# kessel/dune-pnp

Hardware: NVIDIA B200
Metric: newton_step_dofs_per_s (higher is better)
Workload: dtype f64

## Files before the change

### dune_pnp_b200/capi.py

```python
import ctypes as C
import os

import numpy as np

_HERE = os.path.dirname(os.path.abspath(__file__))
LIB_PATH = os.path.join(_HERE, "libpnp_b200.so")

OP_PB, OP_POISSON, OP_DIFFUSION, OP_MASS, OP_PNP = range(5)
JAC_FD_FAITHFUL, JAC_ANALYTIC = 0, 1
SOLVER_BCGS, SOLVER_CG = 0, 1
PREC_NONE, PREC_JACOBI, PREC_SSOR, PREC_ILU0, PREC_AMG = range(5)
TIME_ALEXANDER2, TIME_IMPLICIT_EULER = 0, 1
STATUS = {0: "PNP_OK", 1: "PNP_E_NOT_CONVERGED", 2: "PNP_E_LINEAR_SOLVER", 3: "PNP_E_LINE_SEARCH", 4: "PNP_E_NAN",
          5: "PNP_E_BREAKDOWN", 6: "PNP_E_CUDA", 7: "PNP_E_CONFIG", 8: "PNP_E_ARG", 9: "PNP_E_MESH"}

_dp = C.POINTER(C.c_double)
_ip = C.POINTER(C.c_int)


class LinResult(C.Structure):
    _fields_ = [("converged", C.c_int), ("iterations", C.c_int), ("reduction", C.c_double), ("conv_rate", C.c_double),
                ("seconds", C.c_double), ("status", C.c_int)]


class NewtonOpts(C.Structure):
    _fields_ = [("reduction", C.c_double), ("abs_limit", C.c_double), ("min_linear_reduction", C.c_double),
                ("reassemble_threshold", C.c_double), ("max_iterations", C.c_int),
                ("line_search_max_iterations", C.c_int), ("damping", C.c_double), ("jac_mode", C.c_int),
                ("fd_epsilon", C.c_double), ("verbosity", C.c_int), ("line_search_strategy", C.c_int)]


class NewtonResult(C.Structure):
    _fields_ = [("converged", C.c_int), ("iterations", C.c_int), ("first_defect", C.c_double), ("defect", C.c_double),
                ("reduction", C.c_double), ("linear_iterations", C.c_int), ("line_search_trials", C.c_int),
                ("jacobian_assemblies", C.c_int), ("residual_assemblies", C.c_int), ("seconds_assembly", C.c_double),
                ("seconds_solve", C.c_double), ("seconds_total", C.c_double), ("n_history", C.c_int),
                ("defect_history", C.c_double * 64), ("linear_iterations_history", C.c_int * 64)]


class PnpError(RuntimeError):
    def __init__(self, status, msg):
        super().__init__("%s: %s" % (STATUS.get(status, status), msg))
        self.status = status


_LIB = None


def lib():
    global _LIB
    if _LIB is None:
        if not os.path.exists(LIB_PATH):
            raise ImportError("libpnp_b200.so is missing: run `python -c 'import __graft_entry__ as g; g.build()'` "
                              "(make -C dune_pnp_b200/csrc)")
        try:
            import importlib.util
            for pkg, names in (("nvidia.nccl", ["libnccl.so.2"]), ("nvidia.nvjitlink", ["libnvJitLink.so.12"]),
                               ("nvidia.cublas", ["libcublasLt.so.12", "libcublas.so.12"]),
                               ("nvidia.cusparse", ["libcusparse.so.12"]), ("nvidia.cusolver", ["libcusolver.so.11"])):
                spec = importlib.util.find_spec(pkg)
                if spec is None or not spec.submodule_search_locations:
                    continue
                for nm in names:
                    cand = os.path.join(list(spec.submodule_search_locations)[0], "lib", nm)
                    if os.path.exists(cand):
                        C.CDLL(cand, mode=C.RTLD_GLOBAL)
        except Exception:
            pass
        L = C.CDLL(LIB_PATH)
        L.pnp_last_error.restype = C.c_char_p
        L.pnp_launch_count.restype = C.c_long
        _LIB = L
    return _LIB


def _d(a):
    return None if a is None else a.ctypes.data_as(_dp)


def _i(a):
    return None if a is None else a.ctypes.data_as(_ip)


def tune(name, value):
    st = lib().pnp_tune(name.encode(), C.c_double(value))
    if st != 0:
        raise PnpError(st, "unknown tuning knob " + name)


class Context:

    def __init__(self, device=0, parent=None):
        self._h = C.c_void_p()
        self._children = []
        if parent is not None:
            st = lib().pnp_ctx_create_child(parent._h, C.byref(self._h))
            parent._children.append(self)
        else:
            st = lib().pnp_ctx_create(device, C.byref(self._h))
        if st != 0:
            raise PnpError(st, "cannot create a context on CUDA device %d (no CPU fallback exists)" % device)

    def close(self):
        if self._h:
            lib().pnp_ctx_destroy(self._h)
            self._h = C.c_void_p()

    def __del__(self):
        try:
            self.close()
        except Exception:
            pass

    def _ck(self, st):
        if st != 0:
            raise PnpError(st, lib().pnp_last_error(self._h).decode())

    def profile_spmv(self, enable):
        self._ck(lib().pnp_profile_spmv(self._h, int(enable)))

    def profile_spmv_get(self):
        n = (C.c_long * 3)(); ms = (C.c_double * 3)()
        self._ck(lib().pnp_profile_spmv_get(self._h, n, ms))
        return list(n), list(ms)

    def profile_bytes(self, reset=False):
        out = (C.c_double * 6)()
        self._ck(lib().pnp_profile_bytes(self._h, int(reset), out))
        return dict(zip(("spmv_fine", "spmv_coarse", "assembly", "blas1", "transfer", "dense"), list(out)))

    def profiler_range(self, start):
        self._ck(lib().pnp_profiler_range(self._h, int(start)))

    def timer_start(self):
        self._ck(lib().pnp_timer_start(self._h))

    def timer_stop(self):
        ms = C.c_double()
        self._ck(lib().pnp_timer_stop(self._h, C.byref(ms)))
        return ms.value

    def launch_count(self):
        return lib().pnp_launch_count(self._h)

    def mesh_set(self, x, y, tri, ba, bb, bphys):
        x = np.ascontiguousarray(x, dtype=np.float64); y = np.ascontiguousarray(y, dtype=np.float64)
        tri = np.ascontiguousarray(tri, dtype=np.int32); ba = np.ascontiguousarray(ba, dtype=np.int32)
        bb = np.ascontiguousarray(bb, dtype=np.int32); bphys = np.ascontiguousarray(bphys, dtype=np.int32)
        self._ck(lib().pnp_mesh_set(self._h, C.c_long(len(x)), _d(x), _d(y), C.c_long(len(tri)), _i(tri), C.c_long(len(ba)),
                                    _i(ba), _i(bb), _i(bphys)))

    def mesh_read_gmsh(self, path):
        self._ck(lib().pnp_mesh_read_gmsh(self._h, path.encode()))

    def mesh_refine(self, levels):
        self._ck(lib().pnp_mesh_refine(self._h, levels))

    def carry_set(self, vecs):
        arr = (C.c_int * len(vecs))(*vecs)
        self._ck(lib().pnp_carry_set(self._h, arr, len(vecs)))

    def carry_get(self, index, vec):
        self._ck(lib().pnp_carry_get(self._h, index, vec))

    def carry_set_host(self, field):
        field = np.ascontiguousarray(field, dtype=np.float64)
        self._ck(lib().pnp_carry_set_host(self._h, field.shape[0] if field.ndim == 2 else 1, _d(field)))

    def carry_get_host(self, index, fields):
        out = np.zeros((fields, self.mesh_sizes()["nv"]))
        self._ck(lib().pnp_carry_get_host(self._h, index, _d(out)))
        return out

    def mesh_set_local(self, n_own, x, y, tri, ba, bb, bphys):
        x = np.ascontiguousarray(x, dtype=np.float64); y = np.ascontiguousarray(y, dtype=np.float64)
        tri = np.ascontiguousarray(tri, dtype=np.int32); ba = np.ascontiguousarray(ba, dtype=np.int32)
        bb = np.ascontiguousarray(bb, dtype=np.int32); bphys = np.ascontiguousarray(bphys, dtype=np.int32)
        self._ck(lib().pnp_mesh_set_local(self._h, C.c_long(len(x)), C.c_long(n_own), _d(x), _d(y), C.c_long(len(tri)), _i(tri),
                                          C.c_long(len(ba)), _i(ba), _i(bb), _i(bphys)))

    def mesh_owned(self):
        n = C.c_long()
        self._ck(lib().pnp_mesh_owned(self._h, C.byref(n)))
        return n.value

    @staticmethod
    def comm_unique_id():
        buf = C.create_string_buffer(128)
        if lib().pnp_comm_unique_id(buf) != 0:
            raise PnpError(6, "ncclGetUniqueId failed")
        return buf.raw

    def comm_init(self, rank, world, unique_id):
        self._ck(lib().pnp_comm_init(self._h, rank, world, C.c_char_p(unique_id) if world > 1 else None))

    def halo_set(self, nbr, send_ptr, send_idx, recv_ptr):
        nbr = np.ascontiguousarray(nbr, dtype=np.int32); send_ptr = np.ascontiguousarray(send_ptr, dtype=np.int32)
        send_idx = np.ascontiguousarray(send_idx, dtype=np.int32); recv_ptr = np.ascontiguousarray(recv_ptr, dtype=np.int32)
        self._ck(lib().pnp_halo_set(self._h, len(nbr), _i(nbr), _i(send_ptr), _i(send_idx), _i(recv_ptr)))

    def mg_push_level(self, child, par0, par1):
        par0 = np.ascontiguousarray(par0, dtype=np.int32); par1 = np.ascontiguousarray(par1, dtype=np.int32)
        self._ck(lib().pnp_mg_push_level(self._h, child._h, _i(par0), _i(par1)))

    def mg_set_coarse_global(self, gid, n_global):
        gid = np.ascontiguousarray(gid, dtype=np.int32)
        self._ck(lib().pnp_mg_set_coarse_global(self._h, _i(gid), C.c_long(n_global)))

    def mg_set_coarse_replica(self, replica, gid, n_global):
        gid = np.ascontiguousarray(gid, dtype=np.int32)
        self._ck(lib().pnp_mg_set_coarse_replica(self._h, replica._h, _i(gid), C.c_long(n_global)))

    def mg_set_coarse_aggregates(self, agg, n_agg):
        agg = np.ascontiguousarray(agg, dtype=np.int32)
        self._ck(lib().pnp_mg_set_coarse_aggregates(self._h, _i(agg), C.c_long(n_agg)))

    def halo_exchange(self, vec):
        self._ck(lib().pnp_halo_exchange(self._h, vec))

    def mesh_finalize(self, renumber=True):
        self._ck(lib().pnp_mesh_finalize(self._h, int(renumber)))

    def mesh_sizes(self):
        v = [C.c_long() for _ in range(4)]
        self._ck(lib().pnp_mesh_sizes(self._h, *[C.byref(a) for a in v]))
        return dict(nv=v[0].value, nT=v[1].value, nB=v[2].value, nslots=v[3].value)

    def mesh_get(self):
        s = self.mesh_sizes()
        x = np.zeros(s["nv"]); y = np.zeros(s["nv"]); tri = np.zeros((s["nT"], 3), dtype=np.int32)
        ba = np.zeros(s["nB"], dtype=np.int32); bb = np.zeros(s["nB"], dtype=np.int32); ph = np.zeros(s["nB"], dtype=np.int32)
        self._ck(lib().pnp_mesh_get(self._h, _d(x), _d(y), _i(tri), _i(ba), _i(bb), _i(ph)))
        return dict(x=x, y=y, tri=tri, ba=ba, bb=bb, bphys=ph)

    def params_set(self, sys, surf):
        sys = np.ascontiguousarray(sys, dtype=np.float64); surf = np.ascontiguousarray(surf, dtype=np.float64)
        self._ck(lib().pnp_params_set(self._h, _d(sys), _d(surf)))

    def params_read(self, path):
        self._ck(lib().pnp_params_read(self._h, path.encode()))

    def params_get(self):
        sys = np.zeros(16)
        self._ck(lib().pnp_params_get(self._h, _d(sys), None, None, 0))
        surf = np.zeros((int(sys[0]), 9)); buf = C.create_string_buffer(512)
        self._ck(lib().pnp_params_get(self._h, _d(sys), _d(surf), buf, 512))
        return sys, surf, buf.value.decode()

    def operator(self, op, comp0=0):
        h = C.c_int()
        self._ck(lib().pnp_operator_create(self._h, op, comp0, C.byref(h)))
        return h.value

    def operator_set_coefficient(self, op, which, vec):
        self._ck(lib().pnp_operator_set_coefficient(self._h, op, which, vec))

    def operator_set_valency(self, op, valency):
        self._ck(lib().pnp_operator_set_valency(self._h, op, C.c_double(valency)))

    def constraints(self, op, fields):
        out = np.zeros(fields * self.ndof(), dtype=np.int8)
        self._ck(lib().pnp_constraints_get(self._h, op, out.ctypes.data_as(C.c_char_p)))
        return out.astype(bool)

    def pattern(self, op, fields):
        nv = self.ndof()
        nnz = C.c_long(); rowptr = np.zeros(fields * nv + 1, dtype=np.int32)
        self._ck(lib().pnp_pattern_get(self._h, op, C.byref(nnz), _i(rowptr), None))
        col = np.zeros(nnz.value, dtype=np.int32)
        self._ck(lib().pnp_pattern_get(self._h, op, C.byref(nnz), _i(rowptr), _i(col)))
        return rowptr, col

    def vec(self, fields, host=None):
        h = C.c_int()
        self._ck(lib().pnp_vec_create(self._h, fields, C.byref(h)))
        if host is not None:
            self.upload(h.value, host)
        return h.value

    def vec_destroy(self, v):
        self._ck(lib().pnp_vec_destroy(self._h, v))

    def upload(self, v, host):
        host = np.ascontiguousarray(host, dtype=np.float64)
        self._ck(lib().pnp_vec_upload(self._h, v, _d(host)))

    def download(self, v, fields):
        out = np.zeros(fields * self.ndof())
        self._ck(lib().pnp_vec_download(self._h, v, _d(out)))
        return out

    def vec_set(self, v, value):
        self._ck(lib().pnp_vec_set(self._h, v, C.c_double(value)))

    def vec_copy(self, dst, src):
        self._ck(lib().pnp_vec_copy(self._h, dst, src))

    def axpy(self, y, a, x):
        self._ck(lib().pnp_vec_axpy(self._h, y, C.c_double(a), x))

    def norm(self, x):
        out = C.c_double()
        self._ck(lib().pnp_vec_norm(self._h, x, C.byref(out)))
        return out.value

    def dot(self, x, y):
        out = C.c_double()
        self._ck(lib().pnp_vec_dot(self._h, x, y, C.byref(out)))
        return out.value

    def pack3(self, dst3, phi, cp, cm):
        self._ck(lib().pnp_vec_pack3(self._h, dst3, phi, cp, cm))

    def extract(self, src3, field, dst1):
        self._ck(lib().pnp_vec_extract(self._h, src3, field, dst1))

    def matrix(self, op):
        h = C.c_int()
        self._ck(lib().pnp_matrix_create(self._h, op, C.byref(h)))
        return h.value

    def matrix_destroy(self, m):
        self._ck(lib().pnp_matrix_destroy(self._h, m))

    def residual(self, op, u, r):
        self._ck(lib().pnp_residual(self._h, op, u, r))

    def jacobian(self, op, u, A, mode=JAC_FD_FAITHFUL, eps=1e-11):
        self._ck(lib().pnp_jacobian(self._h, op, u, A, mode, C.c_double(eps)))

    def matrix_values(self, op, A, nnz):
        val = np.zeros(nnz)
        self._ck(lib().pnp_matrix_values_get(self._h, op, A, _d(val)))
        return val

    def spmv(self, A, x, y):
        self._ck(lib().pnp_spmv(self._h, A, x, y))

    def solver(self, kind=SOLVER_BCGS, prec=PREC_NONE, maxit=5000, prec_steps=1, verbosity=0):
        h = C.c_int()
        self._ck(lib().pnp_solver_create(self._h, kind, prec, maxit, prec_steps, verbosity, C.byref(h)))
        return h.value

    def solver_set_option(self, solver, name, value):
        self._ck(lib().pnp_solver_set_option(self._h, solver, name.encode(), C.c_double(value)))

    def solver_get(self, solver, name):
        out = C.c_double(0)
        self._ck(lib().pnp_solver_get(self._h, solver, name.encode(), C.byref(out)))
        return out.value

    def precond_apply(self, solver, A, d, v):
        self._ck(lib().pnp_precond_apply(self._h, solver, A, d, v))

    def solve(self, solver, A, z, r, reduction):
        res = LinResult()
        self._ck(lib().pnp_solver_apply(self._h, solver, A, z, r, C.c_double(reduction), C.byref(res)))
        return res

    def newton_opts(self, **kw):
        o = NewtonOpts()
        self._ck(lib().pnp_newton_opts_from_params(self._h, C.byref(o)))
        for k, v in kw.items():
            setattr(o, k, v)
        return o

    def newton(self, op, u, solver, opts, check=True):
        res = NewtonResult()
        st = lib().pnp_newton_apply(self._h, op, u, solver, C.byref(opts), C.byref(res))
        if check:
            self._ck(st)
        return st, res

    def slp(self, op, u, solver, reduction, jac_mode=JAC_FD_FAITHFUL, eps=1e-11):
        res = LinResult()
        self._ck(lib().pnp_slp_apply(self._h, op, u, solver, C.c_double(reduction), jac_mode, C.c_double(eps), C.byref(res)))
        return res

    def onestep(self, op_space, op_time, solver, dt, x_old, dirichlet_values, x_new, reduction=1e-5, method=TIME_ALEXANDER2,
                jac_mode=JAC_FD_FAITHFUL, eps=1e-11, time=0.0):
        res = (LinResult * 2)()
        self._ck(lib().pnp_onestep_apply(self._h, method, op_space, op_time, solver, C.c_double(time), C.c_double(dt), x_old,
                                         dirichlet_values, x_new, C.c_double(reduction), jac_mode, C.c_double(eps), res))
        return list(res)[: (1 if method == TIME_IMPLICIT_EULER else 2)]

    def ion_flux(self, phi, cp, cm):
        ns = int(self.params_get()[0][0])
        ip = np.zeros(ns); im = np.zeros(ns)
        self._ck(lib().pnp_ion_flux(self._h, phi, cp, cm, _d(ip), _d(im)))
        return ip, im

    def write_cell_data(self, vec, filename):
        self._ck(lib().pnp_write_cell_data(self._h, vec, filename.encode()))

    def write_vtk(self, name, vecs, names, ascii=False):
        arr = (C.c_int * len(vecs))(*vecs)
        nm = (C.c_char_p * len(names))(*[n.encode() for n in names])
        self._ck(lib().pnp_write_vtk(self._h, name.encode(), len(vecs), arr, nm, int(ascii)))

    def matrix_set_csr(self, op, A, rowptr, col, val):
        rowptr = np.ascontiguousarray(rowptr, dtype=np.int32); col = np.ascontiguousarray(col, dtype=np.int32)
        val = np.ascontiguousarray(val, dtype=np.float64)
        self._ck(lib().pnp_matrix_set_csr(self._h, op, A, _i(rowptr), _i(col), _d(val)))

    def mesh_renumber(self, new_index):
        new_index = np.ascontiguousarray(new_index, dtype=np.int32)
        self._ck(lib().pnp_mesh_renumber(self._h, _i(new_index)))

    def space_set_degree(self, degree):
        self._ck(lib().pnp_space_set_degree(self._h, int(degree)))

    def space_sizes(self):
        deg = C.c_int(); nE = C.c_long(); nd = C.c_long()
        self._ck(lib().pnp_space_sizes(self._h, C.byref(deg), C.byref(nE), C.byref(nd)))
        return dict(degree=deg.value, n_edges=nE.value, ndof=nd.value)

    def space_offsets(self):
        eo = C.c_long(); vo = C.c_long()
        self._ck(lib().pnp_space_offsets(self._h, C.byref(eo), C.byref(vo)))
        return eo.value, vo.value

    def operator_set_intorder(self, op, intorder):
        self._ck(lib().pnp_operator_set_intorder(self._h, op, int(intorder)))

    def ndof(self):
        return self.space_sizes()["ndof"]

    def space_edges(self):
        nE = self.space_sizes()["n_edges"]
        va = np.zeros(nE, dtype=np.int32); vb = np.zeros(nE, dtype=np.int32)
        self._ck(lib().pnp_space_edges(self._h, _i(va), _i(vb)))
        return va, vb

    def interpolate_bcext(self, component, pb_vec, out_vec):
        self._ck(lib().pnp_interpolate_bcext(self._h, component, -1 if pb_vec is None else pb_vec, out_vec))
```

### dune_pnp_b200/csrc/pnp_amg.cu

```cuda
#include <cub/cub.cuh>
#include <cusolverDn.h>

#include <chrono>
#include <cmath>
#include <cstdlib>
#include <cstring>

#include "pnp_common.cuh"
#include "pnp_spmv_tma.cuh"
#include "pnp_sweep.cuh"

namespace pnp {

std::shared_ptr<SweepPlan> sweep_plan_build(Ctx&, const SweepView&, int F);
void sweep_gs(Ctx&, const SweepPlan&, const SweepView&, const double* vals, long stride, const double* d, double* x, int dir);

namespace {

constexpr int BLK = 256;

struct Level {
  int nv = 0; long nslots = 0;
  const int* rp = nullptr; const unsigned* col = nullptr; const double* vals = nullptr;
  DBuf<int> rp_own; DBuf<unsigned> col_own; DBuf<double> vals_own;
  DBuf<double> dinv, x, x2, b, r;
  double lmax = 2.0;
  DBuf<int> agg, par1;
  DBuf<int> agg_ptr, agg_mem;
  DBuf<int> seg_ptr, seg_items;
  DBuf<unsigned char> seg_w;
  double alpha = 1.0;
  Ctx* lc = nullptr;
  Vec u; Matrix Amat;
  const unsigned char* dm = nullptr;
  bool redisc = false;
  DBuf<XY> xy_own; DBuf<unsigned char> dmask_own;
  std::shared_ptr<SweepPlan> gs_plan;
};

}

struct Amg {
  int NP = 1, F = 1;
  bool symbolic = false;
  long nv0 = -1, nslots0 = -1;
  long mg_epoch = -1;
  double sym_key = 0.0;
  double omega = 0.7, alpha = 1.6;
  int coarse_sweeps = 40;
  int gamma = 1;
  int wlevels = 99;
  int smoother = 0;
  double cheb_ratio = 8.0;
  int comp0 = 0;
  int pre_steps = -1, post_steps = -1;
  int dense_max = 4096, dense_n = 0;
  cusolverDnHandle_t cus = nullptr;
  DBuf<double> dense, dense_work;
  DBuf<int> dense_piv, dense_info;
  bool distributed = false;
  bool redisc = false;
  DBuf<double> grhs;
  std::unique_ptr<Solver> rep_solver; Matrix rep_A; Vec rep_u; DBuf<double> rep_x;
  int n_geo = 0;
  std::vector<std::unique_ptr<Level>> L;
  DBuf<unsigned char> tmp;
  void* temp(size_t bytes) { if (bytes > tmp.n) tmp.alloc(bytes); return tmp.p; }
  cudaGraphExec_t cg_exec = nullptr;
  bool cg_failed = false;
  int cg_calls = 0;
  double cg_key[8] = {0, 0, 0, 0, 0, 0, 0, 0};
  std::vector<std::pair<double*, double*>> cg_before, cg_after;
  long cg_launches = 0; double cg_bytes[Ctx::ACC_N] = {0, 0, 0, 0, 0, 0};
  void cg_reset() { if (cg_exec) cudaGraphExecDestroy(cg_exec); cg_exec = nullptr; cg_calls = 0; }
  ~Amg() { if (cg_exec) cudaGraphExecDestroy(cg_exec); if (cus) cusolverDnDestroy(cus); }
};

namespace {

__device__ __forceinline__ unsigned hash32(unsigned x) {
  x ^= x >> 16; x *= 0x7feb352du; x ^= x >> 15; x *= 0x846ca68bu; x ^= x >> 16;
  return x;
}
__global__ void k_mis_select(const int* __restrict__ rp, const unsigned* __restrict__ col, int nv,
                             const unsigned char* __restrict__ st, unsigned char* __restrict__ st_out) {
  for (int v = blockIdx.x * blockDim.x + threadIdx.x; v < nv; v += gridDim.x * blockDim.x) {
    unsigned char s = st[v];
    if (s == 0) {
      const unsigned pv = hash32((unsigned)v);
      bool win = true;
      for (int k = rp[v] + 1; k < rp[v + 1]; k++) {
        const int w = (int)(col[k] & STAR_VMASK);
        if (w >= nv || w == v || st[w] != 0) continue;
        const unsigned pw = hash32((unsigned)w);
        if (pw > pv || (pw == pv && w > v)) { win = false; break; }
      }
      if (win) s = 1;
    }
    st_out[v] = s;
  }
}
__global__ void k_mis_cover(const int* __restrict__ rp, const unsigned* __restrict__ col, int nv,
                            unsigned char* __restrict__ st, int* __restrict__ undecided) {
  int local = 0;
  for (int v = blockIdx.x * blockDim.x + threadIdx.x; v < nv; v += gridDim.x * blockDim.x) {
    if (st[v] != 0) continue;
    bool covered = false;
    for (int k = rp[v] + 1; k < rp[v + 1]; k++) {
      const int w = (int)(col[k] & STAR_VMASK);
      if (w < nv && st[w] == 1) { covered = true; break; }
    }
    if (covered) st[v] = 2; else local++;
  }
  if (local) atomicAdd(undecided, local);
}
__global__ void k_root_flag(const unsigned char* __restrict__ st, int nv, int* __restrict__ flag) {
  for (int v = blockIdx.x * blockDim.x + threadIdx.x; v < nv; v += gridDim.x * blockDim.x) flag[v] = st[v] == 1;
}
__global__ void k_attach(const int* __restrict__ rp, const unsigned* __restrict__ col, const double* __restrict__ vals,
                         int nv, const unsigned char* __restrict__ st, const int* __restrict__ root_id,
                         int* __restrict__ agg) {
  for (int v = blockIdx.x * blockDim.x + threadIdx.x; v < nv; v += gridDim.x * blockDim.x) {
    if (st[v] == 1) { agg[v] = root_id[v]; continue; }
    double best = -1.0; int bw = -1;
    for (int k = rp[v] + 1; k < rp[v + 1]; k++) {
      const int w = (int)(col[k] & STAR_VMASK);
      if (w >= nv || st[w] != 1) continue;
      const double s = fabs(vals[k]);
      if (s > best || (s == best && w < bw)) { best = s; bw = w; }
    }
    agg[v] = root_id[bw];
  }
}
__global__ void k_coarse_keys(const int* __restrict__ rp, const unsigned* __restrict__ col, int nv,
                              const int* __restrict__ agg, uint64_t* __restrict__ keys, int* __restrict__ slot_id) {
  for (int v = blockIdx.x * blockDim.x + threadIdx.x; v < nv; v += gridDim.x * blockDim.x) {
    const unsigned I = (unsigned)agg[v];
    for (int k = rp[v]; k < rp[v + 1]; k++) {
      const unsigned w = col[k] & STAR_VMASK;
      if (w >= (unsigned)nv) { keys[k] = ~0ull; slot_id[k] = k; continue; }
      const unsigned J = (unsigned)agg[w];
      keys[k] = ((uint64_t)I << 32) | (J == I ? 0u : J + 1u);
      slot_id[k] = k;
    }
  }
}
__global__ void k_coarse_cols(const uint64_t* __restrict__ ukeys, long n, unsigned* __restrict__ col) {
  for (long i = blockIdx.x * (long)blockDim.x + threadIdx.x; i < n; i += (long)gridDim.x * blockDim.x) {
    const unsigned lo = (unsigned)(ukeys[i] & 0xffffffffu);
    col[i] = lo == 0 ? (unsigned)(ukeys[i] >> 32) : lo - 1u;
  }
}
__global__ void k_row_starts(const uint64_t* __restrict__ ukeys, long n, int nc, int* __restrict__ rp) {
  for (int I = blockIdx.x * blockDim.x + threadIdx.x; I <= nc; I += gridDim.x * blockDim.x)
    rp[I] = (int)lower_bound_u64(ukeys, n, (uint64_t)(unsigned)I << 32);
}
__global__ void k_lower_bounds_i32(const int* __restrict__ sorted, int n, int m, int* __restrict__ out) {
  for (int I = blockIdx.x * blockDim.x + threadIdx.x; I <= m; I += gridDim.x * blockDim.x) {
    int lo = 0, hi = n;
    while (lo < hi) { int mid = (lo + hi) >> 1; if (sorted[mid] < I) lo = mid + 1; else hi = mid; }
    out[I] = lo;
  }
}
__global__ void k_iota(int* a, int n) {
  for (int i = blockIdx.x * blockDim.x + threadIdx.x; i < n; i += gridDim.x * blockDim.x) a[i] = i;
}

template <int NP>
__global__ void k_galerkin(const int* __restrict__ seg_ptr, const int* __restrict__ seg_items,
                           const unsigned char* __restrict__ seg_w, long nsc, const double* __restrict__ vf, long nsf, double* __restrict__ vc,
                           const unsigned char* __restrict__ dmask, const unsigned* __restrict__ colf, const int* __restrict__ rpf,
                           int comp0) {
  for (long cs = blockIdx.x * (long)blockDim.x + threadIdx.x; cs < nsc; cs += (long)gridDim.x * blockDim.x) {
    double acc[NP];
#pragma unroll
    for (int p = 0; p < NP; p++) acc[p] = 0.0;
    constexpr int U = 4;
    const int t1 = seg_ptr[cs + 1];
    for (int t0 = seg_ptr[cs]; t0 < t1; t0 += U) {
      int s[U]; double w[U]; double v[U][NP];
#pragma unroll
      for (int q = 0; q < U; q++) {
        const bool ok = t0 + q < t1;
        s[q] = ok ? seg_items[t0 + q] : -1;
        const unsigned char wc = (ok && seg_w) ? seg_w[t0 + q] : 0;
        w[q] = ok ? (wc == 0 ? 1.0 : (wc == 1 ? 0.5 : 0.25)) : 0.0;
      }
#pragma unroll
      for (int q = 0; q < U; q++)
#pragma unroll
        for (int p = 0; p < NP; p++) v[q][p] = s[q] >= 0 ? vf[p * nsf + s[q]] : 0.0;
      if (dmask) {
#pragma unroll
        for (int q = 0; q < U; q++) {
          if (s[q] < 0) continue;
          const unsigned wv = colf[s[q]] & STAR_VMASK;
          const unsigned m = dmask[wv];
          if (m && rpf[wv] == s[q]) {
            if (NP == 1) { if ((m >> comp0) & 1u) v[q][0] = 0.0; }
            else if (NP == PNP_COMPACT_PLANES) { if (m & 1u) v[q][0] = 0.0; }
            else {
              if (m & 1u) v[q][0] = 0.0;
              if (m & 2u) v[q][NP == 7 ? 4 : 0] = 0.0;
              if (m & 4u) v[q][NP == 7 ? 6 : 0] = 0.0;
            }
          }
        }
      }
#pragma unroll
      for (int q = 0; q < U; q++)
        if (s[q] >= 0) {
#pragma unroll
          for (int p = 0; p < NP; p++) acc[p] += w[q] * v[q][p];
        }
    }
#pragma unroll
    for (int p = 0; p < NP; p++) vc[p * nsc + cs] = acc[p];
  }
}
template <int NP>
__global__ void k_dinv(const int* __restrict__ rp, const double* __restrict__ vals, long stride, int nv,
                       double* __restrict__ dinv) {
  for (int v = blockIdx.x * blockDim.x + threadIdx.x; v < nv; v += gridDim.x * blockDim.x) {
    const int s = rp[v];
    if (NP == 1) { const double d = vals[s]; dinv[v] = d != 0.0 ? 1.0 / d : 0.0; }
    else {
      const PnpBlock B = pnp_block_at<NP>(vals, stride, s);
      const double a = B.a, b = B.b, c_ = B.c, d = B.d, e = B.e, f = B.f, g = B.g;
      const double det = a * e * g - b * d * g - c_ * e * f;
      double* o = dinv + 9l * v;
      const double scale = fabs(a * e * g) + fabs(b * d * g) + fabs(c_ * e * f);
      if (fabs(det) > 1e-12 * scale && scale > 0.0) {
        const double id = 1.0 / det;
        o[0] = e * g * id;   o[1] = -b * g * id;           o[2] = -c_ * e * id;
        o[3] = -d * g * id;  o[4] = (a * g - c_ * f) * id; o[5] = c_ * d * id;
        o[6] = -e * f * id;  o[7] = b * f * id;            o[8] = (a * e - b * d) * id;
      } else {
        for (int i = 0; i < 9; i++) o[i] = 0.0;
        o[0] = a != 0.0 ? 1.0 / a : 0.0; o[4] = e != 0.0 ? 1.0 / e : 0.0; o[8] = g != 0.0 ? 1.0 / g : 0.0;
      }
    }
  }
}
template <int F>
__global__ void k_jacobi0(const double* __restrict__ dinv, const double* __restrict__ b, double omega,
                          double* __restrict__ x, int nv, double* __restrict__ dvec) {
  for (int v = blockIdx.x * blockDim.x + threadIdx.x; v < nv; v += gridDim.x * blockDim.x) {
    if (F == 1) {
      const double z = omega * dinv[v] * b[v];
      x[v] = z; if (dvec) dvec[v] = z;
    } else {
      const double* B = dinv + 9l * v;
      const double r0 = b[3l * v], r1 = b[3l * v + 1], r2 = b[3l * v + 2];
#pragma unroll
      for (int k = 0; k < 3; k++) {
        const double z = omega * (B[3 * k] * r0 + B[3 * k + 1] * r1 + B[3 * k + 2] * r2);
        x[3l * v + k] = z; if (dvec) dvec[3l * v + k] = z;
      }
    }
  }
}
template <int NP>
__global__ void k_gershgorin(const int* __restrict__ rp, const double* __restrict__ vals, long stride, int nv,
                             unsigned long long* __restrict__ out) {
  double best = 0.0;
  for (int v = blockIdx.x * blockDim.x + threadIdx.x; v < nv; v += gridDim.x * blockDim.x) {
    const int s0 = rp[v], s1 = rp[v + 1];
    if (NP == 1) {
      double sum = 0.0;
      for (int s = s0; s < s1; s++) sum += fabs(vals[s]);
      const double d = fabs(vals[s0]);
      if (d > 0.0) best = fmax(best, sum / d);
    } else {
      double s0_ = 0.0, s1_ = 0.0, s2_ = 0.0;
      for (int s = s0; s < s1; s++) {
        const PnpBlock B = pnp_block_at<NP>(vals, stride, s);
        s0_ += fabs(B.a) + fabs(B.b) + fabs(B.c);
        s1_ += fabs(B.d) + fabs(B.e);
        s2_ += fabs(B.f) + fabs(B.g);
      }
      const PnpBlock D = pnp_block_at<NP>(vals, stride, s0);
      const double d0 = fabs(D.a), d1 = fabs(D.e), d2 = fabs(D.g);
      if (d0 > 0.0) best = fmax(best, s0_ / d0);
      if (d1 > 0.0) best = fmax(best, s1_ / d1);
      if (d2 > 0.0) best = fmax(best, s2_ / d2);
    }
  }
  for (int o = 16; o > 0; o >>= 1) best = fmax(best, __shfl_xor_sync(0xffffffffu, best, o));
  if ((threadIdx.x & 31) == 0) atomicMax(out, (unsigned long long)__double_as_longlong(best));
}
template <int F>
__global__ void k_restrict(const int* __restrict__ agg_ptr, const int* __restrict__ agg_mem, const int* __restrict__ par1,
                           int nc, const double* __restrict__ r, double* __restrict__ bc) {
  for (int I = blockIdx.x * blockDim.x + threadIdx.x; I < nc; I += gridDim.x * blockDim.x) {
    double acc[F];
#pragma unroll
    for (int k = 0; k < F; k++) acc[k] = 0.0;
    for (int t = agg_ptr[I]; t < agg_ptr[I + 1]; t++) {
      const long v = agg_mem[t];
      const double w = (par1 && par1[v] >= 0) ? 0.5 : 1.0;
#pragma unroll
      for (int k = 0; k < F; k++) acc[k] += w * r[F * v + k];
    }
#pragma unroll
    for (int k = 0; k < F; k++) bc[(long)F * I + k] = acc[k];
  }
}
template <int F>
__global__ void k_prolong(const int* __restrict__ agg, const int* __restrict__ par1, int nv, const double* __restrict__ xc,
                          double alpha, double* __restrict__ x, const unsigned char* __restrict__ dmask, int comp0) {
  for (int v = blockIdx.x * blockDim.x + threadIdx.x; v < nv; v += gridDim.x * blockDim.x) {
    const long I = agg[v];
    const long J = par1 ? par1[v] : -1;
    const unsigned m = dmask ? (F == 3 ? dmask[v] : (dmask[v] >> comp0) & 1u) : 0u;
#pragma unroll
    for (int k = 0; k < F; k++)
      if (!((m >> k) & 1u))
        x[(long)F * v + k] += alpha * (J >= 0 ? 0.5 * (xc[F * I + k] + xc[F * J + k]) : xc[F * I + k]);
  }
}
__global__ void k_level_geometry(const int* __restrict__ int2ext_c, const int* __restrict__ ext2int_f, const XY* __restrict__ xy_f,
                                 const unsigned char* __restrict__ dmask_f, int nvc, XY* __restrict__ xy_c,
                                 unsigned char* __restrict__ dmask_c) {
  for (int i = blockIdx.x * blockDim.x + threadIdx.x; i < nvc; i += gridDim.x * blockDim.x) {
    const int j = ext2int_f[int2ext_c[i]];
    xy_c[i] = xy_f[j]; dmask_c[i] = dmask_f[j];
  }
}
__global__ void k_geo_parents(const int* __restrict__ int2ext_f, int nvf, int nvc, const uint64_t* __restrict__ edges,
                              const int* __restrict__ ext2int_c, int* __restrict__ par0, int* __restrict__ par1) {
  for (int i = blockIdx.x * blockDim.x + threadIdx.x; i < nvf; i += gridDim.x * blockDim.x) {
    const int e = int2ext_f[i];
    if (e < nvc) { par0[i] = ext2int_c[e]; par1[i] = -1; }
    else {
      const uint64_t k = edges[e - nvc];
      par0[i] = ext2int_c[(int)(k >> 32)]; par1[i] = ext2int_c[(int)(k & 0xffffffffu)];
    }
  }
}
__global__ void k_geo_pairs(const int* __restrict__ par0, const int* __restrict__ par1, int nvf, int nrows_c,
                            int* __restrict__ key, int* __restrict__ val) {
  for (int i = blockIdx.x * blockDim.x + threadIdx.x; i < nvf; i += gridDim.x * blockDim.x) {
    key[2 * i] = (par0[i] >= 0 && par0[i] < nrows_c) ? par0[i] : 0x7fffffff; val[2 * i] = i;
    key[2 * i + 1] = (par1[i] >= 0 && par1[i] < nrows_c) ? par1[i] : 0x7fffffff; val[2 * i + 1] = i;
  }
}
template <int F>
__global__ void k_inject(const int* __restrict__ par0, const int* __restrict__ par1, int nvf, const double* __restrict__ uf,
                         double* __restrict__ uc) {
  for (int i = blockIdx.x * blockDim.x + threadIdx.x; i < nvf; i += gridDim.x * blockDim.x)
    if (par1[i] < 0 && par0[i] >= 0) {
#pragma unroll
      for (int k = 0; k < F; k++) uc[(long)F * par0[i] + k] = uf[(long)F * i + k];
    }
}
template <int F>
__global__ void k_mask_dirichlet(double* __restrict__ b, const unsigned char* __restrict__ dmask, int nv, int comp0) {
  for (int v = blockIdx.x * blockDim.x + threadIdx.x; v < nv; v += gridDim.x * blockDim.x) {
    const unsigned m = F == 3 ? dmask[v] : (dmask[v] >> comp0) & 1u;
#pragma unroll
    for (int k = 0; k < F; k++) if ((m >> k) & 1u) b[(long)F * v + k] = 0.0;
  }
}
template <int NP>
__global__ void k_dense_fill_global(const int* __restrict__ rp, const unsigned* __restrict__ col, const double* __restrict__ vals,
                                    long stride, int nrows, const int* __restrict__ gid, double* __restrict__ Ad, long n,
                                    const unsigned char* __restrict__ dmask, int comp0) {
  constexpr int F = NP == 1 ? 1 : 3;
  for (int r = blockIdx.x * blockDim.x + threadIdx.x; r < nrows; r += gridDim.x * blockDim.x) {
    const long rg = gid[r];
    for (int s = rp[r]; s < rp[r + 1]; s++) {
      const long cg = gid[col[s] & STAR_VMASK];
      const unsigned dm = (dmask && s == rp[r]) ? dmask[r] : 0u;
      if (NP == 1) { if (!((dm >> comp0) & 1u)) atomicAdd(&Ad[cg * n + rg], vals[s]); }
      else {
        const PnpBlock B = pnp_block_at<NP>(vals, stride, s);
#pragma unroll
        for (int ki = 0; ki < 3; ki++)
#pragma unroll
          for (int kj = 0; kj < 3; kj++)
            if (pnp_plane(ki, kj) >= 0 && !(ki == kj && ((dm >> ki) & 1u))) atomicAdd(&Ad[(F * cg + kj) * n + F * rg + ki], B.at(ki, kj));
      }
    }
  }
}
template <int F>
__global__ void k_to_global(const double* __restrict__ loc, const int* __restrict__ gid, int nrows, double* __restrict__ glob) {
  for (int v = blockIdx.x * blockDim.x + threadIdx.x; v < nrows; v += gridDim.x * blockDim.x)
#pragma unroll
    for (int k = 0; k < F; k++) atomicAdd(&glob[(long)F * gid[v] + k], loc[(long)F * v + k]);
}
template <int F>
__global__ void k_add_from_global(const double* __restrict__ glob, const int* __restrict__ gid, int nrows, double alpha,
                                  double* __restrict__ x, const unsigned char* __restrict__ dmask, int comp0) {
  for (int v = blockIdx.x * blockDim.x + threadIdx.x; v < nrows; v += gridDim.x * blockDim.x) {
    const unsigned m = F == 3 ? dmask[v] : (dmask[v] >> comp0) & 1u;
#pragma unroll
    for (int k = 0; k < F; k++) if (!((m >> k) & 1u)) x[(long)F * v + k] += alpha * glob[(long)F * gid[v] + k];
  }
}
template <int F>
__global__ void k_from_global(const double* __restrict__ glob, const int* __restrict__ gid, int nloc, double* __restrict__ loc) {
  for (int v = blockIdx.x * blockDim.x + threadIdx.x; v < nloc; v += gridDim.x * blockDim.x)
#pragma unroll
    for (int k = 0; k < F; k++) loc[(long)F * v + k] = glob[(long)F * gid[v] + k];
}
__device__ __forceinline__ int find_slot(const int* rp, const unsigned* col, int I, int J) {
  for (int s = rp[I]; s < rp[I + 1]; s++) if ((int)(col[s] & STAR_VMASK) == J) return s;
  return -1;
}
__global__ void k_geo_items(const int* __restrict__ rpf, const unsigned* __restrict__ colf, int nvf,
                            const int* __restrict__ par0, const int* __restrict__ par1, const int* __restrict__ rpc,
                            const unsigned* __restrict__ colc, int* __restrict__ key, unsigned* __restrict__ val,
                            int* __restrict__ err) {
  for (int i = blockIdx.x * blockDim.x + threadIdx.x; i < nvf; i += gridDim.x * blockDim.x) {
    const int I[2] = {par0[i], par1[i]};
    for (int s = rpf[i]; s < rpf[i + 1]; s++) {
      const int j = (int)(colf[s] & STAR_VMASK);
      const int J[2] = {par0[j], par1[j]};
#pragma unroll
      for (int a = 0; a < 2; a++)
#pragma unroll
        for (int b = 0; b < 2; b++) {
          const long o = 4l * s + 2 * a + b;
          if (I[a] < 0 || J[b] < 0) { key[o] = 0x7fffffff; val[o] = 0; continue; }
          const int cs = find_slot(rpc, colc, I[a], J[b]);
          if (cs < 0) { atomicExch(err, 1); key[o] = 0x7fffffff; val[o] = 0; continue; }
          const unsigned wc = (I[1] >= 0 ? 1u : 0u) + (J[1] >= 0 ? 1u : 0u);
          key[o] = cs; val[o] = (unsigned)s | (wc << 29);
        }
    }
  }
}
__global__ void k_geo_unpack(const unsigned* __restrict__ val, long n, int* __restrict__ items, unsigned char* __restrict__ w) {
  for (long t = blockIdx.x * (long)blockDim.x + threadIdx.x; t < n; t += (long)gridDim.x * blockDim.x) {
    items[t] = (int)(val[t] & 0x1fffffffu); w[t] = (unsigned char)(val[t] >> 29);
  }
}

#define KL(c, kern, n, ...)                                                                              \
  do { kern<<<grid_for((n), BLK), BLK, 0, (c).stream>>>(__VA_ARGS__); PNP_CHECK_LAUNCH(); (c).launches++; } while (0)

template <int EPI>
void level_op(Ctx& c, const Amg& A, const Level& l, const double* x, const double* b, double* y, double omega_or_c2 = -1.0,
              double c1 = 0.0, double* dvec = nullptr) {
  StarOpArgs a{l.rp, l.col, l.vals, l.nslots, l.nv, x, y};
  a.b = b; a.dinv = l.dinv.p; a.block = A.F == 3; a.omega = omega_or_c2 < 0 ? A.omega : omega_or_c2; a.c1 = c1; a.dvec = dvec;
  const bool fine = &l == A.L[0].get();
  if (A.distributed) halo_exchange(*l.lc, const_cast<double*>(x), A.F);
  if (fine) c.prof_mark(EPI == EPI_RESIDUAL ? 1 : 2);
  launch_star_op_auto<EPI, 0>(c, A.NP, a, fine);
  if (fine) c.prof_mark();
}

bool coarsen(Ctx& c, Amg& A, int li) {
  Level& f = *A.L[li];
  const int nv = f.nv;
  DBuf<unsigned char> st(nv), st2(nv);
  st.zero(c.stream);
  DBuf<int> d_und(1);
  for (int round = 0; round < 200; round++) {
    KL(c, k_mis_select, nv, f.rp, f.col, nv, st.p, st2.p);
    std::swap(st.p, st2.p);
    d_und.zero(c.stream);
    KL(c, k_mis_cover, nv, f.rp, f.col, nv, st.p, d_und.p);
    int und = 0;
    d_und.download(&und, 1, c.stream);
    if (und == 0) break;
    PNP_REQUIRE(round < 199, PNP_E_ARG, "AMG: independent-set selection did not terminate");
  }
  DBuf<int> flag(nv), root_id(nv);
  KL(c, k_root_flag, nv, st.p, nv, flag.p);
  size_t bytes = 0;
  cub::DeviceScan::ExclusiveSum(nullptr, bytes, flag.p, root_id.p, nv, c.stream);
  PNP_CUDA(cub::DeviceScan::ExclusiveSum(A.temp(bytes), bytes, flag.p, root_id.p, nv, c.stream));
  int last_id = 0, last_flag = 0;
  PNP_CUDA(cudaMemcpyAsync(&last_id, root_id.p + nv - 1, sizeof(int), cudaMemcpyDeviceToHost, c.stream));
  PNP_CUDA(cudaMemcpyAsync(&last_flag, flag.p + nv - 1, sizeof(int), cudaMemcpyDeviceToHost, c.stream));
  PNP_CUDA(cudaStreamSynchronize(c.stream));
  const int nc = last_id + last_flag;
  if (nc < 1 || nc > 0.8 * nv) return false;
  f.alpha = A.alpha;
  f.agg.alloc(nv);
  KL(c, k_attach, nv, f.rp, f.col, f.vals, nv, st.p, root_id.p, f.agg.p);
  {
    DBuf<int> ids(nv), agg_sorted(nv);
    f.agg_mem.alloc(nv); f.agg_ptr.alloc(nc + 1);
    KL(c, k_iota, nv, ids.p, nv);
    cub::DeviceRadixSort::SortPairs(nullptr, bytes, f.agg.p, agg_sorted.p, ids.p, f.agg_mem.p, nv, 0, 32, c.stream);
    PNP_CUDA(cub::DeviceRadixSort::SortPairs(A.temp(bytes), bytes, f.agg.p, agg_sorted.p, ids.p, f.agg_mem.p, nv, 0, 32,
                                            c.stream));
    KL(c, k_lower_bounds_i32, nc + 1, agg_sorted.p, nv, nc, f.agg_ptr.p);
  }
  auto nl = std::make_unique<Level>();
  {
    const long ns = f.nslots;
    PNP_REQUIRE(ns < (1l << 31), PNP_E_MESH, "AMG: too many matrix slots on one level");
    DBuf<uint64_t> keys(ns), skeys(ns), ukeys(ns);
    DBuf<int> slot(ns), counts(ns + 1), d_nu(1);
    f.seg_items.alloc(ns);
    KL(c, k_coarse_keys, nv, f.rp, f.col, nv, f.agg.p, keys.p, slot.p);
    cub::DeviceRadixSort::SortPairs(nullptr, bytes, keys.p, skeys.p, slot.p, f.seg_items.p, (int)ns, 0, 64, c.stream);
    PNP_CUDA(cub::DeviceRadixSort::SortPairs(A.temp(bytes), bytes, keys.p, skeys.p, slot.p, f.seg_items.p, (int)ns, 0, 64,
                                            c.stream));
    cub::DeviceRunLengthEncode::Encode(nullptr, bytes, skeys.p, ukeys.p, counts.p, d_nu.p, (int)ns, c.stream);
    PNP_CUDA(cub::DeviceRunLengthEncode::Encode(A.temp(bytes), bytes, skeys.p, ukeys.p, counts.p, d_nu.p, (int)ns, c.stream));
    int nu = 0;
    d_nu.download(&nu, 1, c.stream);
    {
      uint64_t lastkey = 0;
      PNP_CUDA(cudaMemcpyAsync(&lastkey, ukeys.p + (nu - 1), sizeof(uint64_t), cudaMemcpyDeviceToHost, c.stream));
      PNP_CUDA(cudaStreamSynchronize(c.stream));
      if (lastkey == ~0ull) nu--;
    }
    nl->nv = nc; nl->nslots = nu;
    PNP_CUDA(cudaMemsetAsync(counts.p + nu, 0, sizeof(int), c.stream));
    f.seg_ptr.alloc((size_t)nu + 1);
    cub::DeviceScan::ExclusiveSum(nullptr, bytes, counts.p, f.seg_ptr.p, nu + 1, c.stream);
    PNP_CUDA(cub::DeviceScan::ExclusiveSum(A.temp(bytes), bytes, counts.p, f.seg_ptr.p, nu + 1, c.stream));
    nl->rp_own.alloc((size_t)nc + 1); nl->col_own.alloc(nu);
    KL(c, k_row_starts, nc + 1, ukeys.p, (long)nu, nc, nl->rp_own.p);
    KL(c, k_coarse_cols, nu, ukeys.p, (long)nu, nl->col_own.p);
    c.launches += 8;
    PNP_CUDA(cudaStreamSynchronize(c.stream));
  }
  nl->vals_own.alloc((size_t)A.NP * nl->nslots);
  nl->rp = nl->rp_own.p; nl->col = nl->col_own.p; nl->vals = nl->vals_own.p;
  A.L.push_back(std::move(nl));
  return true;
}

void coarsen_geometric(Ctx& c, Amg& A, int li, const HierLevel& h, const int* int2ext_f, bool redisc) {
  Level& f = *A.L[li];
  const int nvf = f.nv, nvc = (int)h.nv;
  size_t bytes = 0;
  f.agg.alloc(nvf); f.par1.alloc(nvf);
  KL(c, k_geo_parents, nvf, int2ext_f, nvf, nvc, h.edges.p, h.ext2int.p, f.agg.p, f.par1.p);
  {
    DBuf<int> key(2 * (size_t)nvf), val(2 * (size_t)nvf), skey(2 * (size_t)nvf), sval(2 * (size_t)nvf);
    KL(c, k_geo_pairs, nvf, f.agg.p, f.par1.p, nvf, nvc, key.p, val.p);
    cub::DeviceRadixSort::SortPairs(nullptr, bytes, key.p, skey.p, val.p, sval.p, 2 * nvf, 0, 32, c.stream);
    PNP_CUDA(cub::DeviceRadixSort::SortPairs(A.temp(bytes), bytes, key.p, skey.p, val.p, sval.p, 2 * nvf, 0, 32, c.stream));
    f.agg_ptr.alloc((size_t)nvc + 1);
    KL(c, k_lower_bounds_i32, nvc + 1, skey.p, 2 * nvf, nvc, f.agg_ptr.p);
    int nvalid = 0;
    PNP_CUDA(cudaMemcpyAsync(&nvalid, f.agg_ptr.p + nvc, sizeof(int), cudaMemcpyDeviceToHost, c.stream));
    PNP_CUDA(cudaStreamSynchronize(c.stream));
    f.agg_mem.alloc(nvalid);
    PNP_CUDA(cudaMemcpyAsync(f.agg_mem.p, sval.p, (size_t)nvalid * sizeof(int), cudaMemcpyDeviceToDevice, c.stream));
    PNP_CUDA(cudaStreamSynchronize(c.stream));
  }
  auto nl = std::make_unique<Level>();
  nl->nv = nvc; nl->nslots = h.nslots; nl->rp = h.rp.p; nl->col = h.adj.p;
  nl->redisc = redisc;
  if (redisc) {
    nl->xy_own.alloc(nvc); nl->dmask_own.alloc(nvc);
    KL(c, k_level_geometry, nvc, h.int2ext.p, c.ext2int.p, c.xy.p, c.dmask.p, nvc, nl->xy_own.p, nl->dmask_own.p);
    nl->dm = nl->dmask_own.p;
    nl->u.fields = A.F; nl->u.d.alloc((size_t)A.F * nvc);
  } else {
    const long n4 = 4 * f.nslots;
    PNP_REQUIRE(n4 < (1l << 31) && f.nslots < (1l << 29), PNP_E_MESH, "multigrid: too many matrix slots on one level");
    DBuf<int> key(n4), skey(n4), err(1);
    DBuf<unsigned> val(n4), sval(n4);
    err.zero(c.stream);
    KL(c, k_geo_items, nvf, f.rp, f.col, nvf, f.agg.p, f.par1.p, nl->rp, nl->col, key.p, val.p, err.p);
    int herr = 0;
    err.download(&herr, 1, c.stream);
    PNP_REQUIRE(herr == 0, PNP_E_MESH, "multigrid: refinement levels are not nested");
    cub::DeviceRadixSort::SortPairs(nullptr, bytes, key.p, skey.p, val.p, sval.p, (int)n4, 0, 32, c.stream);
    PNP_CUDA(cub::DeviceRadixSort::SortPairs(A.temp(bytes), bytes, key.p, skey.p, val.p, sval.p, (int)n4, 0, 32, c.stream));
    key.release(); val.release();
    f.seg_ptr.alloc((size_t)nl->nslots + 1);
    KL(c, k_lower_bounds_i32, nl->nslots + 1, skey.p, (int)n4, (int)nl->nslots, f.seg_ptr.p);
    int nvalid = 0;
    PNP_CUDA(cudaMemcpyAsync(&nvalid, f.seg_ptr.p + nl->nslots, sizeof(int), cudaMemcpyDeviceToHost, c.stream));
    PNP_CUDA(cudaStreamSynchronize(c.stream));
    f.seg_items.alloc(nvalid); f.seg_w.alloc(nvalid);
    KL(c, k_geo_unpack, nvalid, sval.p, (long)nvalid, f.seg_items.p, f.seg_w.p);
    PNP_CUDA(cudaStreamSynchronize(c.stream));
    c.launches += 4;
  }
  f.alpha = 1.0;
  nl->vals_own.alloc((size_t)A.NP * nl->nslots);
  nl->vals = nl->vals_own.p;
  A.L.push_back(std::move(nl));
}

void alloc_work(Ctx& c, Amg& A, Level& l) {
  const size_t n = (size_t)A.F * l.nv, nall = (A.distributed && l.lc) ? (size_t)A.F * l.lc->nv : n;
  l.dinv.alloc(A.F == 3 ? 9 * (size_t)l.nv : n); l.x.alloc(nall); l.x2.alloc(nall); l.b.alloc(nall); l.r.alloc(nall);
  l.x.zero(c.stream); l.x2.zero(c.stream); l.b.zero(c.stream); l.r.zero(c.stream);
}

void coarsen_distributed(Ctx& c, Amg& A, int li, MgLevelRef& ref) {
  Level& f = *A.L[li];
  Ctx& fc = *f.lc; Ctx& kc = *ref.lc;
  const int nvf_all = (int)fc.nv, nvc = (int)kc.n_own;
  size_t bytes = 0;
  f.agg.alloc(nvf_all); f.par1.alloc(nvf_all);
  PNP_CUDA(cudaMemcpyAsync(f.agg.p, ref.par0.p, nvf_all * sizeof(int), cudaMemcpyDeviceToDevice, c.stream));
  PNP_CUDA(cudaMemcpyAsync(f.par1.p, ref.par1.p, nvf_all * sizeof(int), cudaMemcpyDeviceToDevice, c.stream));
  {
    DBuf<int> key(2 * (size_t)nvf_all), val(2 * (size_t)nvf_all), skey(2 * (size_t)nvf_all), sval(2 * (size_t)nvf_all);
    KL(c, k_geo_pairs, nvf_all, f.agg.p, f.par1.p, nvf_all, nvc, key.p, val.p);
    cub::DeviceRadixSort::SortPairs(nullptr, bytes, key.p, skey.p, val.p, sval.p, 2 * nvf_all, 0, 32, c.stream);
    PNP_CUDA(cub::DeviceRadixSort::SortPairs(A.temp(bytes), bytes, key.p, skey.p, val.p, sval.p, 2 * nvf_all, 0, 32, c.stream));
    f.agg_ptr.alloc((size_t)nvc + 1);
    KL(c, k_lower_bounds_i32, nvc + 1, skey.p, 2 * nvf_all, nvc, f.agg_ptr.p);
    int nvalid = 0;
    PNP_CUDA(cudaMemcpyAsync(&nvalid, f.agg_ptr.p + nvc, sizeof(int), cudaMemcpyDeviceToHost, c.stream));
    PNP_CUDA(cudaStreamSynchronize(c.stream));
    f.agg_mem.alloc(nvalid);
    PNP_CUDA(cudaMemcpyAsync(f.agg_mem.p, sval.p, (size_t)nvalid * sizeof(int), cudaMemcpyDeviceToDevice, c.stream));
    PNP_CUDA(cudaStreamSynchronize(c.stream));
  }
  f.alpha = 1.0;
  auto nl = std::make_unique<Level>();
  nl->lc = &kc; nl->nv = nvc; nl->nslots = kc.nslots; nl->rp = kc.rp.p; nl->col = kc.adj.p;
  nl->dm = kc.dmask.p;
  nl->u.fields = A.F; nl->u.d.alloc((size_t)A.F * kc.nv); nl->u.d.zero(c.stream);
  nl->Amat.op = A.F == 3 ? OP_PNP : OP_PB; nl->Amat.nplanes = A.NP;
  nl->Amat.vals.alloc((size_t)A.NP * kc.nslots);
  nl->vals = nl->Amat.vals.p;
  A.L.push_back(std::move(nl));
}

void dense_factor(Ctx& c, Amg& A);

void dense_factor_global(Ctx& c, Amg& A);
void replica_setup(Ctx& c, Amg& A);

const double* level_values(Ctx& c, Amg& A, int li, const double* uf, int comp0) {
  Level& l = *A.L[li]; Level& n = *A.L[li + 1];
  if (n.redisc) {
    if (A.F == 1) KL(c, k_inject<1>, l.nv, l.agg.p, l.par1.p, l.nv, uf, n.u.d.p);
    else KL(c, k_inject<3>, l.nv, l.agg.p, l.par1.p, l.nv, uf, n.u.d.p);
    c.acct(Ctx::ACC_TRANSFER, 8.0 * l.nv + 16.0 * A.F * n.nv);
    Operator op = c.last_op; op.aux0 = op.aux1 = -1;
    assemble_jacobian_on(c, StarView{n.rp, n.col, n.xy_own.p, n.dmask_own.p, n.nv}, n.nslots, op, n.u.d.p, n.vals_own.p,
                         A.NP, c.last_mode, c.last_eps);
    return n.u.d.p;
  }
  if (A.NP == 1)
    KL(c, k_galerkin<1>, n.nslots, l.seg_ptr.p, l.seg_items.p, l.seg_w.p, n.nslots, l.vals, l.nslots, n.vals_own.p, l.dm, l.col, l.rp, comp0);
  else if (A.NP == PNP_COMPACT_PLANES)
    KL(c, k_galerkin<PNP_COMPACT_PLANES>, n.nslots, l.seg_ptr.p, l.seg_items.p, l.seg_w.p, n.nslots, l.vals, l.nslots, n.vals_own.p, l.dm, l.col, l.rp, comp0);
  else
    KL(c, k_galerkin<7>, n.nslots, l.seg_ptr.p, l.seg_items.p, l.seg_w.p, n.nslots, l.vals, l.nslots, n.vals_own.p, l.dm, l.col, l.rp, comp0);
  c.acct(Ctx::ACC_ASSEMBLY, 8.0 * A.NP * ((double)l.nslots + (double)n.nslots) + 5.0 * (double)l.seg_items.n + 4.0 * (double)n.nslots);
  return nullptr;
}

void level_dinv(Ctx& c, Amg& A, Level& l) {
  if (A.NP == 1) KL(c, k_dinv<1>, l.nv, l.rp, l.vals, l.nslots, l.nv, l.dinv.p);
  else if (A.NP == PNP_COMPACT_PLANES) KL(c, k_dinv<PNP_COMPACT_PLANES>, l.nv, l.rp, l.vals, l.nslots, l.nv, l.dinv.p);
  else KL(c, k_dinv<7>, l.nv, l.rp, l.vals, l.nslots, l.nv, l.dinv.p);
}

void gershgorin_bounds(Ctx& c, Amg& A) {
  DBuf<unsigned long long> d_l(A.L.size());
  d_l.zero(c.stream);
  for (size_t li = 0; li < A.L.size(); li++) {
    Level& l = *A.L[li];
    if (A.NP == 1) KL(c, k_gershgorin<1>, l.nv, l.rp, l.vals, l.nslots, l.nv, d_l.p + li);
    else if (A.NP == PNP_COMPACT_PLANES) KL(c, k_gershgorin<PNP_COMPACT_PLANES>, l.nv, l.rp, l.vals, l.nslots, l.nv, d_l.p + li);
    else KL(c, k_gershgorin<7>, l.nv, l.rp, l.vals, l.nslots, l.nv, d_l.p + li);
  }
  if (A.distributed) allreduce_max_u64(c, d_l.p, A.L.size());
  std::vector<unsigned long long> h = d_l.to_host(c.stream);
  for (size_t li = 0; li < A.L.size(); li++) {
    double v; std::memcpy(&v, &h[li], sizeof v);
    A.L[li]->lmax = (v > 0.0 && std::isfinite(v)) ? v : 2.0;
  }
}

void numeric(Ctx& c, Amg& A, int comp0) {
  if (A.distributed) {
    PNP_REQUIRE(c.last_u, PNP_E_ARG, "distributed multigrid needs the state of the last Jacobian assembly (the vector must stay alive)");
    PNP_REQUIRE(c.last_vals == A.L[0]->vals, PNP_E_ARG,
                "distributed multigrid re-discretises its coarse levels: the matrix must be the Jacobian of the last assembly");
    const double* uf = c.last_u;
    for (size_t li = 0; li + 1 < A.L.size(); li++) {
      Level& l = *A.L[li]; Level& n = *A.L[li + 1];
      const int nvf_all = (int)l.lc->nv;
      if (A.F == 1) KL(c, k_inject<1>, nvf_all, l.agg.p, l.par1.p, nvf_all, uf, n.u.d.p);
      else KL(c, k_inject<3>, nvf_all, l.agg.p, l.par1.p, nvf_all, uf, n.u.d.p);
      c.acct(Ctx::ACC_TRANSFER, 8.0 * nvf_all + 16.0 * A.F * n.nv);
      Operator op = c.last_op; op.aux0 = op.aux1 = -1;
      n.Amat.op = op.op;
      n.lc->launches = 0;
      assemble_jacobian(*n.lc, op, n.u, n.Amat, c.last_mode, c.last_eps);
      c.absorb(*n.lc);
      uf = n.u.d.p;
    }
    for (size_t li = 0; li < A.L.size(); li++) {
      Level& l = *A.L[li];
      level_dinv(c, A, l);
      c.acct(Ctx::ACC_ASSEMBLY, (4.0 + 8.0 * A.NP + (A.F == 3 ? 72.0 : 8.0)) * l.nv);
    }
    if (c.mg_replica) replica_setup(c, A); else dense_factor_global(c, A);
    if (A.smoother == 1) gershgorin_bounds(c, A);
    return;
  }
  const double* uf = c.last_u;
  for (size_t li = 0; li < A.L.size(); li++) {
    Level& l = *A.L[li];
    if (li + 1 < A.L.size()) uf = level_values(c, A, (int)li, uf, comp0);
    level_dinv(c, A, l);
    c.acct(Ctx::ACC_ASSEMBLY, (4.0 + 8.0 * A.NP + (A.F == 3 ? 72.0 : 8.0)) * l.nv);
  }
  A.dense_n = 0;
  if ((long)A.F * A.L.back()->nv <= A.dense_max) dense_factor(c, A);
  if (A.smoother == 1) gershgorin_bounds(c, A);
}

template <int NP>
__global__ void k_dense_fill(const int* __restrict__ rp, const unsigned* __restrict__ col, const double* __restrict__ vals,
                             long stride, int nv, double* __restrict__ Ad, long n) {
  constexpr int F = NP == 1 ? 1 : 3;
  for (int r = blockIdx.x * blockDim.x + threadIdx.x; r < nv; r += gridDim.x * blockDim.x)
    for (int s = rp[r]; s < rp[r + 1]; s++) {
      const long cidx = col[s] & STAR_VMASK;
      if (cidx >= nv) continue;
      if (NP == 1) Ad[cidx * n + r] = vals[s];
      else {
        const PnpBlock B = pnp_block_at<NP>(vals, stride, s);
#pragma unroll
        for (int ki = 0; ki < 3; ki++)
#pragma unroll
          for (int kj = 0; kj < 3; kj++)
            if (pnp_plane(ki, kj) >= 0) Ad[(F * cidx + kj) * n + F * r + ki] = B.at(ki, kj);
      }
    }
}
__global__ void k_dense_fix_diag(double* __restrict__ Ad, long n) {
  for (long i = blockIdx.x * (long)blockDim.x + threadIdx.x; i < n; i += (long)gridDim.x * blockDim.x)
    if (Ad[i * n + i] == 0.0) Ad[i * n + i] = 1.0;
}
#define PNP_CUSOLVER(call)                                                                                          \
  do { cusolverStatus_t s_ = (call); if (s_ != CUSOLVER_STATUS_SUCCESS)                                             \
    throw ::pnp::Error(PNP_E_CUDA, std::string(#call) + " -> cusolver status " + std::to_string((int)s_)); } while (0)

void dense_factor(Ctx& c, Amg& A) {
  Level& l = *A.L.back();
  const long n = (long)A.F * l.nv;
  A.dense_n = (int)n;
  if (!A.cus) PNP_CUSOLVER(cusolverDnCreate(&A.cus));
  PNP_CUSOLVER(cusolverDnSetStream(A.cus, c.stream));
  if (A.dense.n != (size_t)(n * n)) { A.dense.alloc(n * n); A.dense_piv.alloc(n); A.dense_info.alloc(1); }
  A.dense.zero(c.stream);
  if (A.NP == 1) KL(c, k_dense_fill<1>, l.nv, l.rp, l.col, l.vals, l.nslots, l.nv, A.dense.p, n);
  else if (A.NP == PNP_COMPACT_PLANES) KL(c, k_dense_fill<PNP_COMPACT_PLANES>, l.nv, l.rp, l.col, l.vals, l.nslots, l.nv, A.dense.p, n);
  else KL(c, k_dense_fill<7>, l.nv, l.rp, l.col, l.vals, l.nslots, l.nv, A.dense.p, n);
  KL(c, k_dense_fix_diag, n, A.dense.p, n);
  int lwork = 0;
  PNP_CUSOLVER(cusolverDnDgetrf_bufferSize(A.cus, (int)n, (int)n, A.dense.p, (int)n, &lwork));
  if (A.dense_work.n < (size_t)lwork) A.dense_work.alloc(lwork);
  PNP_CUSOLVER(cusolverDnDgetrf(A.cus, (int)n, (int)n, A.dense.p, (int)n, A.dense_work.p, A.dense_piv.p, A.dense_info.p));
  c.acct(Ctx::ACC_DENSE, 24.0 * (double)n * (double)n);
  int info = 0;
  A.dense_info.download(&info, 1, c.stream);
  PNP_REQUIRE(info == 0, PNP_E_BREAKDOWN, "multigrid: coarsest-level matrix is singular (LU info " + std::to_string(info) + ")");
}
void dense_solve(Ctx& c, Amg& A, Level& l) {
  const long n = A.dense_n;
  PNP_CUDA(cudaMemcpyAsync(l.x.p, l.b.p, n * sizeof(double), cudaMemcpyDeviceToDevice, c.stream));
  PNP_CUSOLVER(cusolverDnDgetrs(A.cus, CUBLAS_OP_N, (int)n, 1, A.dense.p, (int)n, A.dense_piv.p, l.x.p, (int)n, A.dense_info.p));
  c.launches += 2; c.acct(Ctx::ACC_DENSE, 8.0 * (double)n * (double)n);
}

void dense_factor_global(Ctx& c, Amg& A) {
  Level& l = *A.L.back();
  const long n = (long)A.F * c.mg_nglobal;
  A.dense_n = (int)n;
  if (!A.cus) PNP_CUSOLVER(cusolverDnCreate(&A.cus));
  PNP_CUSOLVER(cusolverDnSetStream(A.cus, c.stream));
  if (A.dense.n != (size_t)(n * n)) { A.dense.alloc(n * n); A.dense_piv.alloc(n); A.dense_info.alloc(1); A.grhs.alloc(n); }
  A.dense.zero(c.stream);
  const unsigned char* dm = c.mg_aggregated ? l.lc->dmask.p : nullptr;
  if (A.NP == 1) KL(c, k_dense_fill_global<1>, l.nv, l.rp, l.col, l.vals, l.nslots, l.nv, c.mg_gid.p, A.dense.p, n, dm, A.comp0);
  else if (A.NP == PNP_COMPACT_PLANES)
    KL(c, k_dense_fill_global<PNP_COMPACT_PLANES>, l.nv, l.rp, l.col, l.vals, l.nslots, l.nv, c.mg_gid.p, A.dense.p, n, dm, A.comp0);
  else KL(c, k_dense_fill_global<7>, l.nv, l.rp, l.col, l.vals, l.nslots, l.nv, c.mg_gid.p, A.dense.p, n, dm, A.comp0);
  allreduce_sum(c, A.dense.p, (size_t)(n * n));
  KL(c, k_dense_fix_diag, n, A.dense.p, n);
  int lwork = 0;
  PNP_CUSOLVER(cusolverDnDgetrf_bufferSize(A.cus, (int)n, (int)n, A.dense.p, (int)n, &lwork));
  if (A.dense_work.n < (size_t)lwork) A.dense_work.alloc(lwork);
  static const bool timing = std::getenv("PNP_AMG_TIMING") != nullptr;
  if (timing) PNP_CUDA(cudaStreamSynchronize(c.stream));
  const auto t0 = std::chrono::steady_clock::now();
  PNP_CUSOLVER(cusolverDnDgetrf(A.cus, (int)n, (int)n, A.dense.p, (int)n, A.dense_work.p, A.dense_piv.p, A.dense_info.p));
  int info = 0;
  A.dense_info.download(&info, 1, c.stream);
  if (timing) std::printf("[amg] rank %d global dense LU n = %ld: %.1f ms\n", c.rank, n,
                          1e3 * std::chrono::duration<double>(std::chrono::steady_clock::now() - t0).count());
  PNP_REQUIRE(info == 0, PNP_E_BREAKDOWN, "multigrid: coarsest-level matrix is singular (LU info " + std::to_string(info) + ")");
}
void dense_correct_aggregated(Ctx& c, Amg& A, Level& l) {
  const long n = A.dense_n;
  A.grhs.zero(c.stream);
  if (A.F == 1) KL(c, k_to_global<1>, l.nv, l.r.p, c.mg_gid.p, l.nv, A.grhs.p);
  else KL(c, k_to_global<3>, l.nv, l.r.p, c.mg_gid.p, l.nv, A.grhs.p);
  allreduce_sum(c, A.grhs.p, (size_t)n);
  PNP_CUSOLVER(cusolverDnDgetrs(A.cus, CUBLAS_OP_N, (int)n, 1, A.dense.p, (int)n, A.dense_piv.p, A.grhs.p, (int)n, A.dense_info.p));
  if (A.F == 1) KL(c, k_add_from_global<1>, l.nv, A.grhs.p, c.mg_gid.p, l.nv, A.alpha, l.x.p, l.lc->dmask.p, A.comp0);
  else KL(c, k_add_from_global<3>, l.nv, A.grhs.p, c.mg_gid.p, l.nv, A.alpha, l.x.p, l.lc->dmask.p, A.comp0);
  c.launches += 2;
}
void dense_solve_global(Ctx& c, Amg& A, Level& l) {
  const long n = A.dense_n;
  A.grhs.zero(c.stream);
  if (A.F == 1) KL(c, k_to_global<1>, l.nv, l.b.p, c.mg_gid.p, l.nv, A.grhs.p);
  else KL(c, k_to_global<3>, l.nv, l.b.p, c.mg_gid.p, l.nv, A.grhs.p);
  allreduce_sum(c, A.grhs.p, (size_t)n);
  PNP_CUSOLVER(cusolverDnDgetrs(A.cus, CUBLAS_OP_N, (int)n, 1, A.dense.p, (int)n, A.dense_piv.p, A.grhs.p, (int)n, A.dense_info.p));
  const int nloc = (int)l.lc->nv;
  if (A.F == 1) KL(c, k_from_global<1>, nloc, A.grhs.p, c.mg_gid.p, nloc, l.x.p);
  else KL(c, k_from_global<3>, nloc, A.grhs.p, c.mg_gid.p, nloc, l.x.p);
  c.launches += 2;
}

}
void amg_setup(Ctx& c, Solver& S, const Matrix& M);
void amg_apply(Ctx& c, Solver& S, const Matrix&, const double* d, double* y);
namespace {
void replica_setup(Ctx& c, Amg& A) {
  Ctx& rc = *c.mg_replica;
  Level& l = *A.L.back();
  const long n = (long)A.F * c.mg_nglobal;
  A.dense_n = (int)n;
  if (A.grhs.n != (size_t)n) { A.grhs.alloc(n); A.rep_x.alloc(n); A.rep_u.d.alloc(n); }
  A.rep_u.fields = A.F;
  A.rep_u.d.zero(c.stream);
  if (A.F == 1) KL(c, k_to_global<1>, l.nv, l.u.d.p, c.mg_gid.p, l.nv, A.rep_u.d.p);
  else KL(c, k_to_global<3>, l.nv, l.u.d.p, c.mg_gid.p, l.nv, A.rep_u.d.p);
  allreduce_sum(c, A.rep_u.d.p, (size_t)n);
  Operator op = c.last_op; op.aux0 = op.aux1 = -1;
  A.rep_A.op = op.op; A.rep_A.nplanes = A.NP;
  if (A.rep_A.vals.n != (size_t)A.NP * rc.nslots) A.rep_A.vals.alloc((size_t)A.NP * rc.nslots);
  rc.launches = 0;
  assemble_jacobian(rc, op, A.rep_u, A.rep_A, c.last_mode, c.last_eps);
  if (!A.rep_solver) { A.rep_solver = std::make_unique<Solver>(); A.rep_solver->prec = PNP_PREC_AMG; }
  auto& ro = A.rep_solver->opts;
  ro["amg_geometric"] = 1;  ro["amg_omega"] = A.omega; ro["amg_alpha"] = A.alpha; ro["amg_gamma"] = A.gamma;
  ro["amg_dense_max"] = A.dense_max; ro["amg_coarse_sweeps"] = A.coarse_sweeps; ro["amg_smoother"] = A.smoother;
  ro["amg_cheb_ratio"] = A.cheb_ratio; ro["amg_pre_steps"] = A.pre_steps; ro["amg_post_steps"] = A.post_steps;
  amg_setup(rc, *A.rep_solver, A.rep_A);
  c.absorb(rc);
}
void replica_solve(Ctx& c, Amg& A, Level& l, int nu) {
  Ctx& rc = *c.mg_replica;
  const long n = (long)A.F * c.mg_nglobal;
  A.grhs.zero(c.stream);
  if (A.F == 1) KL(c, k_to_global<1>, l.nv, l.b.p, c.mg_gid.p, l.nv, A.grhs.p);
  else KL(c, k_to_global<3>, l.nv, l.b.p, c.mg_gid.p, l.nv, A.grhs.p);
  allreduce_sum(c, A.grhs.p, (size_t)n);
  A.rep_solver->prec_steps = nu;
  rc.launches = 0;
  amg_apply(rc, *A.rep_solver, A.rep_A, A.grhs.p, A.rep_x.p);
  const int nloc = (int)l.lc->nv;
  if (A.F == 1) KL(c, k_from_global<1>, nloc, A.rep_x.p, c.mg_gid.p, nloc, l.x.p);
  else KL(c, k_from_global<3>, nloc, A.rep_x.p, c.mg_gid.p, nloc, l.x.p);
  c.absorb(rc); c.launches += 2;
}

void jacobi0(Ctx& c, Amg& A, Level& l, double omega, double* dvec) {
  if (A.F == 1) KL(c, k_jacobi0<1>, l.nv, l.dinv.p, l.b.p, omega, l.x.p, l.nv, dvec);
  else KL(c, k_jacobi0<3>, l.nv, l.dinv.p, l.b.p, omega, l.x.p, l.nv, dvec);
  c.acct(Ctx::ACC_TRANSFER, ((A.F == 3 ? 72.0 : 8.0) + 16.0 * A.F + (dvec ? 8.0 * A.F : 0.0)) * l.nv);
}

void smooth(Ctx& c, Amg& A, Level& l, int steps, bool zero) {
  const long n = (long)A.F * l.nv;
  if (steps <= 0) { if (zero) PNP_CUDA(cudaMemsetAsync(l.x.p, 0, n * sizeof(double), c.stream)); return; }
  if (A.smoother == 0) {
    int s = 0;
    if (zero) { jacobi0(c, A, l, A.omega, nullptr); s = 1; }
    for (; s < steps; s++) { level_op<2>(c, A, l, l.x.p, l.b.p, l.x2.p); std::swap(l.x.p, l.x2.p); }
    return;
  }
  if (A.smoother == 2) {
    const bool finest = &l == A.L[0].get();
    const SweepView V{l.rp, l.col, finest ? c.int2ext.p : nullptr, l.nv};
    if (!l.gs_plan) l.gs_plan = sweep_plan_build(c, V, A.F);
    if (zero) PNP_CUDA(cudaMemsetAsync(l.x.p, 0, n * sizeof(double), c.stream));
    for (int s = 0; s < steps; s++) {
      sweep_gs(c, *l.gs_plan, V, l.vals, l.nslots, l.b.p, l.x.p, +1);
      sweep_gs(c, *l.gs_plan, V, l.vals, l.nslots, l.b.p, l.x.p, -1);
    }
    c.acct(finest ? Ctx::ACC_SPMV_FINE : Ctx::ACC_SPMV_COARSE, 2.0 * steps * ((8.0 * A.NP + 4.0) * (double)l.nslots + 24.0 * n));
    return;
  }
  const double lmx = 1.1 * l.lmax, lmn = l.lmax / A.cheb_ratio;
  const double theta = 0.5 * (lmx + lmn), delta = 0.5 * (lmx - lmn), sigma = theta / delta;
  double rho = 1.0 / sigma;
  int s = 0;
  if (zero) { jacobi0(c, A, l, 1.0 / theta, l.r.p); s = 1; }
  else { level_op<3>(c, A, l, l.x.p, l.b.p, l.x2.p, 1.0 / theta, 0.0, l.r.p); std::swap(l.x.p, l.x2.p); s = 1; }
  for (; s < steps; s++) {
    const double rho_new = 1.0 / (2.0 * sigma - rho);
    level_op<3>(c, A, l, l.x.p, l.b.p, l.x2.p, 2.0 * rho_new / delta, rho_new * rho, l.r.p);
    std::swap(l.x.p, l.x2.p);
    rho = rho_new;
  }
}

void cycle(Ctx& c, Amg& A, int li, int nu, int comp0, bool zero);

void coarse_correction(Ctx& c, Amg& A, int nu, int comp0) {
  auto direct = [&] {
    const int visits = 0 < A.wlevels ? A.gamma : 1;
    for (int g = 0; g < visits; g++) cycle(c, A, 1, nu, comp0, g == 0);
  };
  auto snapshot = [&](std::vector<std::pair<double*, double*>>& v) {
    v.clear();
    for (size_t li = 1; li < A.L.size(); li++) v.push_back({A.L[li]->x.p, A.L[li]->x2.p});
  };
  auto restore = [&](const std::vector<std::pair<double*, double*>>& v) {
    for (size_t li = 1; li < A.L.size(); li++) { A.L[li]->x.p = v[li - 1].first; A.L[li]->x2.p = v[li - 1].second; }
  };
  cudaStreamCaptureStatus cap = cudaStreamCaptureStatusNone;
  PNP_CUDA(cudaStreamIsCapturing(c.stream, &cap));
  if (!tune().graph || A.cg_failed || A.smoother != 0 || cap != cudaStreamCaptureStatusNone) { direct(); return; }
  const double key[8] = {(double)nu, A.omega, (double)A.gamma, (double)A.wlevels, (double)A.pre_steps, (double)A.post_steps,
                         (double)A.coarse_sweeps, (double)comp0 + 16.0 * A.dense_n};
  if (A.cg_exec && std::memcmp(key, A.cg_key, sizeof key) != 0) A.cg_reset();
  if (!A.cg_exec) {
    if (A.cg_calls++ < 1) { direct(); return; }
    std::memcpy(A.cg_key, key, sizeof key);
    snapshot(A.cg_before);
    const long l0 = c.launches;
    double b0[Ctx::ACC_N];
    for (int k = 0; k < Ctx::ACC_N; k++) b0[k] = c.alg_bytes[k];
    cudaGraph_t graph = nullptr;
    bool ok = cudaStreamBeginCapture(c.stream, cudaStreamCaptureModeThreadLocal) == cudaSuccess;
    if (ok) {
      try { direct(); } catch (const Error&) { ok = false; }
      if (cudaStreamEndCapture(c.stream, &graph) != cudaSuccess || !graph) ok = false;
    }
    if (ok && cudaGraphInstantiate(&A.cg_exec, graph, 0) != cudaSuccess) { ok = false; A.cg_exec = nullptr; }
    if (graph) cudaGraphDestroy(graph);
    A.cg_launches = c.launches - l0; c.launches = l0;
    for (int k = 0; k < Ctx::ACC_N; k++) { A.cg_bytes[k] = c.alg_bytes[k] - b0[k]; c.alg_bytes[k] = b0[k]; }
    snapshot(A.cg_after);
    if (!ok) {
      cudaGetLastError();
      A.cg_failed = true; A.cg_exec = nullptr;
      restore(A.cg_before);
      direct();
      return;
    }
  }
  restore(A.cg_before);
  PNP_CUDA(cudaGraphLaunch(A.cg_exec, c.stream));
  restore(A.cg_after);
  c.launches += A.cg_launches;
  for (int k = 0; k < Ctx::ACC_N; k++) c.alg_bytes[k] += A.cg_bytes[k];
}

void cycle(Ctx& c, Amg& A, int li, int nu, int comp0, bool zero) {
  Level& l = *A.L[li];
  const bool coarsest = li + 1 == (int)A.L.size();
  if (coarsest && A.dense_n > 0 && A.distributed && c.mg_aggregated) {
    smooth(c, A, l, nu, zero);
    level_op<1>(c, A, l, l.x.p, l.b.p, l.r.p);
    dense_correct_aggregated(c, A, l);
    smooth(c, A, l, nu, false);
    return;
  }
  if (coarsest && A.dense_n > 0) {
    if (A.distributed && c.mg_replica) replica_solve(c, A, l, nu);
    else if (A.distributed) dense_solve_global(c, A, l);
    else dense_solve(c, A, l);
    return;
  }
  const int nu_pre = A.pre_steps >= 0 ? A.pre_steps : nu, nu_post = A.post_steps >= 0 ? A.post_steps : nu;
  smooth(c, A, l, coarsest ? A.coarse_sweeps : nu_pre, zero);
  if (coarsest) return;
  Level& nx = *A.L[li + 1];
  level_op<1>(c, A, l, l.x.p, l.b.p, l.r.p);
  if (A.distributed) halo_exchange(*l.lc, l.r.p, A.F);
  if (A.F == 1) KL(c, k_restrict<1>, nx.nv, l.agg_ptr.p, l.agg_mem.p, l.par1.p, nx.nv, l.r.p, nx.b.p);
  else KL(c, k_restrict<3>, nx.nv, l.agg_ptr.p, l.agg_mem.p, l.par1.p, nx.nv, l.r.p, nx.b.p);
  c.acct(Ctx::ACC_TRANSFER, (8.0 * A.F + 4.0) * l.nv + 4.0 * (double)l.agg_mem.n + (8.0 * A.F + 4.0) * nx.nv);
  if (nx.dm) {
    if (A.F == 1) KL(c, k_mask_dirichlet<1>, nx.nv, nx.b.p, nx.dm, nx.nv, comp0);
    else KL(c, k_mask_dirichlet<3>, nx.nv, nx.b.p, nx.dm, nx.nv, comp0);
    c.acct(Ctx::ACC_TRANSFER, 1.0 * nx.nv);
  }
  if (li == 0) coarse_correction(c, A, nu, comp0);
  else {
    const int visits = li < A.wlevels ? A.gamma : 1;
    for (int g = 0; g < visits; g++) cycle(c, A, li + 1, nu, comp0, g == 0);
  }
  if (A.distributed && !(li + 2 == (int)A.L.size() && A.dense_n > 0 && !c.mg_aggregated)) halo_exchange(*nx.lc, nx.x.p, A.F);
  const unsigned char* dm = l.dm;
  if (A.F == 1) KL(c, k_prolong<1>, l.nv, l.agg.p, l.par1.p, l.nv, nx.x.p, l.alpha, l.x.p, dm, comp0);
  else KL(c, k_prolong<3>, l.nv, l.agg.p, l.par1.p, l.nv, nx.x.p, l.alpha, l.x.p, dm, comp0);
  c.acct(Ctx::ACC_TRANSFER, (16.0 * A.F + 9.0) * l.nv + 8.0 * A.F * nx.nv);
  smooth(c, A, l, nu_post, false);
}

}

int amg_graph_state(const Solver& S) { return !S.amg ? 0 : (S.amg->cg_exec ? 1 : (S.amg->cg_failed ? -1 : 0)); }

void amg_setup(Ctx& c, Solver& S, const Matrix& M) {
  if (!S.amg) S.amg = std::make_shared<Amg>();
  Amg& A = *S.amg;
  const int comp0 = M.comp0;
  A.comp0 = comp0;
  const bool want_redisc = S.opt("amg_geometric", 1) != 0 && S.opt("amg_rediscretise", 1) != 0 && c.n_own == c.nv &&
                           !c.hier.empty() && c.mg.empty() && c.last_u && c.last_vals == M.vals.p &&
                           (M.op == OP_PB || M.op == OP_PNP || M.op == OP_MASS);
  const double sym_key = S.opt("amg_geometric", 1) + 3.0 * S.opt("amg_dense_max", 4096) + 1e7 * S.opt("amg_alpha", 1.6);
  if (!A.symbolic || A.NP != M.nplanes || A.nv0 != c.n_own || A.nslots0 != c.nslots || A.redisc != want_redisc ||
      A.mg_epoch != c.mg_epoch || A.sym_key != sym_key) {
    A.L.clear(); A.cg_reset(); A.cg_failed = false;
    A.NP = M.nplanes; A.F = M.nplanes == 1 ? 1 : 3;
    A.nv0 = c.n_own; A.nslots0 = c.nslots; A.mg_epoch = c.mg_epoch; A.sym_key = sym_key;
    auto l0 = std::make_unique<Level>();
    l0->nv = (int)c.n_own; l0->nslots = c.nslots; l0->rp = c.rp.p; l0->col = c.adj.p; l0->vals = M.vals.p;
    A.L.push_back(std::move(l0));
    A.alpha = S.opt("amg_alpha", 1.6);
    A.L[0]->lc = &c;
    A.L[0]->dm = c.dmask.p;
    A.redisc = want_redisc;
    A.distributed = S.opt("amg_geometric", 1) != 0 && !c.mg.empty() && c.mg_nglobal > 0 &&
                    (M.op == OP_PB || M.op == OP_PNP || M.op == OP_MASS);
    if (A.distributed) {
      for (auto& ref : c.mg) coarsen_distributed(c, A, (int)A.L.size() - 1, ref);
      A.n_geo = (int)c.mg.size();
    }
    const bool geometric = !A.distributed && S.opt("amg_geometric", 1) != 0 && c.n_own == c.nv && !c.hier.empty();
    if (!A.distributed) A.n_geo = 0;
    if (geometric) {
      const int* i2e = c.int2ext.p;
      const double* uf = c.last_u;
      for (int hi = (int)c.hier.size() - 1; hi >= 0; hi--) {
        const int li = (int)A.L.size() - 1;
        coarsen_geometric(c, A, li, c.hier[hi], i2e, A.redisc);
        i2e = c.hier[hi].int2ext.p;
        uf = level_values(c, A, li, uf, comp0);
        A.n_geo++;
      }
    }
    A.dense_max = (int)S.opt("amg_dense_max", 4096);
    for (int li = (int)A.L.size() - 1; li < 24 && !A.distributed; li++) {
      if (A.L[li]->nv <= 64 || (long)A.F * A.L[li]->nv <= A.dense_max) break;
      if (!coarsen(c, A, li)) break;
      level_values(c, A, li, nullptr, comp0);
    }
    for (auto& l : A.L) alloc_work(c, A, *l);
    if (!A.distributed) {
      Level& l0r = *A.L[0];
      const size_t nall = (size_t)A.F * c.nv;
      l0r.x.alloc(nall); l0r.x2.alloc(nall);
      l0r.x.zero(c.stream); l0r.x2.zero(c.stream);
    }
    A.symbolic = true;
    if (S.verbosity > 0) {
      std::printf("multigrid hierarchy (%d geometric transfers):", A.n_geo);
      for (auto& l : A.L) std::printf(" %d", l->nv);
      std::printf("\n");
    }
  }
  A.L[0]->vals = M.vals.p;
  static const bool timing = std::getenv("PNP_AMG_TIMING") != nullptr;
  if (timing) PNP_CUDA(cudaStreamSynchronize(c.stream));
  const auto t_num0 = std::chrono::steady_clock::now();
  A.omega = S.opt("amg_omega", 0.7); A.gamma = (int)S.opt("amg_gamma", 1); A.wlevels = (int)S.opt("amg_wlevels", 99);
  A.coarse_sweeps = (int)S.opt("amg_coarse_sweeps", 40); A.smoother = (int)S.opt("amg_smoother", 0);
  PNP_REQUIRE(A.smoother >= 0 && A.smoother <= 2, PNP_E_ARG, "amg_smoother: 0 damped Jacobi, 1 Chebyshev, 2 symmetric Gauss-Seidel");
  PNP_REQUIRE(A.smoother != 2 || !A.distributed, PNP_E_ARG, "the Gauss-Seidel smoother sweeps the rows of one GPU: use Jacobi / Chebyshev on a partitioned mesh");
  PNP_REQUIRE(A.smoother != 2 || A.NP != PNP_COMPACT_PLANES, PNP_E_ARG, "the Gauss-Seidel smoother sweeps 7-plane PNP matrices only");
  A.cheb_ratio = S.opt("amg_cheb_ratio", 8.0);
  A.pre_steps = (int)S.opt("amg_pre_steps", -1); A.post_steps = (int)S.opt("amg_post_steps", -1);
  numeric(c, A, comp0);
  if (timing) {
    PNP_CUDA(cudaStreamSynchronize(c.stream));
    std::printf("[amg] rank %d numeric setup %.1f ms (levels %zu, dense n = %d, distributed %d)\n", c.rank,
                1e3 * std::chrono::duration<double>(std::chrono::steady_clock::now() - t_num0).count(), A.L.size(), A.dense_n,
                (int)A.distributed);
  }
}

void amg_apply(Ctx& c, Solver& S, const Matrix&, const double* d, double* y) {
  Amg& A = *S.amg;
  Level& l0 = *A.L[0];
  const long n = (long)A.F * l0.nv;
  const int nu = S.prec_steps > 0 ? S.prec_steps : 1;
  if (c.n_own == c.nv) {
    double *keep_b = l0.b.p, *keep_x = l0.x.p, *keep_x2 = l0.x2.p;
    const int pre = A.pre_steps >= 0 ? A.pre_steps : nu, post = A.post_steps >= 0 ? A.post_steps : nu;
    const int swaps = A.smoother == 2 ? 0 : (pre > 0 ? pre - 1 : 0) + post;
    struct Restore {
      Level& l; double *b, *x, *x2;
      ~Restore() { l.b.p = b; l.x.p = x; l.x2.p = x2; }
    } restore{l0, keep_b, keep_x, keep_x2};
    l0.b.p = const_cast<double*>(d);
    if (swaps & 1) l0.x2.p = y; else l0.x.p = y;
    cycle(c, A, 0, nu, A.comp0, true);
    double* result = l0.x.p;
    if (result != y) { PNP_CUDA(cudaMemcpyAsync(y, result, n * sizeof(double), cudaMemcpyDeviceToDevice, c.stream)); c.acct(Ctx::ACC_BLAS1, 16.0 * n); }
    return;
  }
  PNP_CUDA(cudaMemcpyAsync(l0.b.p, d, n * sizeof(double), cudaMemcpyDeviceToDevice, c.stream));
  cycle(c, A, 0, nu, A.comp0, true);
  PNP_CUDA(cudaMemcpyAsync(y, l0.x.p, n * sizeof(double), cudaMemcpyDeviceToDevice, c.stream));
}

}
```

### dune_pnp_b200/csrc/pnp_capi.cu

```cuda
#include <cuda_profiler_api.h>

#include <cstring>

#include "pnp_common.cuh"

namespace pnp {
int newton_apply(Ctx&, const Operator&, Vec&, Solver&, const pnp_newton_opts&, pnp_newton_result&);
int amg_graph_state(const Solver&);
LinResult slp_apply(Ctx&, const Operator&, Vec&, Solver&, double, int, double);
int onestep_apply(Ctx&, int, const Operator&, const Operator&, Solver&, double, Vec&, Vec&, Vec&, double, int, double, LinResult*);
namespace {
__global__ void k_fill(double* x, long n, double v) {
  for (long i = blockIdx.x * (long)blockDim.x + threadIdx.x; i < n; i += (long)gridDim.x * blockDim.x) x[i] = v;
}
__global__ void k_pack3(const double* a, const double* b, const double* c, long nv, double* out) {
  for (long i = blockIdx.x * (long)blockDim.x + threadIdx.x; i < nv; i += (long)gridDim.x * blockDim.x) {
    out[3 * i] = a[i]; out[3 * i + 1] = b[i]; out[3 * i + 2] = c[i];
  }
}
__global__ void k_extract(const double* in, long nv, int field, double* out) {
  for (long i = blockIdx.x * (long)blockDim.x + threadIdx.x; i < nv; i += (long)gridDim.x * blockDim.x) out[i] = in[3 * i + field];
}
void to_lin(const LinResult& lr, pnp_lin_result* out) {
  if (!out) return;
  out->converged = lr.converged; out->iterations = lr.iterations; out->reduction = lr.reduction;
  out->conv_rate = lr.conv_rate; out->seconds = lr.seconds; out->status = lr.status;
}
}
}

using namespace pnp;


#define API_BEGIN(ctx)                                  \
  if (!(ctx)) return PNP_E_ARG;                         \
  Ctx& c = (ctx)->c;                                    \
  try {                                                 \
    PNP_CUDA(cudaSetDevice(c.device));
#define API_END                                                      \
    return PNP_OK;                                                   \
  } catch (const pnp::Error& e) { c.err = e.what(); return e.code; } \
  catch (const std::exception& e) { c.err = e.what(); return PNP_E_ARG; }

namespace pnp {
Ctx* ctx_make_owned_child(Ctx& p) {
  pnp_ctx* h = new pnp_ctx;
  h->c.device = p.device; h->c.stream = p.stream; h->c.owns_stream = false; h->c.sm_count = p.sm_count;
  h->c.params = p.params;
  h->c.parent = &p; p.children.push_back(&h->c);
  p.owned_children.push_back(h);
  return &h->c;
}
void ctx_destroy_owned_child(Ctx& p, Ctx* child) {
  for (size_t i = 0; i < p.owned_children.size(); i++) {
    pnp_ctx* h = (pnp_ctx*)p.owned_children[i];
    if (&h->c != child) continue;
    p.owned_children.erase(p.owned_children.begin() + i);
    pnp_ctx_destroy(h);
    return;
  }
}
}

extern "C" {

pnp_status pnp_ctx_create(int device, pnp_ctx** out) {
  if (!out) return PNP_E_ARG;
  *out = nullptr;
  int ndev = 0;
  if (cudaGetDeviceCount(&ndev) != cudaSuccess || device < 0 || device >= ndev) return PNP_E_CUDA;
  pnp_ctx* h = new pnp_ctx;
  h->c.device = device;
  if (cudaSetDevice(device) != cudaSuccess || cudaStreamCreate(&h->c.stream) != cudaSuccess) { delete h; return PNP_E_CUDA; }
  cudaDeviceGetAttribute(&h->c.sm_count, cudaDevAttrMultiProcessorCount, device);
  *out = h;
  return PNP_OK;
}
pnp_status pnp_ctx_create_child(pnp_ctx* parent, pnp_ctx** out) {
  if (!parent || !out) return PNP_E_ARG;
  pnp_ctx* h = new pnp_ctx;
  Ctx& p = parent->c;
  h->c.device = p.device; h->c.stream = p.stream; h->c.owns_stream = false; h->c.sm_count = p.sm_count;
  h->c.rank = p.rank; h->c.world = p.world; h->c.nccl = p.nccl;
  h->c.params = p.params;
  h->c.parent = &p; p.children.push_back(&h->c);
  *out = h;
  return PNP_OK;
}
void pnp_ctx_destroy(pnp_ctx* ctx) {
  if (!ctx) return;
  Ctx& c = ctx->c;
  cudaSetDevice(c.device);
  if (c.parent) {
    Ctx& p = *c.parent;
    for (size_t i = 0; i < p.children.size(); i++) if (p.children[i] == &c) { p.children.erase(p.children.begin() + i); break; }
    for (size_t i = 0; i < p.mg.size(); i++) if (p.mg[i].lc == &c) { p.mg.resize(i); p.mg_gid.release(); p.mg_nglobal = 0; p.mg_replica = nullptr; break; }
    if (p.mg_replica == &c) { p.mg_replica = nullptr; p.mg_gid.release(); p.mg_nglobal = 0; }
    p.mg_epoch++;
  }
  if (c.stream) cudaStreamSynchronize(c.stream);
  c.solvers.clear();
  {
    std::vector<void*> owned;
    owned.swap(c.owned_children);
    for (void* h : owned) pnp_ctx_destroy((pnp_ctx*)h);
  }
  for (Ctx* k : c.children) { k->solvers.clear(); k->parent = nullptr; k->stream = nullptr; k->nccl = nullptr; }
  if (c.h_red) cudaFreeHost(c.h_red);
  for (cudaEvent_t e : c.prof_ev) cudaEventDestroy(e);
  if (c.tm0) cudaEventDestroy(c.tm0);
  if (c.tm1) cudaEventDestroy(c.tm1);
  if (c.owns_comm) comm_destroy(c);
  cudaStream_t s = c.owns_stream ? c.stream : nullptr;
  delete ctx;
  if (s) cudaStreamDestroy(s);
}
pnp_status pnp_mg_push_level(pnp_ctx* ctx, pnp_ctx* child, const int* par0, const int* par1) {
  API_BEGIN(ctx)
  PNP_REQUIRE(c.degree == 1, PNP_E_ARG, "built for linear elements only");
  PNP_REQUIRE(child && par0 && par1, PNP_E_ARG, "null arguments");
  Ctx& f = c.mg.empty() ? c : *c.mg.back().lc;
  Ctx& k = child->c;
  PNP_REQUIRE(f.finalized && k.finalized, PNP_E_ARG, "both levels must be finalized");
  std::vector<int> fi2e = f.int2ext.to_host(c.stream), ke2i = k.ext2int.to_host(c.stream);
  std::vector<int> p0(f.nv), p1(f.nv);
  for (long i = 0; i < f.nv; i++) {
    const int e = fi2e[i];
    PNP_REQUIRE(par0[e] < k.nv && par1[e] < k.nv, PNP_E_ARG, "parent index out of range");
    p0[i] = par0[e] >= 0 ? ke2i[par0[e]] : -1;
    p1[i] = par1[e] >= 0 ? ke2i[par1[e]] : -1;
  }
  MgLevelRef r; r.lc = &k;
  r.par0.alloc(f.nv); r.par1.alloc(f.nv);
  r.par0.upload(p0.data(), f.nv, c.stream); r.par1.upload(p1.data(), f.nv, c.stream);
  PNP_CUDA(cudaStreamSynchronize(c.stream));
  c.mg.push_back(std::move(r));
  c.mg_epoch++;
  API_END
}
pnp_status pnp_mg_set_coarse_aggregates(pnp_ctx* ctx, const int* agg, long n_aggregates) {
  const pnp_status st = pnp_mg_set_coarse_global(ctx, agg, n_aggregates);
  if (st == PNP_OK) ctx->c.mg_aggregated = true;
  return st;
}
pnp_status pnp_mg_set_coarse_global(pnp_ctx* ctx, const int* gid, long n_global) {
  API_BEGIN(ctx)
  c.mg_aggregated = false; c.mg_replica = nullptr;
  PNP_REQUIRE(!c.mg.empty() && gid && n_global > 0, PNP_E_ARG, "no multigrid level pushed");
  Ctx& k = *c.mg.back().lc;
  std::vector<int> i2e = k.int2ext.to_host(c.stream), g(k.nv);
  for (long i = 0; i < k.nv; i++) { g[i] = gid[i2e[i]]; PNP_REQUIRE(g[i] >= 0 && g[i] < n_global, PNP_E_ARG, "global index out of range"); }
  c.mg_gid.alloc(k.nv); c.mg_gid.upload(g.data(), k.nv, c.stream);
  PNP_CUDA(cudaStreamSynchronize(c.stream));
  c.mg_nglobal = n_global; c.mg_epoch++;
  API_END
}
pnp_status pnp_mg_set_coarse_replica(pnp_ctx* ctx, pnp_ctx* replica, const int* gid, long n_global) {
  API_BEGIN(ctx)
  c.mg_aggregated = false; c.mg_replica = nullptr;
  PNP_REQUIRE(!c.mg.empty() && gid && n_global > 0 && replica, PNP_E_ARG, "no multigrid level pushed / null arguments");
  Ctx& k = *c.mg.back().lc;
  Ctx& r = replica->c;
  PNP_REQUIRE(r.finalized && r.n_own == r.nv && r.nv == n_global, PNP_E_ARG, "the replica must hold the whole coarsest mesh, finalized");
  std::vector<int> i2e = k.int2ext.to_host(c.stream), re2i = r.ext2int.to_host(c.stream), g(k.nv);
  for (long i = 0; i < k.nv; i++) {
    const int gi = gid[i2e[i]];
    PNP_REQUIRE(gi >= 0 && gi < n_global, PNP_E_ARG, "global index out of range");
    g[i] = re2i[gi];
  }
  c.mg_gid.alloc(k.nv); c.mg_gid.upload(g.data(), k.nv, c.stream);
  PNP_CUDA(cudaStreamSynchronize(c.stream));
  c.mg_nglobal = n_global; c.mg_replica = &r; c.mg_epoch++;
  API_END
}
pnp_status pnp_profile_spmv(pnp_ctx* ctx, int enable) {
  API_BEGIN(ctx) c.prof = enable != 0; c.prof_used = 0; API_END
}
pnp_status pnp_profile_spmv_get(pnp_ctx* ctx, long* launches, double* total_ms) {
  API_BEGIN(ctx)
  PNP_CUDA(cudaStreamSynchronize(c.stream));
  for (int k = 0; k < 3; k++) { if (launches) launches[k] = 0; if (total_ms) total_ms[k] = 0; }
  for (size_t i = 0; i + 1 < c.prof_used; i += 2) {
    float t = 0; PNP_CUDA(cudaEventElapsedTime(&t, c.prof_ev[i], c.prof_ev[i + 1]));
    const int k = c.prof_kind[i / 2];
    if (launches) launches[k]++;
    if (total_ms) total_ms[k] += t;
  }
  API_END
}
pnp_status pnp_profile_bytes(pnp_ctx* ctx, int reset, double* out6) {
  API_BEGIN(ctx)
  for (int k = 0; k < Ctx::ACC_N; k++) { if (out6) out6[k] = c.alg_bytes[k]; if (reset) c.alg_bytes[k] = 0; }
  API_END
}
pnp_status pnp_profiler_range(pnp_ctx* ctx, int start) {
  API_BEGIN(ctx)
  PNP_CUDA(cudaStreamSynchronize(c.stream));
  if (start) cudaProfilerStart(); else cudaProfilerStop();
  API_END
}
pnp_status pnp_timer_start(pnp_ctx* ctx) {
  API_BEGIN(ctx)
  if (!c.tm0) { PNP_CUDA(cudaEventCreate(&c.tm0)); PNP_CUDA(cudaEventCreate(&c.tm1)); }
  PNP_CUDA(cudaEventRecord(c.tm0, c.stream));
  API_END
}
pnp_status pnp_timer_stop(pnp_ctx* ctx, double* ms) {
  API_BEGIN(ctx)
  PNP_REQUIRE(c.tm0 && ms, PNP_E_ARG, "timer not started");
  PNP_CUDA(cudaEventRecord(c.tm1, c.stream));
  PNP_CUDA(cudaEventSynchronize(c.tm1));
  float t = 0; PNP_CUDA(cudaEventElapsedTime(&t, c.tm0, c.tm1));
  *ms = t;
  API_END
}
pnp_status pnp_tune(const char* name, double value) {
  if (!name) return PNP_E_ARG;
  const std::string n(name);
  Tune& t = tune();
  if (n == "tma") t.tma = value != 0;
  else if (n == "tma_stages") t.tma_stages = (int)value;
  else if (n == "tma_lpr") t.tma_lpr = (int)value;
  else if (n == "graph") t.graph = value != 0;
  else if (n == "fd_warp") t.fd_warp = value != 0;
  else if (n == "jac_compact") t.jac_compact = value != 0;
  else if (n == "p2_chunk") t.p2_chunk = (long)value;
  else if (n == "tma_min_rows") t.tma_min_rows = (long)value;
  else return PNP_E_ARG;
  return PNP_OK;
}
const char* pnp_last_error(pnp_ctx* ctx) { return ctx ? ctx->c.err.c_str() : "null context"; }
long pnp_launch_count(pnp_ctx* ctx) { return ctx ? ctx->c.launches : 0; }

pnp_status pnp_mesh_set(pnp_ctx* ctx, long nv, const double* x, const double* y, long nT, const int* tri, long nB,
                        const int* ba, const int* bb, const int* bphys) {
  API_BEGIN(ctx) mesh_set(c, nv, x, y, nT, tri, nB, ba, bb, bphys, nv); API_END
}
pnp_status pnp_mesh_set_local(pnp_ctx* ctx, long nv, long n_own, const double* x, const double* y, long nT, const int* tri,
                              long nB, const int* ba, const int* bb, const int* bphys) {
  API_BEGIN(ctx) mesh_set(c, nv, x, y, nT, tri, nB, ba, bb, bphys, n_own); API_END
}
pnp_status pnp_comm_unique_id(char* out128) {
  try { comm_unique_id(out128); return PNP_OK; } catch (...) { return PNP_E_CUDA; }
}
pnp_status pnp_comm_init(pnp_ctx* ctx, int rank, int world, const char* unique_id128) {
  API_BEGIN(ctx) comm_init(c, rank, world, unique_id128); API_END
}
pnp_status pnp_comm_init_file(pnp_ctx* ctx, int rank, int world, const char* path) {
  API_BEGIN(ctx)
  PNP_REQUIRE(world == 1 || path, PNP_E_ARG, "null rendezvous path");
  comm_bootstrap_file(c, rank, world, path ? path : "");
  API_END
}
pnp_status pnp_comm_allgatherv(pnp_ctx* ctx, const void* send, long nbytes, void* recv, long cap, long* counts) {
  API_BEGIN(ctx)
  PNP_REQUIRE(nbytes >= 0 && counts && (nbytes == 0 || send), PNP_E_ARG, "bad all-gather arguments");
  std::vector<long> cnt;
  std::vector<unsigned char> all = comm_allgatherv(c, send, nbytes, cnt);
  for (int r = 0; r < c.world; r++) counts[r] = cnt[r];
  if (recv) {
    PNP_REQUIRE((long)all.size() <= cap, PNP_E_ARG, "receive buffer too small");
    std::memcpy(recv, all.data(), all.size());
  }
  API_END
}
pnp_status pnp_halo_set(pnp_ctx* ctx, int n_nbr, const int* nbr, const int* send_ptr, const int* send_idx, const int* recv_ptr) {
  API_BEGIN(ctx) halo_set(c, n_nbr, nbr, send_ptr, send_idx, recv_ptr); API_END
}
pnp_status pnp_halo_exchange(pnp_ctx* ctx, int vec_handle) {
  API_BEGIN(ctx)
  PNP_REQUIRE(c.degree == 1, PNP_E_ARG, "built for linear elements only");
  halo_exchange(c, c.vec(vec_handle).d.p, c.vec(vec_handle).fields);
  PNP_CUDA(cudaStreamSynchronize(c.stream));
  API_END
}
pnp_status pnp_mesh_read_gmsh(pnp_ctx* ctx, const char* path) {
  API_BEGIN(ctx)
  std::vector<double> x, y; std::vector<int> tri, ba, bb, ph;
  read_gmsh_file(path, x, y, tri, ba, bb, ph);
  mesh_set(c, (long)x.size(), x.data(), y.data(), (long)tri.size() / 3, tri.data(), (long)ba.size(), ba.data(), bb.data(),
           ph.data(), (long)x.size());
  API_END
}
pnp_status pnp_mesh_refine(pnp_ctx* ctx, int levels) { API_BEGIN(ctx) mesh_refine(c, levels); API_END }
pnp_status pnp_carry_set(pnp_ctx* ctx, const int* vec_handles, int n) { API_BEGIN(ctx) PNP_REQUIRE(c.degree == 1, PNP_E_ARG, "built for linear elements only"); carry_set(c, vec_handles, n); API_END }
pnp_status pnp_carry_get(pnp_ctx* ctx, int index, int vec_handle) { API_BEGIN(ctx) PNP_REQUIRE(c.degree == 1, PNP_E_ARG, "built for linear elements only"); carry_get(c, index, c.vec(vec_handle)); API_END }
pnp_status pnp_carry_set_host(pnp_ctx* ctx, int fields, const double* host) {
  API_BEGIN(ctx)
  PNP_REQUIRE(c.degree == 1, PNP_E_ARG, "built for linear elements only");
  PNP_REQUIRE(c.nv > 0 && fields >= 1 && host, PNP_E_ARG, "no mesh / bad field count");
  Vec cf; cf.fields = fields; cf.d.alloc((size_t)fields * c.nv);
  cf.d.upload(host, (size_t)fields * c.nv, c.stream);
  PNP_CUDA(cudaStreamSynchronize(c.stream));
  c.carry.clear();
  c.carry.push_back(std::move(cf));
  API_END
}
pnp_status pnp_carry_get_host(pnp_ctx* ctx, int index, double* host) {
  API_BEGIN(ctx)
  PNP_REQUIRE(c.degree == 1, PNP_E_ARG, "built for linear elements only");
  PNP_REQUIRE(index >= 0 && index < (int)c.carry.size() && host, PNP_E_ARG, "no such carried field");
  c.carry[index].d.download(host, c.carry[index].d.n, c.stream);
  API_END
}
pnp_status pnp_mesh_finalize(pnp_ctx* ctx, int renumber) { API_BEGIN(ctx) mesh_finalize(c, renumber != 0); API_END }
pnp_status pnp_mesh_sizes(pnp_ctx* ctx, long* nv, long* nT, long* nB, long* nslots) {
  API_BEGIN(ctx)
  if (nv) *nv = c.nv;
  if (nT) *nT = c.nT; if (nB) *nB = c.nB; if (nslots) *nslots = c.finalized ? c.nslots : 0;
  API_END
}
pnp_status pnp_mesh_get(pnp_ctx* ctx, double* x, double* y, int* tri, int* ba, int* bb, int* bphys) {
  API_BEGIN(ctx)
  if (x) c.cx.download(x, c.nv, c.stream);
  if (y) c.cy.download(y, c.nv, c.stream);
  if (tri) c.ctri.download(tri, 3 * c.nT, c.stream);
  if (ba) c.cba.download(ba, c.nB, c.stream);
  if (bb) c.cbb.download(bb, c.nB, c.stream);
  if (bphys) c.cbphys.download(bphys, c.nB, c.stream);
  API_END
}

pnp_status pnp_params_set(pnp_ctx* ctx, const double* sys, const double* surf) {
  API_BEGIN(ctx)
  PNP_REQUIRE(sys && (sys[0] == 0 || surf), PNP_E_ARG, "null parameter arrays");
  HostParams p;
  p.n_surfaces = (int)sys[0]; p.cylindrical = sys[1] != 0; p.l_b = sys[2]; p.c0 = sys[3]; p.PI = sys[4];
  p.linearSolverIterations = (int)sys[5]; p.newtonReassembleThreshold = sys[6]; p.newtonReduction = sys[7];
  p.newtonMinLinearReduction = sys[8]; p.newtonMaxIterations = sys[9]; p.newtonLineSearchMaxIteration = sys[10];
  p.tau = sys[11]; p.nSteps = (int)sys[12]; p.outputFreq = (int)sys[13]; p.potentialUpdateFreq = (int)sys[14];
  p.verbosity = (int)sys[15];
  PNP_REQUIRE(p.n_surfaces >= 0, PNP_E_CONFIG, "n_surfaces must be non-negative");
  p.surfaces.assign(p.n_surfaces, HostSurface());
  for (int i = 0; i < p.n_surfaces; i++)
    for (int k = 0; k < 3; k++) {
      p.surfaces[i].btype[k] = (int)surf[9 * i + 3 * k];
      p.surfaces[i].flux[k] = surf[9 * i + 3 * k + 1];
      p.surfaces[i].dval[k] = surf[9 * i + 3 * k + 2];
    }
  p.set = true;
  c.params = p;
  c.constraints_built = false;
  if (c.finalized) constraints_build(c);
  API_END
}
pnp_status pnp_params_read(pnp_ctx* ctx, const char* cfg_path) {
  API_BEGIN(ctx)
  read_config_file(cfg_path, c.params);
  c.constraints_built = false;
  if (c.finalized) constraints_build(c);
  API_END
}
pnp_status pnp_params_get(pnp_ctx* ctx, double* sys, double* surf, char* meshfile, int meshfile_cap) {
  API_BEGIN(ctx)
  PNP_REQUIRE(c.params.set, PNP_E_ARG, "parameters not set");
  const HostParams& p = c.params;
  const double v[16] = {(double)p.n_surfaces, (double)p.cylindrical, p.l_b, p.c0, p.PI, (double)p.linearSolverIterations,
                        p.newtonReassembleThreshold, p.newtonReduction, p.newtonMinLinearReduction, p.newtonMaxIterations,
                        p.newtonLineSearchMaxIteration, p.tau, (double)p.nSteps, (double)p.outputFreq,
                        (double)p.potentialUpdateFreq, (double)p.verbosity};
  if (sys) std::memcpy(sys, v, sizeof v);
  if (surf)
    for (int i = 0; i < p.n_surfaces; i++)
      for (int k = 0; k < 3; k++) {
        surf[9 * i + 3 * k] = p.surfaces[i].btype[k];
        surf[9 * i + 3 * k + 1] = p.surfaces[i].flux[k];
        surf[9 * i + 3 * k + 2] = p.surfaces[i].dval[k];
      }
  if (meshfile && meshfile_cap > 0) { std::strncpy(meshfile, p.meshfile.c_str(), meshfile_cap - 1); meshfile[meshfile_cap - 1] = 0; }
  API_END
}
pnp_status pnp_constraints_build(pnp_ctx* ctx) { API_BEGIN(ctx) constraints_build(c); API_END }

pnp_status pnp_operator_create(pnp_ctx* ctx, int op, int comp0, int* handle) {
  API_BEGIN(ctx)
  PNP_REQUIRE(op >= PNP_OP_PB && op <= PNP_OP_PNP && comp0 >= 0 && comp0 < 3 && handle, PNP_E_ARG, "bad operator arguments");
  auto o = std::make_unique<Operator>();
  o->op = op; o->comp0 = comp0;
  c.ops.push_back(std::move(o));
  *handle = (int)c.ops.size() - 1;
  API_END
}
pnp_status pnp_operator_set_coefficient(pnp_ctx* ctx, int h, int which, int vec_handle) {
  API_BEGIN(ctx)
  PNP_REQUIRE(which == 0 || which == 1, PNP_E_ARG, "coefficient index must be 0 or 1");
  c.vec(vec_handle);
  (which == 0 ? c.oper(h).aux0 : c.oper(h).aux1) = vec_handle;
  API_END
}
pnp_status pnp_operator_set_valency(pnp_ctx* ctx, int h, double valency) { API_BEGIN(ctx) c.oper(h).valency = valency; API_END }
pnp_status pnp_constraints_get(pnp_ctx* ctx, int h, char* out) {
  API_BEGIN(ctx)
  PNP_REQUIRE(c.constraints_built, PNP_E_ARG, "constraints not built");
  const Operator& op = c.oper(h);
  if (c.degree >= 2) { p2_constraints_get(c, op, out); return PNP_OK; }
  const int F = op_fields(op.op);
  std::vector<unsigned char> m = c.dmask.to_host(c.stream);
  std::vector<int> i2e = c.int2ext.to_host(c.stream);
  for (long v = 0; v < c.nv; v++)
    for (int k = 0; k < F; k++) out[(long)k * c.nv + i2e[v]] = (char)((m[v] >> (F == 3 ? k : op.comp0)) & 1);
  API_END
}
pnp_status pnp_pattern_get(pnp_ctx* ctx, int h, long* nnz, int* rowptr, int* col) {
  API_BEGIN(ctx)
  long n = pattern_export(c, h, rowptr, col);
  if (nnz) *nnz = n;
  API_END
}

pnp_status pnp_vec_create(pnp_ctx* ctx, int fields, int* handle) {
  API_BEGIN(ctx)
  PNP_REQUIRE(c.finalized, PNP_E_ARG, "mesh not finalized");
  PNP_REQUIRE((fields == 1 || fields == 3) && handle, PNP_E_ARG, "fields must be 1 or 3");
  auto v = std::make_unique<Vec>();
  v->fields = fields; v->d.alloc((size_t)fields * c.cols()); v->d.zero(c.stream);
  c.vecs.push_back(std::move(v));
  *handle = (int)c.vecs.size() - 1;
  API_END
}
pnp_status pnp_vec_destroy(pnp_ctx* ctx, int h) {
  API_BEGIN(ctx)
  if (c.vec(h).d.p == c.last_u) { c.last_u = nullptr; c.last_vals = nullptr; }
  c.vecs[h].reset();
  API_END
}
pnp_status pnp_vec_upload(pnp_ctx* ctx, int h, const double* host) { API_BEGIN(ctx) vec_upload(c, c.vec(h), host); API_END }
pnp_status pnp_vec_download(pnp_ctx* ctx, int h, double* host) { API_BEGIN(ctx) vec_download(c, c.vec(h), host); API_END }
pnp_status pnp_vec_set(pnp_ctx* ctx, int h, double value) {
  API_BEGIN(ctx)
  Vec& v = c.vec(h);
  k_fill<<<grid_for((long)v.d.n, 256), 256, 0, c.stream>>>(v.d.p, (long)v.d.n, value);
  PNP_CHECK_LAUNCH(); c.launches++;
  API_END
}
pnp_status pnp_vec_copy(pnp_ctx* ctx, int dst, int src) {
  API_BEGIN(ctx)
  PNP_REQUIRE(c.vec(dst).d.n == c.vec(src).d.n, PNP_E_ARG, "vector sizes differ");
  vec_copy(c, c.vec(src).d.p, c.vec(dst).d.p, (long)c.vec(src).d.n);
  API_END
}
pnp_status pnp_vec_axpy(pnp_ctx* ctx, int y, double a, int x) {
  API_BEGIN(ctx)
  PNP_REQUIRE(c.vec(y).d.n == c.vec(x).d.n, PNP_E_ARG, "vector sizes differ");
  vec_axpy(c, a, c.vec(x).d.p, c.vec(y).d.p, (long)c.vec(x).d.n);
  API_END
}
pnp_status pnp_vec_norm(pnp_ctx* ctx, int x, double* out) {
  API_BEGIN(ctx) *out = vec_norm(c, c.vec(x).d.p, c.rows() * c.vec(x).fields); API_END
}
pnp_status pnp_vec_dot(pnp_ctx* ctx, int x, int y, double* out) {
  API_BEGIN(ctx)
  PNP_REQUIRE(c.vec(y).d.n == c.vec(x).d.n, PNP_E_ARG, "vector sizes differ");
  *out = vec_dot(c, c.vec(x).d.p, c.vec(y).d.p, c.rows() * c.vec(x).fields);
  API_END
}
pnp_status pnp_vec_pack3(pnp_ctx* ctx, int dst3, int phi, int cp, int cm) {
  API_BEGIN(ctx)
  PNP_REQUIRE(c.vec(dst3).fields == 3 && c.vec(phi).fields == 1 && c.vec(cp).fields == 1 && c.vec(cm).fields == 1,
              PNP_E_ARG, "pack3 needs one 3-field and three 1-field vectors");
  if (c.degree >= 2) {
    const int src[3] = {phi, cp, cm};
    for (int k = 0; k < 3; k++) vec_copy(c, c.vec(src[k]).d.p, c.vec(dst3).d.p + k * c.p2_nd, c.p2_nd);
    return PNP_OK;
  }
  k_pack3<<<grid_for(c.nv, 256), 256, 0, c.stream>>>(c.vec(phi).d.p, c.vec(cp).d.p, c.vec(cm).d.p, c.nv, c.vec(dst3).d.p);
  PNP_CHECK_LAUNCH(); c.launches++;
  API_END
}
pnp_status pnp_vec_extract(pnp_ctx* ctx, int src3, int field, int dst1) {
  API_BEGIN(ctx)
  PNP_REQUIRE(c.vec(src3).fields == 3 && c.vec(dst1).fields == 1 && field >= 0 && field < 3, PNP_E_ARG, "bad extract arguments");
  if (c.degree >= 2) { vec_copy(c, c.vec(src3).d.p + field * c.p2_nd, c.vec(dst1).d.p, c.p2_nd); return PNP_OK; }
  k_extract<<<grid_for(c.nv, 256), 256, 0, c.stream>>>(c.vec(src3).d.p, c.nv, field, c.vec(dst1).d.p);
  PNP_CHECK_LAUNCH(); c.launches++;
  API_END
}

pnp_status pnp_matrix_create(pnp_ctx* ctx, int op_handle, int* handle) {
  API_BEGIN(ctx)
  PNP_REQUIRE(c.finalized && handle, PNP_E_ARG, "mesh not finalized");
  auto m = std::make_unique<Matrix>();
  m->op = c.oper(op_handle).op; m->nplanes = op_planes(m->op);
  if (c.degree >= 2) { PNP_REQUIRE(c.constraints_built, PNP_E_ARG, "constraints not built"); p2_matrix_init(c, *m, c.oper(op_handle)); }
  else { m->vals.alloc((size_t)m->nplanes * c.nslots); m->vals.zero(c.stream); }
  c.mats.push_back(std::move(m));
  *handle = (int)c.mats.size() - 1;
  API_END
}
pnp_status pnp_matrix_destroy(pnp_ctx* ctx, int h) {
  API_BEGIN(ctx)
  if (c.mat(h).vals.p == c.last_vals) c.last_vals = nullptr;
  c.mats[h].reset();
  API_END
}
pnp_status pnp_residual(pnp_ctx* ctx, int op, int u, int r) {
  API_BEGIN(ctx)
  assemble_residual(c, c.oper(op), c.vec(u), c.vec(r));
  PNP_CUDA(cudaStreamSynchronize(c.stream));
  API_END
}
pnp_status pnp_jacobian(pnp_ctx* ctx, int op, int u, int A, int mode, double eps) {
  API_BEGIN(ctx)
  assemble_jacobian(c, c.oper(op), c.vec(u), c.mat(A), mode, eps);
  PNP_CUDA(cudaStreamSynchronize(c.stream));
  API_END
}
pnp_status pnp_matrix_values_get(pnp_ctx* ctx, int op, int A, double* val) {
  API_BEGIN(ctx) matrix_export(c, op, c.mat(A), val); API_END
}
pnp_status pnp_spmv(pnp_ctx* ctx, int A, int x, int y) {
  API_BEGIN(ctx)
  const Matrix& M = c.mat(A);
  PNP_REQUIRE(c.vec(x).fields == (M.nplanes == 1 ? 1 : 3) && c.vec(y).fields == c.vec(x).fields && x != y, PNP_E_ARG,
              "spmv operands do not match the matrix");
  spmv(c, M, c.vec(x).d.p, c.vec(y).d.p);
  PNP_CUDA(cudaStreamSynchronize(c.stream));
  API_END
}

pnp_status pnp_solver_create(pnp_ctx* ctx, int kind, int prec, int maxit, int prec_steps, int verbosity, int* handle) {
  API_BEGIN(ctx)
  PNP_REQUIRE((kind == PNP_SOLVER_BCGS || kind == PNP_SOLVER_CG) && prec >= PNP_PREC_NONE && prec <= PNP_PREC_AMG && handle,
              PNP_E_ARG, "bad solver arguments");
  auto s = std::make_unique<Solver>();
  s->kind = kind; s->prec = prec; s->maxit = maxit; s->prec_steps = prec_steps; s->verbosity = verbosity;
  c.solvers.push_back(std::move(s));
  *handle = (int)c.solvers.size() - 1;
  API_END
}
pnp_status pnp_solver_set_option(pnp_ctx* ctx, int s, const char* name, double value) {
  API_BEGIN(ctx)
  PNP_REQUIRE(name, PNP_E_ARG, "null option name");
// ... 148 lines not shown
```

### dune_pnp_b200/csrc/pnp_common.cuh

```cuda
#pragma once
#include <cuda_runtime.h>

#include <cstdint>
#include <cstdio>
#include <map>
#include <memory>
#include <stdexcept>
#include <string>
#include <vector>

#include "../../include/pnp_b200.h"
#include "pnp_setup_algos.cuh"
#include "pnp_star.cuh"

namespace pnp {

struct Error : std::runtime_error {
  int code;
  Error(int c, const std::string& m) : std::runtime_error(m), code(c) {}
};

#define PNP_CUDA(call)                                                                               \
  do {                                                                                               \
    cudaError_t e_ = (call);                                                                         \
    if (e_ != cudaSuccess)                                                                           \
      throw ::pnp::Error(PNP_E_CUDA, std::string(__FILE__) + ":" + std::to_string(__LINE__) + " " +  \
                                         #call + " -> " + cudaGetErrorString(e_));                   \
  } while (0)
#define PNP_CHECK_LAUNCH() PNP_CUDA(cudaGetLastError())
#define PNP_REQUIRE(cond, code, msg)                                                                 \
  do { if (!(cond)) throw ::pnp::Error(code, std::string(msg)); } while (0)

template <class T> struct DBuf {
  T* p = nullptr;
  size_t n = 0;
  DBuf() = default;
  explicit DBuf(size_t n_) { alloc(n_); }
  DBuf(const DBuf&) = delete;
  DBuf& operator=(const DBuf&) = delete;
  DBuf(DBuf&& o) noexcept : p(o.p), n(o.n) { o.p = nullptr; o.n = 0; }
  DBuf& operator=(DBuf&& o) noexcept { if (this != &o) { release(); p = o.p; n = o.n; o.p = nullptr; o.n = 0; } return *this; }
  ~DBuf() { release(); }
  void release() { if (p) cudaFree(p); p = nullptr; n = 0; }
  void alloc(size_t n_) {
    release();
    n = n_;
    if (n) PNP_CUDA(cudaMalloc(&p, n * sizeof(T) + 64));
  }
  void zero(cudaStream_t s) { if (n) PNP_CUDA(cudaMemsetAsync(p, 0, n * sizeof(T), s)); }
  void upload(const T* h, size_t cnt, cudaStream_t s) {
    if (cnt) PNP_CUDA(cudaMemcpyAsync(p, h, cnt * sizeof(T), cudaMemcpyHostToDevice, s));
  }
  void download(T* h, size_t cnt, cudaStream_t s) const {
    if (cnt) PNP_CUDA(cudaMemcpyAsync(h, p, cnt * sizeof(T), cudaMemcpyDeviceToHost, s));
    PNP_CUDA(cudaStreamSynchronize(s));
  }
  std::vector<T> to_host(cudaStream_t s) const { std::vector<T> h(n); download(h.data(), n, s); return h; }
};

struct Tune {
  int tma = 1;
  int tma_stages = 2;
  int tma_lpr = 2;
  long tma_min_rows = -1;
  int graph = 1;
  int fd_warp = 1;
  int jac_compact = 1;
  long p2_chunk = 0;
};
inline Tune& tune() { static Tune t; return t; }

inline int grid_for(long n, int block, int max_blocks = 148 * 32) {
  long g = (n + block - 1) / block;
  if (g < 1) g = 1;
  return (int)(g > max_blocks ? max_blocks : g);
}

struct HostSurface { int btype[3] = {1, 1, 1}; double flux[3] = {0, 0, 0}; double dval[3] = {0, 0, 0}; };
struct HostParams {
  bool set = false;
  int n_surfaces = 0, verbosity = 0, cylindrical = 0;
  double l_b = 1, c0 = 0.06, PI = 3.1415;
  int linearSolverIterations = 50;
  double newtonReassembleThreshold = 0, newtonReduction = 1e-5, newtonMinLinearReduction = 1e-5;
  double newtonMaxIterations = 50, newtonLineSearchMaxIteration = 500, tau = 0.1;
  int nSteps = 100, outputFreq = 1, potentialUpdateFreq = 1;
  std::string meshfile;
  std::vector<HostSurface> surfaces;
};

struct Vec {
  int fields = 1;
  DBuf<double> d;
};
struct Matrix {
  int op = 0;
  int nplanes = 1;
  int comp0 = 0;
  DBuf<double> vals;
  const int* csr_rp = nullptr; const int* csr_col = nullptr; long csr_nnz = 0, csr_n = 0;
  void* csr_pattern = nullptr;
};

struct Operator {
  int op = OP_PB;
  int comp0 = 0;
  double valency = 1.0;
  int aux0 = -1, aux1 = -1;
  int intorder = 0;
};

struct HierLevel {
  long nv = 0, nslots = 0, nE = 0;
  DBuf<int> rp, int2ext, ext2int;
  DBuf<unsigned> adj;
  DBuf<uint64_t> edges;
};

struct Ctx;
struct MgLevelRef {
  Ctx* lc = nullptr;
  DBuf<int> par0, par1;
};

struct Amg;
struct P2Space;
struct SweepPrec;
struct SweepPlan;

struct Solver {
  int kind = PNP_SOLVER_BCGS, prec = PNP_PREC_NONE, maxit = 5000, prec_steps = 1, verbosity = 0;
  std::shared_ptr<Amg> amg;
  std::shared_ptr<SweepPrec> sweep;
  std::map<std::string, double> opts;
  double opt(const char* name, double dflt) const { auto it = opts.find(name); return it == opts.end() ? dflt : it->second; }
  DBuf<double> w[6];
  DBuf<double> dinv;
  DBuf<double> csr_lu; int csr_levels = 0;
  std::shared_ptr<void> pmg;
  void ensure(size_t n) { for (auto& b : w) if (b.n != n) b.alloc(n); if (dinv.n != n) dinv.alloc(n); }
};

struct Ctx {
  int device = 0;
  cudaStream_t stream = nullptr;
  std::string err;
  int sm_count = 148;
  long nv = 0, nT = 0, nB = 0;
  long n_own = 0;
  int degree = 1; long p2_nd = 0;
  std::shared_ptr<P2Space> p2;
  long rows() const { return degree >= 2 ? p2_nd : n_own; }
  long cols() const { return degree >= 2 ? p2_nd : nv; }
  int rank = 0, world = 1;
  void* nccl = nullptr;
  std::vector<int> halo_nbr, halo_send_ptr, halo_recv_ptr;
  std::vector<int> halo_send_ext;
  DBuf<int> halo_send_idx;
  DBuf<double> halo_send_buf;
  DBuf<double> cx, cy;
  DBuf<int> ctri, cba, cbb, cbphys;
  bool finalized = false;
  long nslots = 0;
  DBuf<int> rp;
  DBuf<unsigned> adj;
  DBuf<XY> xy;
  DBuf<unsigned char> dmask;
  DBuf<int> int2ext, ext2int;
  std::vector<BFace> bfaces;
  DBuf<BFace> d_bfaces;
  DBuf<int> d_bv, d_bv_ptr, d_bv_items;
  int n_bv = 0;
  DBuf<double> d_surf;
  DBuf<unsigned char> d_surf_dir;
  HostParams params;
  bool constraints_built = false;
  long launches = 0;
  enum { ACC_SPMV_FINE = 0, ACC_SPMV_COARSE = 1, ACC_ASSEMBLY = 2, ACC_BLAS1 = 3, ACC_TRANSFER = 4, ACC_DENSE = 5, ACC_N = 6 };
  double alg_bytes[ACC_N] = {0, 0, 0, 0, 0, 0};
  void acct(int cls, double bytes) { alg_bytes[cls] += bytes; }
  void absorb(Ctx& child) {
    launches += child.launches; child.launches = 0;
    for (int k = 0; k < ACC_N; k++) { alg_bytes[k] += child.alg_bytes[k]; child.alg_bytes[k] = 0; }
  }
  bool prof = false;
  std::vector<cudaEvent_t> prof_ev;
  std::vector<int> prof_kind;
  size_t prof_used = 0;
  cudaEvent_t tm0 = nullptr, tm1 = nullptr;
  void prof_mark(int kind = 0) {
    if (!prof) return;
    if (prof_used == prof_ev.size()) { cudaEvent_t e; cudaEventCreate(&e); prof_ev.push_back(e); }
    if (prof_used % 2 == 0) { if (prof_kind.size() <= prof_used / 2) prof_kind.resize(prof_used / 2 + 1); prof_kind[prof_used / 2] = kind; }
    cudaEventRecord(prof_ev[prof_used++], stream);
  }
  std::vector<std::unique_ptr<Vec>> vecs;
  std::vector<std::unique_ptr<Matrix>> mats;
  std::vector<std::unique_ptr<Operator>> ops;
  std::vector<std::unique_ptr<Solver>> solvers;
  Vec ws_r, ws_z, ws_prev;
  Matrix ws_A;
  Vec ws_stage[6];
  Matrix ws_B;
  DBuf<double> io_stage;
  bool owns_stream = true;
  std::vector<MgLevelRef> mg;
  DBuf<int> mg_gid; long mg_nglobal = 0; bool mg_aggregated = false;
  Ctx* mg_replica = nullptr;
  long mg_epoch = 0;
  Ctx* parent = nullptr;
  std::vector<Ctx*> children;
  std::vector<void*> owned_children;
  bool owns_comm = false;
  const double* last_u = nullptr; Operator last_op; int last_mode = 0; double last_eps = 1e-11;
  const double* last_vals = nullptr;
  std::vector<HierLevel> hier;
  std::vector<Vec> carry;
  void invalidate_mesh_objects() {
    finalized = false; constraints_built = false; p2.reset(); p2_nd = 0;
    vecs.clear(); mats.clear(); ops.clear(); solvers.clear();
    last_u = nullptr; last_vals = nullptr;
    ws_r.d.release(); ws_z.d.release(); ws_prev.d.release(); ws_A.vals.release(); ws_B.vals.release();
    for (auto& v : ws_stage) v.d.release();
    io_stage.release();
  }
  DBuf<double> red_partial, red_out;
  double* h_red = nullptr;

  StarView star() const { return StarView{rp.p, adj.p, xy.p, dmask.p, (int)n_own}; }
  PhysParams phys(double valency) const {
    PhysParams P; P.PI = params.PI; P.l_b = params.l_b; P.c0 = params.c0; P.valency = valency;
    P.cylindrical = params.cylindrical; return P;
  }
  Vec& vec(int h) { PNP_REQUIRE(h >= 0 && h < (int)vecs.size() && vecs[h], PNP_E_ARG, "bad vector handle"); return *vecs[h]; }
  Matrix& mat(int h) { PNP_REQUIRE(h >= 0 && h < (int)mats.size() && mats[h], PNP_E_ARG, "bad matrix handle"); return *mats[h]; }
  Operator& oper(int h) { PNP_REQUIRE(h >= 0 && h < (int)ops.size() && ops[h], PNP_E_ARG, "bad operator handle"); return *ops[h]; }
  Solver& solver(int h) { PNP_REQUIRE(h >= 0 && h < (int)solvers.size() && solvers[h], PNP_E_ARG, "bad solver handle"); return *solvers[h]; }
};

inline int op_fields(int op) { return op == OP_PNP ? 3 : 1; }
inline int op_planes(int op) { return op == OP_PNP ? 7 : 1; }

void mesh_set(Ctx&, long nv, const double* x, const double* y, long nT, const int* tri, long nB, const int* ba,
              const int* bb, const int* bphys, long n_own);
void mesh_refine(Ctx&, int levels);
void mesh_finalize(Ctx&, bool renumber);
void constraints_build(Ctx&);
void comm_init(Ctx&, int rank, int world, const char* unique_id128);
void comm_unique_id(char* out128);
void comm_destroy(Ctx&);
void comm_bootstrap_file(Ctx&, int rank, int world, const std::string& path);
std::vector<unsigned char> comm_allgatherv(Ctx&, const void* send, long nbytes, std::vector<long>& counts);
void halo_set(Ctx&, int n_nbr, const int* nbr, const int* send_ptr, const int* send_idx, const int* recv_ptr);
void halo_finalize(Ctx&);
void halo_exchange(Ctx&, double* x, int fields);
void allreduce_sum(Ctx&, double* dev, size_t n);
void allreduce_max_u64(Ctx&, unsigned long long* dev, size_t n);
void carry_set(Ctx&, const int* handles, int n);
void carry_get(Ctx&, int i, Vec& out);
void vec_upload(Ctx&, Vec&, const double* host_lex);
void vec_download(Ctx&, const Vec&, double* host_lex);
void vec_from_lex_device(Ctx&, Vec&, const double* d_lex);
void vec_to_lex_device(Ctx&, const Vec&, double* d_lex);
Ctx* ctx_make_owned_child(Ctx& parent);
void ctx_destroy_owned_child(Ctx& parent, Ctx* child);
long pattern_export(Ctx&, int op_handle, int* rowptr, int* col);
void matrix_export(Ctx&, int op_handle, const Matrix&, double* val);
void matrix_import(Ctx&, int op_handle, Matrix&, const int* rowptr, const int* col, const double* val);
void mesh_renumber(Ctx&, const int* new_index);
void read_gmsh_file(const std::string& path, std::vector<double>& x, std::vector<double>& y, std::vector<int>& tri,
                    std::vector<int>& ba, std::vector<int>& bb, std::vector<int>& bphys);
void read_config_file(const std::string& path, HostParams& p);
void interpolate_bcext(Ctx&, int comp, const Vec* pb, Vec& out);
void assemble_residual(Ctx&, const Operator&, Vec& u, Vec& r);
void assemble_jacobian(Ctx&, const Operator&, Vec& u, Matrix& A, int mode, double eps);
void assemble_jacobian_on(Ctx&, const StarView& M, long stride, const Operator&, const double* u, double* vals, int nplanes,
                          int mode, double eps);
void spmv(Ctx&, const Matrix& A, double* x, double* y);
double vec_norm(Ctx&, const double* x, long n);
double vec_dot(Ctx&, const double* x, const double* y, long n);
void vec_axpy(Ctx&, double a, const double* x, double* y, long n);
void vec_copy(Ctx&, const double* x, double* y, long n);
void vec_zero(Ctx&, double* x, long n);
struct LinResult { bool converged = false; int iterations = 0; double reduction = 1, conv_rate = 1; int status = 0; double seconds = 0; };
LinResult solver_apply(Ctx&, Solver&, const Matrix& A, Vec& z, Vec& r, double reduction);
void precond_apply(Ctx&, Solver&, const Matrix& A, Vec& d, Vec& v);
int sweep_levels(const Solver&, bool ilu);
void p2_build(Ctx&);
void p2_constraints(Ctx&);
void p2_matrix_init(Ctx&, Matrix&, const Operator&);
void p2_assemble_residual(Ctx&, const Operator&, Vec& u, Vec& r);
void p2_assemble_jacobian(Ctx&, const Operator&, Vec& u, Matrix& A, int mode, double eps);
void csr_spmv(Ctx&, const Matrix& A, const double* x, double* y);
void csr_diag_inverse(Ctx&, const Matrix& A, double* dinv);
void csr_sweep_setup(Ctx&, Solver&, const Matrix& A, bool ilu);
void csr_ssor_apply(Ctx&, Solver&, const Matrix& A, const double* d, double* y);
void csr_ilu0_apply(Ctx&, Solver&, const Matrix& A, const double* d, double* y);
void pmg_setup(Ctx&, Solver&, const Matrix& A);
void pmg_apply(Ctx&, Solver&, const Matrix& A, const double* d, double* y);
const unsigned char* p2_dirichlet_flags(Ctx&);
void p2_sizes(Ctx&, long* nE, long* nd);
void p2_offsets(Ctx&, long* eoff, long* voff);
void p2_edges(Ctx&, int* eva, int* evb);
void p2_constraints_get(Ctx&, const Operator&, char* out);
long p2_pattern_export(Ctx&, const Operator&, int* rowptr, int* col);
void p2_matrix_import(Ctx&, const Operator&, Matrix&, const int* rowptr, const int* col, const double* val);
void p2_interpolate_bcext(Ctx&, int comp, const Vec* pb, Vec& out);
void p2_ion_flux(Ctx&, const Vec& phi, const Vec& cp, const Vec& cm, double* ip, double* im);
void p2_write_cell_data(Ctx&, const Vec& u, const std::string& filename);
void p2_vertex_values(Ctx&, const Vec& u, double* out);
void ion_flux(Ctx&, const Vec& phi, const Vec& cp, const Vec& cm, double* ip, double* im);
void write_cell_data(Ctx&, const Vec& u, const std::string& filename);
void write_vtk(Ctx&, const std::string& name, int nfields, const Vec* const* fields, const char* const* names, int ascii);

}

struct pnp_ctx { pnp::Ctx c; };
```

### dune_pnp_b200/csrc/pnp_spmv_tma.cuh

```cuda
#pragma once
#include "pnp_spmv.cuh"

namespace pnp {

constexpr int TMA_TR = 128;
constexpr int tma_nw(int lpr) { return TMA_TR * lpr / 32; }
constexpr int tma_producers(int np, int epi, int ndot) { return np + 3 + ((epi != EPI_PLAIN || ndot >= 1) ? 1 : 0); }
constexpr int tma_threads(int np, int epi, int ndot, int lpr) { return (tma_nw(lpr) + tma_producers(np, epi, ndot)) * 32; }
constexpr int TMA_CAP = 960;
constexpr int TMA_MAX_STAGES = 3;
constexpr int TMA_W = 128;

template <int NP> struct TmaLayout {
  static constexpr int F = NP == 1 ? 1 : 3;
  static constexpr int PLANE = (TMA_CAP + 2) * 8;
  static constexpr int COLS = NP * PLANE;
  static constexpr int RP = COLS + (TMA_CAP + 4) * 4;
  static constexpr int B = RP + (TMA_TR + 4) * 4;
  static constexpr int XW = B + (F * TMA_TR + 2) * 8;
  static constexpr int STAGE = XW + (F * (TMA_TR + 2 * TMA_W) + 2) * 8;
  static constexpr int YBUF = TMA_TR * F * 8;
  static constexpr int HEAD = 128;
  static_assert(PLANE % 16 == 0 && COLS % 16 == 0 && RP % 16 == 0 && B % 16 == 0 && XW % 16 == 0 && STAGE % 16 == 0, "bulk copy alignment");
  static constexpr int smem_bytes(int stages) { return HEAD + stages * STAGE + YBUF; }
};

__device__ __forceinline__ unsigned smem_u32(const void* p) { return (unsigned)__cvta_generic_to_shared(p); }
__device__ __forceinline__ void mbar_init(uint64_t* bar, unsigned count) {
  asm volatile("mbarrier.init.shared::cta.b64 [%0], %1;" ::"r"(smem_u32(bar)), "r"(count) : "memory");
}
__device__ __forceinline__ void mbar_expect_tx(uint64_t* bar, unsigned bytes) {
  asm volatile("mbarrier.arrive.expect_tx.shared::cta.b64 _, [%0], %1;" ::"r"(smem_u32(bar)), "r"(bytes) : "memory");
}
__device__ __forceinline__ void mbar_arrive(uint64_t* bar) {
  asm volatile("mbarrier.arrive.shared::cta.b64 _, [%0];" ::"r"(smem_u32(bar)) : "memory");
}
__device__ __forceinline__ void mbar_wait(uint64_t* bar, unsigned parity) {
  unsigned done;
  do {
    asm volatile("{\n .reg .pred p;\n mbarrier.try_wait.parity.shared::cta.b64 p, [%1], %2;\n selp.u32 %0, 1, 0, p;\n}"
                 : "=r"(done) : "r"(smem_u32(bar)), "r"(parity) : "memory");
  } while (!done);
}
__device__ __forceinline__ void bulk_g2s(void* dst, const void* src, unsigned bytes, uint64_t* bar) {
  asm volatile("cp.async.bulk.shared::cluster.global.mbarrier::complete_tx::bytes [%0], [%1], %2, [%3];"
               ::"r"(smem_u32(dst)), "l"(src), "r"(bytes), "r"(smem_u32(bar)) : "memory");
}

template <int NP>
__device__ __forceinline__ void block_inverse_row(const double* dv, int k, double* o) {
  const PnpBlock B = pnp_block<NP>(dv);
  const double a = B.a, b = B.b, c_ = B.c, d = B.d, e = B.e, f = B.f, g = B.g;
  const double det = a * e * g - b * d * g - c_ * e * f;
  const double scale = fabs(a * e * g) + fabs(b * d * g) + fabs(c_ * e * f);
  if (fabs(det) > 1e-12 * scale && scale > 0.0) {
    const double id = 1.0 / det;
    if (k == 0) { o[0] = e * g * id; o[1] = -b * g * id; o[2] = -c_ * e * id; }
    else if (k == 1) { o[0] = -d * g * id; o[1] = (a * g - c_ * f) * id; o[2] = c_ * d * id; }
    else { o[0] = -e * f * id; o[1] = b * f * id; o[2] = (a * e - b * d) * id; }
  } else {
    const double dd = k == 0 ? a : (k == 1 ? e : g);
    const double inv = dd != 0.0 ? 1.0 / dd : 0.0;
    o[0] = k == 0 ? inv : 0.0; o[1] = k == 1 ? inv : 0.0; o[2] = k == 2 ? inv : 0.0;
  }
}

template <int NP, bool STAGED>
__device__ __forceinline__ void slot_product(const StarOpArgs& a, bool ok, int s, const double* sv, const int* vb, const unsigned* sc,
                                             int cbase, const double* sx, int wlo, unsigned wn, double* acc, double* dg) {
  constexpr int F = NP == 1 ? 1 : 3;
  const unsigned c = !ok ? 0u : ((STAGED ? sc[s - cbase] : a.col[s]) & STAR_VMASK);
  const unsigned cw = c - (unsigned)wlo;
  const bool in = cw < wn;
  double x[F], v[NP];
#pragma unroll
  for (int k = 0; k < F; k++) x[k] = !ok ? 0.0 : (in ? sx[F * cw + k] : a.x[(size_t)F * c + k]);
#pragma unroll
  for (int p = 0; p < NP; p++) v[p] = !ok ? 0.0 : (STAGED ? sv[vb[p] + s] : a.vals[(size_t)p * a.stride + s]);
  if (dg) {
#pragma unroll
    for (int p = 0; p < NP; p++) dg[p] = v[p];
  }
  if constexpr (NP == 1) acc[0] += v[0] * x[0];
  else block_mac<NP>(v, x, acc);
}

template <int NP, int EPI, int NDOT, int LPR>
__global__ void __launch_bounds__(tma_threads(NP, EPI, NDOT, LPR), 1) k_star_op_tma(const StarOpArgs a, const int nstages) {
  using L = TmaLayout<NP>;
  constexpr int F = L::F;
  constexpr int TMA_NW = tma_nw(LPR);
  constexpr int RW = 32 / LPR;
  extern __shared__ __align__(128) unsigned char smem[];
  uint64_t* full = reinterpret_cast<uint64_t*>(smem);
  uint64_t* empty = full + TMA_MAX_STAGES;
  unsigned char* stages = smem + L::HEAD;
  double* ybuf = reinterpret_cast<double*>(stages + (size_t)nstages * L::STAGE);
  const int warp = threadIdx.x >> 5, lane = threadIdx.x & 31;
  const int ntiles = (a.nv + TMA_TR - 1) / TMA_TR;
  const int sp = (int)(a.stride & 1);
  if (threadIdx.x == 0) {
    for (int s = 0; s < nstages; s++) { mbar_init(&full[s], tma_producers(NP, EPI, NDOT)); mbar_init(&empty[s], TMA_NW); }
    asm volatile("fence.mbarrier_init.release.cluster;" ::: "memory");
  }
  __syncthreads();
  double dsum[NDOT > 0 ? NDOT : 1];
#pragma unroll
  for (int j = 0; j < (NDOT > 0 ? NDOT : 1); j++) dsum[j] = 0.0;

  if (warp >= TMA_NW) {
    const int role = warp - TMA_NW;
    auto load_batch = [&](int batch, int& lo, int& hi) {
      const long tt = blockIdx.x + (long)(batch * 32 + lane) * gridDim.x;
      lo = 0; hi = 0;
      if (tt < ntiles) { lo = a.rp[tt * TMA_TR]; hi = a.rp[min((int)tt * TMA_TR + TMA_TR, a.nv)]; }
    };
    int cur_lo, cur_hi, nxt_lo, nxt_hi;
    load_batch(0, cur_lo, cur_hi);
    load_batch(1, nxt_lo, nxt_hi);
    int t = blockIdx.x;
    for (int it = 0; t < ntiles; t += gridDim.x, it++) {
      if (it > 0 && (it & 31) == 0) { cur_lo = nxt_lo; cur_hi = nxt_hi; load_batch(it / 32 + 1, nxt_lo, nxt_hi); }
      const int lo = __shfl_sync(0xffffffffu, cur_lo, it & 31), hi = __shfl_sync(0xffffffffu, cur_hi, it & 31);
      if (lane == 0) {
        const int stage = it % nstages;
        const unsigned parity = (unsigned)((it / nstages) & 1);
        mbar_wait(&empty[stage], parity ^ 1u);
        unsigned char* st = stages + (size_t)stage * L::STAGE;
        const int r0 = t * TMA_TR, rows = min(TMA_TR, a.nv - r0);
        const bool staged = hi - lo <= TMA_CAP;
        const void* src = nullptr; void* dst = nullptr; unsigned nb = 0;
        if (role < NP) {
          if (staged) {
            const int o = (lo + role * sp) & 1;
            nb = (unsigned)(((hi - lo + o) + 1) & ~1) * 8u;
            src = a.vals + (size_t)role * a.stride + (lo - o); dst = st + role * L::PLANE;
          }
        } else if (role == NP) {
          if (staged) {
            const int lo_c = lo & ~3;
            nb = (unsigned)(((hi - lo_c) + 3) & ~3) * 4u;
            src = a.col + lo_c; dst = st + L::COLS;
          }
        } else if (role == NP + 1) {
          nb = (unsigned)((rows + 1 + 3) & ~3) * 4u;
          src = a.rp + r0; dst = st + L::RP;
        } else if (role == NP + 2) {
          const int wlo = max(r0 - TMA_W, 0), whi = min(r0 + TMA_TR + TMA_W, a.nv);
          nb = (unsigned)((F * (whi - wlo) + 1) & ~1) * 8u;
          src = a.x + (size_t)F * wlo; dst = st + L::XW;
        } else {
          nb = (unsigned)((F * rows + 1) & ~1) * 8u;
          src = (EPI == EPI_PLAIN ? a.w1 : a.b) + (size_t)F * r0; dst = st + L::B;
        }
        if (nb) { mbar_expect_tx(&full[stage], nb); bulk_g2s(dst, src, nb, &full[stage]); }
        else mbar_arrive(&full[stage]);
      }
      __syncwarp();
    }
  } else {
    const int sub = lane % LPR;
    double* yw = ybuf + warp * RW * F;
    int t = blockIdx.x;
    for (int it = 0; t < ntiles; t += gridDim.x, it++) {
      const int stage = it % nstages;
      const unsigned parity = (unsigned)((it / nstages) & 1);
      mbar_wait(&full[stage], parity);
      const unsigned char* st = stages + (size_t)stage * L::STAGE;
      const double* sv = reinterpret_cast<const double*>(st);
      const unsigned* sc = reinterpret_cast<const unsigned*>(st + L::COLS);
      const int* srp = reinterpret_cast<const int*>(st + L::RP);
      const double* sb = reinterpret_cast<const double*>(st + L::B);
      const double* sx = reinterpret_cast<const double*>(st + L::XW);
      const int r0 = t * TMA_TR, rows = min(TMA_TR, a.nv - r0);
      const int wlo = max(r0 - TMA_W, 0);
      const unsigned wn = (unsigned)(min(r0 + TMA_TR + TMA_W, a.nv) - wlo);
      const double* sxo = sx + (size_t)F * (r0 - wlo);
      const int lo = srp[0], hi = srp[rows];
      const bool staged = hi - lo <= TMA_CAP;
      const int cbase = lo & ~3;
      int vb[NP];
#pragma unroll
      for (int p = 0; p < NP; p++) vb[p] = p * (TMA_CAP + 2) - lo + ((lo + p * sp) & 1);
      const int rl = RW * warp + lane / LPR;
      const bool valid = rl < rows;
      const int b0 = valid ? srp[rl] : hi, e0 = valid ? srp[rl + 1] : hi;
      double acc[F], dg[NP];
#pragma unroll
      for (int k = 0; k < F; k++) acc[k] = 0.0;
#pragma unroll
      for (int p = 0; p < NP; p++) dg[p] = 0.0;
      const int len = e0 - b0;
      const int maxlen = __reduce_max_sync(0xffffffffu, len);
      if (staged) {
        constexpr int MAXS = (8 + LPR - 1) / LPR;
        unsigned cj[MAXS];
        bool okj[MAXS];
        double xj[MAXS][F];
#pragma unroll
        for (int u = 0; u < MAXS; u++) {
          const int j = sub + u * LPR;
          okj[u] = j < len;
          cj[u] = okj[u] ? (sc[b0 + j - cbase] & STAR_VMASK) : 0u;
        }
#pragma unroll
        for (int u = 0; u < MAXS; u++) {
          const unsigned cw = cj[u] - (unsigned)wlo;
          const bool in = cw < wn;
          const bool ldg = okj[u] && !in, lds = okj[u] && in;
#pragma unroll
          for (int k = 0; k < F; k++) {
            double xg = 0.0, xs = 0.0;
            if (ldg) xg = a.x[(size_t)F * cj[u] + k];
            if (lds) xs = sx[F * cw + k];
            xj[u][k] = in ? xs : xg;
          }
        }
#pragma unroll
        for (int u = 0; u < MAXS; u++) {
          const int s = b0 + sub + u * LPR;
          double v[NP];
#pragma unroll
          for (int p = 0; p < NP; p++) v[p] = okj[u] ? sv[vb[p] + s] : 0.0;
          if (EPI == EPI_JACOBI && u == 0) {
#pragma unroll
            for (int p = 0; p < NP; p++) dg[p] = v[p];
          }
          if constexpr (NP == 1) acc[0] += v[0] * xj[u][0];
          else block_mac<NP>(v, xj[u], acc);
        }
        for (int j = sub + MAXS * LPR; j < maxlen; j += LPR)
          slot_product<NP, true>(a, j < len, b0 + j, sv, vb, sc, cbase, sx, wlo, wn, acc, nullptr);
      } else {
        slot_product<NP, false>(a, sub < len, b0 + sub, sv, vb, sc, cbase, sx, wlo, wn, acc, EPI == EPI_JACOBI ? dg : nullptr);
        for (int j = sub + LPR; j < maxlen; j += LPR)
          slot_product<NP, false>(a, j < len, b0 + j, sv, vb, sc, cbase, sx, wlo, wn, acc, nullptr);
      }
      if (LPR > 1) {
#pragma unroll
        for (int k = 0; k < F; k++)
#pragma unroll
          for (int o = LPR / 2; o > 0; o >>= 1) acc[k] += __shfl_xor_sync(0xffffffffu, acc[k], o);
      }
      const bool mine = valid && sub == 0;
      double yv[F];
#pragma unroll
      for (int k = 0; k < F; k++) yv[k] = 0.0;
      if (mine) {
        if (EPI == EPI_PLAIN) {
#pragma unroll
          for (int k = 0; k < F; k++) {
            yv[k] = acc[k];
            if (NDOT >= 1) dsum[0] += acc[k] * sb[F * rl + k];
            if (NDOT >= 2) dsum[NDOT >= 2 ? 1 : 0] += acc[k] * acc[k];
          }
        } else if (EPI == EPI_RESIDUAL) {
#pragma unroll
          for (int k = 0; k < F; k++) yv[k] = sb[F * rl + k] - acc[k];
        } else {
          double r[F], z[F];
#pragma unroll
          for (int k = 0; k < F; k++) r[k] = sb[F * rl + k] - acc[k];
          if constexpr (F == 3) {
#pragma unroll
            for (int k = 0; k < F; k++) {
              double o[3];
              block_inverse_row<NP>(dg, k, o);
              z[k] = o[0] * r[0] + o[1] * r[1] + o[2] * r[2];
            }
          } else z[0] = (dg[0] != 0.0 ? 1.0 / dg[0] : 0.0) * r[0];
#pragma unroll
          for (int k = 0; k < F; k++) yv[k] = sxo[F * rl + k] + a.omega * z[k];
        }
      }
      if (sub == 0) {
#pragma unroll
        for (int k = 0; k < F; k++) yw[F * (lane / LPR) + k] = yv[k];
      }
      __syncwarp();
      {
        const size_t g0 = (size_t)F * (r0 + RW * warp);
        const size_t gend = (size_t)F * a.nv;
#pragma unroll
        for (int i = lane; i < RW * F; i += 32)
          if (g0 + i < gend) a.y[g0 + i] = yw[i];
      }
      __syncwarp();
      if (lane == 0) mbar_arrive(&empty[stage]);
    }
  }
  if (NDOT > 0) {
    __shared__ double sm[NDOT > 0 ? NDOT : 1][TMA_NW];
#pragma unroll
    for (int j = 0; j < (NDOT > 0 ? NDOT : 1); j++) {
      double s = dsum[j];
#pragma unroll
      for (int o = 16; o > 0; o >>= 1) s += __shfl_xor_sync(0xffffffffu, s, o);
      if (lane == 0 && warp < TMA_NW) sm[j][warp] = s;
    }
    __syncthreads();
    if (warp == 0) {
#pragma unroll
      for (int j = 0; j < (NDOT > 0 ? NDOT : 1); j++) {
        double s = lane < TMA_NW ? sm[j][lane] : 0.0;
#pragma unroll
        for (int o = 16; o > 0; o >>= 1) s += __shfl_xor_sync(0xffffffffu, s, o);
        if (lane == 0) a.partial[(long)blockIdx.x * NDOT + j] = s;
      }
    }
  }
}

inline bool star_op_tma_ok(const Ctx& c, const StarOpArgs& a, int epi) {
  const Tune& t = tune();
  if (!t.tma || epi == EPI_CHEBYSHEV) return false;
  if ((long)a.nv < (t.tma_min_rows >= 0 ? t.tma_min_rows : 2l * TMA_TR * c.sm_count)) return false;
  auto al = [](const void* p) { return (reinterpret_cast<uintptr_t>(p) & 15u) == 0; };
  return al(a.rp) && al(a.col) && al(a.vals) && al(a.x) && (!a.b || al(a.b)) && (!a.w1 || al(a.w1));
}

inline int star_op_tma_stages() {
  const int v = tune().tma_stages;
  return v < 2 ? 2 : (v > TMA_MAX_STAGES ? TMA_MAX_STAGES : v);
}

template <int NP, int EPI, int NDOT, int LPR>
inline int launch_star_op_tma_lpr(Ctx& c, const StarOpArgs& a) {
  using L = TmaLayout<NP>;
  const int nstages = star_op_tma_stages();
  const int smem = L::smem_bytes(nstages);
  static unsigned long long configured = 0;
  if (!(configured >> (c.device & 63) & 1ull)) {
    PNP_CUDA(cudaFuncSetAttribute(k_star_op_tma<NP, EPI, NDOT, LPR>, cudaFuncAttributeMaxDynamicSharedMemorySize, L::smem_bytes(TMA_MAX_STAGES)));
    configured |= 1ull << (c.device & 63);
  }
  const int ntiles = (a.nv + TMA_TR - 1) / TMA_TR;
  const int grid = ntiles < c.sm_count ? ntiles : c.sm_count;
  k_star_op_tma<NP, EPI, NDOT, LPR><<<grid, tma_threads(NP, EPI, NDOT, LPR), smem, c.stream>>>(a, nstages);
  PNP_CHECK_LAUNCH(); c.launches++;
  return grid;
}
template <int NP, int EPI, int NDOT>
inline int launch_star_op_tma_inst(Ctx& c, const StarOpArgs& a) {
  return tune().tma_lpr == 2 ? launch_star_op_tma_lpr<NP, EPI, NDOT, 2>(c, a) : launch_star_op_tma_lpr<NP, EPI, NDOT, 1>(c, a);
}

template <int EPI, int NDOT>
inline double star_op_bytes(int nplanes, const StarOpArgs& a) {
  const double F = nplanes == 1 ? 1 : 3, nv = a.nv, ns = a.rp ? (double)a.stride : 0.0;
  double b = (8.0 * nplanes + 4.0) * ns + (4.0 + 16.0 * F) * nv;
  if (EPI != EPI_PLAIN) b += 8.0 * F * nv;
  if (EPI == EPI_PLAIN && NDOT >= 1) b += 8.0 * F * nv;
  if (EPI == EPI_CHEBYSHEV) b += 16.0 * F * nv;
  return b;
}
template <int EPI, int NDOT>
inline int launch_star_op_auto(Ctx& c, int nplanes, const StarOpArgs& a, bool fine = true) {
  c.acct(fine ? Ctx::ACC_SPMV_FINE : Ctx::ACC_SPMV_COARSE, star_op_bytes<EPI, NDOT>(nplanes, a));
  if (EPI != EPI_CHEBYSHEV && star_op_tma_ok(c, a, EPI)) {
    constexpr int E = EPI == EPI_CHEBYSHEV ? EPI_PLAIN : EPI;
    return nplanes == 1 ? launch_star_op_tma_inst<1, E, NDOT>(c, a)
         : nplanes == PNP_COMPACT_PLANES ? launch_star_op_tma_inst<PNP_COMPACT_PLANES, E, NDOT>(c, a)
                                         : launch_star_op_tma_inst<7, E, NDOT>(c, a);
  }
  return launch_star_op<EPI, NDOT>(c, nplanes, a);
}

}
```

### include/pnp_b200.h

```cpp
#ifndef PNP_B200_H
#define PNP_B200_H

#ifdef __cplusplus
extern "C" {
#endif

typedef struct pnp_ctx pnp_ctx;
typedef int pnp_status;

enum {
  PNP_OK = 0,
  PNP_E_NOT_CONVERGED = 1,
  PNP_E_LINEAR_SOLVER = 2,
  PNP_E_LINE_SEARCH = 3,
  PNP_E_NAN = 4,
  PNP_E_BREAKDOWN = 5,
  PNP_E_CUDA = 6,
  PNP_E_CONFIG = 7,
  PNP_E_ARG = 8,
  PNP_E_MESH = 9
};

enum { PNP_OP_PB = 0, PNP_OP_POISSON = 1, PNP_OP_DIFFUSION = 2, PNP_OP_MASS = 3, PNP_OP_PNP = 4 };
enum { PNP_JAC_FD_FAITHFUL = 0, PNP_JAC_ANALYTIC = 1 };
enum { PNP_SOLVER_BCGS = 0, PNP_SOLVER_CG = 1 };
enum { PNP_PREC_NONE = 0, PNP_PREC_JACOBI = 1, PNP_PREC_SSOR = 2, PNP_PREC_ILU0 = 3, PNP_PREC_AMG = 4 };

pnp_status pnp_ctx_create(int device, pnp_ctx** out);
void pnp_ctx_destroy(pnp_ctx* ctx);
const char* pnp_last_error(pnp_ctx* ctx);
pnp_status pnp_tune(const char* name, double value);
long pnp_launch_count(pnp_ctx* ctx);

pnp_status pnp_profile_spmv(pnp_ctx*, int enable);
pnp_status pnp_profile_spmv_get(pnp_ctx*, long* launches, double* total_ms);
pnp_status pnp_profile_bytes(pnp_ctx*, int reset, double* out6);
pnp_status pnp_profiler_range(pnp_ctx*, int start);
pnp_status pnp_timer_start(pnp_ctx*);
pnp_status pnp_timer_stop(pnp_ctx*, double* elapsed_ms);

pnp_status pnp_mesh_set(pnp_ctx*, long nv, const double* x, const double* y, long nT, const int* tri ,
                        long nB, const int* ba, const int* bb, const int* bphys);
pnp_status pnp_mesh_read_gmsh(pnp_ctx*, const char* path);
pnp_status pnp_mesh_set_local(pnp_ctx*, long nv, long n_own, const double* x, const double* y, long nT, const int* tri,
                              long nB, const int* ba, const int* bb, const int* bphys);
pnp_status pnp_mesh_owned(pnp_ctx*, long* n_own);
pnp_status pnp_comm_unique_id(char* out128);
pnp_status pnp_comm_init(pnp_ctx*, int rank, int world, const char* unique_id128);
pnp_status pnp_comm_init_file(pnp_ctx*, int rank, int world, const char* path);
pnp_status pnp_comm_allgatherv(pnp_ctx*, const void* send, long nbytes, void* recv, long cap, long* counts);
pnp_status pnp_halo_set(pnp_ctx*, int n_nbr, const int* nbr, const int* send_ptr, const int* send_idx, const int* recv_ptr);
pnp_status pnp_halo_exchange(pnp_ctx*, int vec_handle);
pnp_status pnp_ctx_create_child(pnp_ctx* parent, pnp_ctx** child);
pnp_status pnp_mg_push_level(pnp_ctx*, pnp_ctx* child, const int* par0, const int* par1);
pnp_status pnp_mg_set_coarse_global(pnp_ctx*, const int* global_vertex_index, long n_global);
pnp_status pnp_mg_set_coarse_aggregates(pnp_ctx*, const int* aggregate, long n_aggregates);
pnp_status pnp_mg_set_coarse_replica(pnp_ctx*, pnp_ctx* replica, const int* global_vertex_index, long n_global);
typedef struct pnp_part pnp_part;
pnp_status pnp_part_create(long nv, const double* x, const double* y, long nT, const int* tri, long nB, const int* ba,
                           const int* bb, const int* bphys, int world, int rank, int levels, pnp_part** out);
void pnp_part_destroy(pnp_part*);
const char* pnp_part_last_error(pnp_part*);
pnp_status pnp_part_ghost_keys(pnp_part*, int level, long* n, unsigned long long* keys );
pnp_status pnp_part_claim(pnp_part*, int level, const long* ghost_ptr , const unsigned long long* ghost_keys_all,
                          long* claim_ptr , long* claim_pos );
pnp_status pnp_part_finalize(pnp_part*, int level, const long* mine_ptr , const long* mine_pos);
pnp_status pnp_part_sizes(pnp_part*, int level, long* sizes);
pnp_status pnp_part_get(pnp_part*, int level, double* x, double* y, int* tri, int* ba, int* bb, int* bphys, int* nbr,
                        int* send_ptr, int* send_idx, int* recv_ptr, int* par0, int* par1, int* gid);
pnp_status pnp_partition_build(pnp_ctx* root, int levels, int replica_level, int field_level, int nfields, long nf,
                               const double* fx, const double* fy, const double* fields, int* start_vec);
pnp_status pnp_mesh_refine(pnp_ctx*, int levels);
pnp_status pnp_carry_set(pnp_ctx*, const int* vec_handles, int n);
pnp_status pnp_carry_get(pnp_ctx*, int index, int vec_handle);
pnp_status pnp_carry_set_host(pnp_ctx*, int fields, const double* host);
pnp_status pnp_carry_get_host(pnp_ctx*, int index, double* host);
pnp_status pnp_mesh_renumber(pnp_ctx*, const int* new_index);
pnp_status pnp_mesh_finalize(pnp_ctx*, int renumber);
pnp_status pnp_mesh_sizes(pnp_ctx*, long* nv, long* nT, long* nB, long* nslots);
pnp_status pnp_mesh_get(pnp_ctx*, double* x, double* y, int* tri, int* ba, int* bb, int* bphys);

pnp_status pnp_params_set(pnp_ctx*, const double* sys, const double* surf);
pnp_status pnp_params_read(pnp_ctx*, const char* cfg_path);
pnp_status pnp_params_get(pnp_ctx*, double* sys, double* surf , char* meshfile, int meshfile_cap);
pnp_status pnp_constraints_build(pnp_ctx*);

pnp_status pnp_operator_create(pnp_ctx*, int op, int comp0, int* op_handle);
pnp_status pnp_operator_set_coefficient(pnp_ctx*, int op_handle, int which, int vec_handle);
pnp_status pnp_operator_set_valency(pnp_ctx*, int op_handle, double valency);
pnp_status pnp_constraints_get(pnp_ctx*, int op_handle, char* is_dirichlet);
pnp_status pnp_pattern_get(pnp_ctx*, int op_handle, long* nnz, int* rowptr, int* col);

pnp_status pnp_vec_create(pnp_ctx*, int fields, int* vec_handle);
pnp_status pnp_vec_destroy(pnp_ctx*, int vec_handle);
pnp_status pnp_vec_upload(pnp_ctx*, int vec_handle, const double* host);
pnp_status pnp_vec_download(pnp_ctx*, int vec_handle, double* host);
pnp_status pnp_vec_set(pnp_ctx*, int vec_handle, double value);
pnp_status pnp_vec_copy(pnp_ctx*, int dst, int src);
pnp_status pnp_vec_axpy(pnp_ctx*, int y, double a, int x);
pnp_status pnp_vec_norm(pnp_ctx*, int x, double* two_norm);
pnp_status pnp_vec_dot(pnp_ctx*, int x, int y, double* result);

pnp_status pnp_matrix_create(pnp_ctx*, int op_handle, int* mat_handle);
pnp_status pnp_matrix_destroy(pnp_ctx*, int mat_handle);
pnp_status pnp_residual(pnp_ctx*, int op_handle, int u, int r);
pnp_status pnp_jacobian(pnp_ctx*, int op_handle, int u, int mat_handle, int mode, double fd_epsilon);
pnp_status pnp_matrix_values_get(pnp_ctx*, int op_handle, int mat_handle, double* val);
pnp_status pnp_spmv(pnp_ctx*, int mat_handle, int x, int y);
pnp_status pnp_matrix_set_csr(pnp_ctx*, int op_handle, int mat_handle, const int* rowptr, const int* col, const double* val);

typedef struct {
  int converged;
  int iterations;
  double reduction;
  double conv_rate;
  double seconds;
  int status;
} pnp_lin_result;
pnp_status pnp_solver_create(pnp_ctx*, int kind, int prec, int maxit, int prec_steps, int verbosity, int* solver);
pnp_status pnp_solver_set_option(pnp_ctx*, int solver, const char* name, double value);
pnp_status pnp_solver_get(pnp_ctx*, int solver, const char* name, double* value);
pnp_status pnp_precond_apply(pnp_ctx*, int solver, int mat_handle, int d, int v);
pnp_status pnp_solver_apply(pnp_ctx*, int solver, int mat_handle, int z, int r, double reduction, pnp_lin_result*);

enum { PNP_LS_HACKBUSCH_REUSKEN_ACCEPT_BEST = 0, PNP_LS_NONE = 1, PNP_LS_HACKBUSCH_REUSKEN = 2 };
typedef struct {
  double reduction;
  double abs_limit;
  double min_linear_reduction;
  double reassemble_threshold;
  int max_iterations;
  int line_search_max_iterations;
  double damping;
  int jac_mode;
  double fd_epsilon;
  int verbosity;
  int line_search_strategy;
} pnp_newton_opts;
typedef struct {
  int converged;
  int iterations;
  double first_defect, defect, reduction;
  int linear_iterations, line_search_trials, jacobian_assemblies, residual_assemblies;
  double seconds_assembly, seconds_solve, seconds_total;
  int n_history;
  double defect_history[64];
  int linear_iterations_history[64];
} pnp_newton_result;
void pnp_newton_opts_default(pnp_newton_opts*);
pnp_status pnp_newton_opts_from_params(pnp_ctx*, pnp_newton_opts*);
pnp_status pnp_newton_apply(pnp_ctx*, int op_handle, int u, int solver, const pnp_newton_opts*, pnp_newton_result*);
pnp_status pnp_slp_apply(pnp_ctx*, int op_handle, int u, int solver, double reduction, int jac_mode, double fd_epsilon,
                         pnp_lin_result*);

enum { PNP_TIME_ALEXANDER2 = 0, PNP_TIME_IMPLICIT_EULER = 1 };
pnp_status pnp_onestep_apply(pnp_ctx*, int method, int op_space, int op_time, int solver, double time, double dt, int x_old,
                             int dirichlet_values, int x_new, double reduction, int jac_mode, double fd_epsilon,
                             pnp_lin_result* stage_results);

pnp_status pnp_ion_flux(pnp_ctx*, int phi, int cp, int cm, double* ip, double* im);
pnp_status pnp_write_cell_data(pnp_ctx*, int vec_handle, const char* filename);

pnp_status pnp_write_vtk(pnp_ctx*, const char* name, int n, const int* vec_handles, const char* const* names, int ascii);

pnp_status pnp_interpolate_bcext(pnp_ctx*, int component, int pb_vec, int out_vec);

pnp_status pnp_space_set_degree(pnp_ctx*, int degree);
pnp_status pnp_space_sizes(pnp_ctx*, int* degree, long* n_edges, long* ndof);
pnp_status pnp_space_edges(pnp_ctx*, int* va , int* vb);
pnp_status pnp_space_offsets(pnp_ctx*, long* edge_offset, long* vertex_offset);
pnp_status pnp_operator_set_intorder(pnp_ctx*, int op_handle, int intorder);
pnp_status pnp_vec_pack3(pnp_ctx*, int dst3, int phi, int cp, int cm);
pnp_status pnp_vec_extract(pnp_ctx*, int src3, int field, int dst1);

#ifdef __cplusplus
}
#endif
#endif
```

Measured before the change: 448.8 million.

## Fuse pairs of Jacobi smoothing sweeps into one block-local TMA kernel with halo

Adds a fused 'star pair' kernel that does two damped-Jacobi sweeps (or one sweep plus the residual) per launch. Each block keeps its first-sweep result for its own rows and a recomputed halo in shared memory, so the second pass reads x locally through 16-bit local column indices. A per-level fuse plan (halo rows, local columns, copied halo matrix values) is built at setup and its values refreshed at each numeric setup. The aim is to halve the launches and global x/matrix traffic of the multigrid smoother, at the cost of redundant halo computation, extra setup sorts and higher shared-memory use. It is on by default through the new mg_fuse tune flag.

```diff
diff --git a/dune_pnp_b200/capi.py b/dune_pnp_b200/capi.py
--- a/dune_pnp_b200/capi.py
+++ b/dune_pnp_b200/capi.py
@@ -140,6 +140,21 @@
         self._ck(lib().pnp_timer_stop(self._h, C.byref(ms)))
         return ms.value
 
+    def fuse_plan(self, rows_per_block, arrays=True):
+        sz = (C.c_long * 4)()
+        self._ck(lib().pnp_fuse_plan_get(self._h, int(rows_per_block), sz, None, None, None, None, None))
+        nv, ns, nh, hmax = list(sz)
+        out = dict(nv=nv, nslots=ns, nhalo=nh, hmax=hmax)
+        if arrays:
+            nb = (nv + rows_per_block - 1) // rows_per_block
+            rp = np.zeros(nv + 1, dtype=np.int32); col = np.zeros(ns, dtype=np.int32)
+            hptr = np.zeros(nb + 1, dtype=np.int32); hrows = np.zeros(max(nh, 1), dtype=np.int32)
+            lcol = np.zeros(ns, dtype=np.uint16)
+            self._ck(lib().pnp_fuse_plan_get(self._h, int(rows_per_block), sz, _i(rp), _i(col), _i(hptr), _i(hrows),
+                                             lcol.ctypes.data_as(C.c_void_p)))
+            out.update(rowptr=rp, col=col, hptr=hptr, hrows=hrows[:nh], lcol=lcol)
+        return out
+
     def launch_count(self):
         return lib().pnp_launch_count(self._h)
 
diff --git a/dune_pnp_b200/csrc/pnp_amg.cu b/dune_pnp_b200/csrc/pnp_amg.cu
--- a/dune_pnp_b200/csrc/pnp_amg.cu
+++ b/dune_pnp_b200/csrc/pnp_amg.cu
@@ -36,6 +36,7 @@
   bool redisc = false;
   DBuf<XY> xy_own; DBuf<unsigned char> dmask_own;
   std::shared_ptr<SweepPlan> gs_plan;
+  FusePlan fuse;
 };
 
 }
@@ -162,6 +163,52 @@
     out[I] = lo;
   }
 }
+__global__ void k_halo_keys(const int* __restrict__ rp, const unsigned* __restrict__ col, int nv, int T, uint64_t* __restrict__ keys) {
+  for (int v = blockIdx.x * blockDim.x + threadIdx.x; v < nv; v += gridDim.x * blockDim.x) {
+    const unsigned blk = (unsigned)(v / T);
+    for (int s = rp[v]; s < rp[v + 1]; s++) {
+      const unsigned w = col[s] & STAR_VMASK;
+      keys[s] = (w < (unsigned)nv && w / (unsigned)T != blk) ? ((uint64_t)blk << 32 | w) : ~0ull;
+    }
+  }
+}
+__global__ void k_halo_rows(const uint64_t* __restrict__ ukeys, long n, int* __restrict__ hrows) {
+  for (long i = blockIdx.x * (long)blockDim.x + threadIdx.x; i < n; i += (long)gridDim.x * blockDim.x) hrows[i] = (int)(ukeys[i] & 0xffffffffu);
+}
+__global__ void k_local_cols(const int* __restrict__ rp, const unsigned* __restrict__ col, int nv, int T, const int* __restrict__ hptr,
+                             const int* __restrict__ hrows, unsigned short* __restrict__ lcol) {
+  for (int v = blockIdx.x * blockDim.x + threadIdx.x; v < nv; v += gridDim.x * blockDim.x) {
+    const int blk = v / T, h0 = hptr[blk], h1 = hptr[blk + 1];
+    for (int s = rp[v]; s < rp[v + 1]; s++) {
+      const int w = (int)(col[s] & STAR_VMASK);
+      if (w / T == blk) { lcol[s] = (unsigned short)(w - blk * T); continue; }
+      int lo = h0, hi = h1;
+      while (lo < hi) { const int mid = (lo + hi) >> 1; if (hrows[mid] < w) lo = mid + 1; else hi = mid; }
+      lcol[s] = (unsigned short)(T + lo - h0);
+    }
+  }
+}
+__global__ void k_halo_lens(const int* __restrict__ rp, const int* __restrict__ hrows, int nh, int* __restrict__ len) {
+  for (int i = blockIdx.x * blockDim.x + threadIdx.x; i <= nh; i += gridDim.x * blockDim.x)
+    len[i] = i < nh ? rp[hrows[i] + 1] - rp[hrows[i]] : 0;
+}
+__global__ void k_halo_cols(const int* __restrict__ rp, const unsigned* __restrict__ col, const int* __restrict__ hrows, int nh,
+                            const int* __restrict__ hrp, unsigned* __restrict__ hcol) {
+  for (int i = blockIdx.x * blockDim.x + threadIdx.x; i < nh; i += gridDim.x * blockDim.x) {
+    const int s0 = rp[hrows[i]], n = hrp[i + 1] - hrp[i];
+    for (int k = 0; k < n; k++) hcol[hrp[i] + k] = col[s0 + k];
+  }
+}
+template <int NP>
+__global__ void k_halo_vals(const int* __restrict__ rp, const double* __restrict__ vals, long stride, const int* __restrict__ hrows,
+                            int nh, const int* __restrict__ hrp, long hns, double* __restrict__ hvals) {
+  for (int i = blockIdx.x * blockDim.x + threadIdx.x; i < nh; i += gridDim.x * blockDim.x) {
+    const int s0 = rp[hrows[i]], n = hrp[i + 1] - hrp[i];
+    for (int k = 0; k < n; k++)
+#pragma unroll
+      for (int p = 0; p < NP; p++) hvals[p * hns + hrp[i] + k] = vals[p * stride + s0 + k];
+  }
+}
 __global__ void k_iota(int* a, int n) {
   for (int i = blockIdx.x * blockDim.x + threadIdx.x; i < n; i += gridDim.x * blockDim.x) a[i] = i;
 }
@@ -450,6 +497,22 @@
   if (A.distributed) halo_exchange(*l.lc, const_cast<double*>(x), A.F);
   if (fine) c.prof_mark(EPI == EPI_RESIDUAL ? 1 : 2);
   launch_star_op_auto<EPI, 0>(c, A.NP, a, fine);
+  if (fine) c.prof_mark();
+}
+
+bool fuse_on(const Ctx& c, const Amg& A, const Level& l) {
+  if (A.distributed || A.smoother != 0) return false;
+  StarOpArgs a{l.rp, l.col, l.vals, l.nslots, l.nv, l.x.p, l.x2.p};
+  a.b = l.b.p;
+  return star_pair_ok(c, a, l.fuse, A.NP);
+}
+template <int SS>
+void level_pair(Ctx& c, const Amg& A, Level& l) {
+  StarOpArgs a{l.rp, l.col, l.vals, l.nslots, l.nv, l.x.p, l.x2.p};
+  a.b = l.b.p; a.omega = A.omega;
+  const bool fine = &l == A.L[0].get();
+  if (fine) c.prof_mark(SS ? 2 : 1);
+  launch_star_pair<SS>(c, A.NP, a, l.fuse, l.r.p, fine);
   if (fine) c.prof_mark();
 }
 
@@ -708,6 +771,7 @@
     Level& l = *A.L[li];
     if (li + 1 < A.L.size()) uf = level_values(c, A, (int)li, uf, comp0);
     level_dinv(c, A, l);
+    if (l.fuse.T) fuse_plan_values(c, l.fuse, l.rp, l.vals, l.nslots, A.NP);
     c.acct(Ctx::ACC_ASSEMBLY, (4.0 + 8.0 * A.NP + (A.F == 3 ? 72.0 : 8.0)) * l.nv);
   }
   A.dense_n = 0;
@@ -876,9 +940,14 @@
   const long n = (long)A.F * l.nv;
   if (steps <= 0) { if (zero) PNP_CUDA(cudaMemsetAsync(l.x.p, 0, n * sizeof(double), c.stream)); return; }
   if (A.smoother == 0) {
+    const bool fuse = fuse_on(c, A, l);
     int s = 0;
     if (zero) { jacobi0(c, A, l, A.omega, nullptr); s = 1; }
-    for (; s < steps; s++) { level_op<2>(c, A, l, l.x.p, l.b.p, l.x2.p); std::swap(l.x.p, l.x2.p); }
+    while (s < steps) {
+      if (fuse && steps - s >= 2) { level_pair<1>(c, A, l); s += 2; }
+      else { level_op<2>(c, A, l, l.x.p, l.b.p, l.x2.p); s++; }
+      std::swap(l.x.p, l.x2.p);
+    }
     return;
   }
   if (A.smoother == 2) {
@@ -977,10 +1046,12 @@
     return;
   }
   const int nu_pre = A.pre_steps >= 0 ? A.pre_steps : nu, nu_post = A.post_steps >= 0 ? A.post_steps : nu;
-  smooth(c, A, l, coarsest ? A.coarse_sweeps : nu_pre, zero);
+  const bool pair_r = !coarsest && nu_pre >= 2 && fuse_on(c, A, l);
+  smooth(c, A, l, coarsest ? A.coarse_sweeps : nu_pre - (pair_r ? 1 : 0), zero);
   if (coarsest) return;
   Level& nx = *A.L[li + 1];
-  level_op<1>(c, A, l, l.x.p, l.b.p, l.r.p);
+  if (pair_r) { level_pair<0>(c, A, l); std::swap(l.x.p, l.x2.p); }
+  else level_op<1>(c, A, l, l.x.p, l.b.p, l.r.p);
   if (A.distributed) halo_exchange(*l.lc, l.r.p, A.F);
   if (A.F == 1) KL(c, k_restrict<1>, nx.nv, l.agg_ptr.p, l.agg_mem.p, l.par1.p, nx.nv, l.r.p, nx.b.p);
   else KL(c, k_restrict<3>, nx.nv, l.agg_ptr.p, l.agg_mem.p, l.par1.p, nx.nv, l.r.p, nx.b.p);
@@ -1003,6 +1074,67 @@
   smooth(c, A, l, nu_post, false);
 }
 
+}
+
+void fuse_plan_build(Ctx& c, const int* rp, const unsigned* col, int nv, long nslots, int T, FusePlan& P) {
+  PNP_REQUIRE(T > 0 && T % TMA_TR == 0 && nv > 0, PNP_E_ARG, "fused smoothing: rows per block must be a positive multiple of 128");
+  PNP_REQUIRE(nslots < (1l << 31), PNP_E_MESH, "fused smoothing: too many matrix slots on one level");
+  const int nb = (nv + T - 1) / T;
+  const int ns = (int)nslots;
+  DBuf<uint64_t> keys(ns), skeys(ns);
+  DBuf<int> d_nu(1);
+  DBuf<unsigned char> tmp;
+  size_t bytes = 0;
+  KL(c, k_halo_keys, nv, rp, col, nv, T, keys.p);
+  cub::DeviceRadixSort::SortKeys(nullptr, bytes, keys.p, skeys.p, ns, 0, 64, c.stream);
+  tmp.alloc(bytes);
+  PNP_CUDA(cub::DeviceRadixSort::SortKeys(tmp.p, bytes, keys.p, skeys.p, ns, 0, 64, c.stream));
+  cub::DeviceSelect::Unique(nullptr, bytes, skeys.p, keys.p, d_nu.p, ns, c.stream);
+  if (bytes > tmp.n) tmp.alloc(bytes);
+  PNP_CUDA(cub::DeviceSelect::Unique(tmp.p, bytes, skeys.p, keys.p, d_nu.p, ns, c.stream));
+  int nu = 0;
+  d_nu.download(&nu, 1, c.stream);
+  if (nu > 0) {
+    uint64_t last = 0;
+    PNP_CUDA(cudaMemcpyAsync(&last, keys.p + (nu - 1), sizeof last, cudaMemcpyDeviceToHost, c.stream));
+    PNP_CUDA(cudaStreamSynchronize(c.stream));
+    if (last == ~0ull) nu--;
+  }
+  P.T = T; P.nblocks = nb;
+  P.hptr.alloc((size_t)nb + 1); P.hrows.alloc(nu); P.lcol.alloc(ns);
+  KL(c, k_row_starts, nb + 1, keys.p, (long)nu, nb, P.hptr.p);
+  if (nu) KL(c, k_halo_rows, nu, keys.p, (long)nu, P.hrows.p);
+  KL(c, k_local_cols, nv, rp, col, nv, T, P.hptr.p, P.hrows.p, P.lcol.p);
+  {
+    DBuf<int> len((size_t)nu + 1);
+    KL(c, k_halo_lens, nu + 1, rp, P.hrows.p, nu, len.p);
+    P.hrp.alloc((size_t)nu + 1);
+    cub::DeviceScan::ExclusiveSum(nullptr, bytes, len.p, P.hrp.p, nu + 1, c.stream);
+    if (bytes > tmp.n) tmp.alloc(bytes);
+    PNP_CUDA(cub::DeviceScan::ExclusiveSum(tmp.p, bytes, len.p, P.hrp.p, nu + 1, c.stream));
+    int hns = 0;
+    PNP_CUDA(cudaMemcpyAsync(&hns, P.hrp.p + nu, sizeof hns, cudaMemcpyDeviceToHost, c.stream));
+    PNP_CUDA(cudaStreamSynchronize(c.stream));
+    P.hns = hns;
+    P.hcol.alloc((size_t)hns);
+    if (nu) KL(c, k_halo_cols, nu, rp, col, P.hrows.p, nu, P.hrp.p, P.hcol.p);
+    P.hvals.release();
+  }
+  c.launches += 3;
+  const std::vector<int> hp = P.hptr.to_host(c.stream);
+  P.hmax = 0;
+  for (int b = 0; b < nb; b++) P.hmax = std::max(P.hmax, hp[b + 1] - hp[b]);
+  PNP_REQUIRE(T + P.hmax < 65536, PNP_E_MESH, "fused smoothing: block and halo rows exceed the 16-bit local column index");
+}
+
+void fuse_plan_values(Ctx& c, FusePlan& P, const int* rp, const double* vals, long stride, int nplanes) {
+  const int nh = (int)P.hrows.n;
+  if (P.hvals.n != (size_t)nplanes * P.hns) P.hvals.alloc((size_t)nplanes * P.hns);
+  if (!nh) return;
+  if (nplanes == 1) KL(c, k_halo_vals<1>, nh, rp, vals, stride, P.hrows.p, nh, P.hrp.p, P.hns, P.hvals.p);
+  else if (nplanes == PNP_COMPACT_PLANES) KL(c, k_halo_vals<PNP_COMPACT_PLANES>, nh, rp, vals, stride, P.hrows.p, nh, P.hrp.p, P.hns, P.hvals.p);
+  else KL(c, k_halo_vals<7>, nh, rp, vals, stride, P.hrows.p, nh, P.hrp.p, P.hns, P.hvals.p);
+  c.acct(Ctx::ACC_ASSEMBLY, (16.0 * nplanes + 4.0) * (double)P.hns + 12.0 * nh);
 }
 
 int amg_graph_state(const Solver& S) { return !S.amg ? 0 : (S.amg->cg_exec ? 1 : (S.amg->cg_failed ? -1 : 0)); }
@@ -1054,6 +1186,10 @@
       level_values(c, A, li, nullptr, comp0);
     }
     for (auto& l : A.L) alloc_work(c, A, *l);
+    if (!A.distributed && tune().mg_fuse && tune().tma)
+      for (auto& l : A.L)
+        if (l->nv >= (tune().tma_min_rows >= 0 ? tune().tma_min_rows : 2l * FUSE_T * c.sm_count))
+          fuse_plan_build(c, l->rp, l->col, l->nv, l->nslots, FUSE_T, l->fuse);
     if (!A.distributed) {
       Level& l0r = *A.L[0];
       const size_t nall = (size_t)A.F * c.nv;
@@ -1094,13 +1230,18 @@
   const int nu = S.prec_steps > 0 ? S.prec_steps : 1;
   if (c.n_own == c.nv) {
     double *keep_b = l0.b.p, *keep_x = l0.x.p, *keep_x2 = l0.x2.p;
-    const int pre = A.pre_steps >= 0 ? A.pre_steps : nu, post = A.post_steps >= 0 ? A.post_steps : nu;
-    const int swaps = A.smoother == 2 ? 0 : (pre > 0 ? pre - 1 : 0) + post;
     struct Restore {
       Level& l; double *b, *x, *x2;
       ~Restore() { l.b.p = b; l.x.p = x; l.x2.p = x2; }
     } restore{l0, keep_b, keep_x, keep_x2};
     l0.b.p = const_cast<double*>(d);
+    const int pre = A.pre_steps >= 0 ? A.pre_steps : nu, post = A.post_steps >= 0 ? A.post_steps : nu;
+    const bool fuse = fuse_on(c, A, l0), pair_r = fuse && pre >= 2 && A.L.size() > 1;
+    auto launches = [&](int steps, bool zero) {
+      const int m = steps <= 0 ? 0 : steps - (zero ? 1 : 0);
+      return fuse ? m / 2 + m % 2 : m;
+    };
+    const int swaps = A.smoother == 2 ? 0 : launches(pre - (pair_r ? 1 : 0), true) + (pair_r ? 1 : 0) + launches(post, false);
     if (swaps & 1) l0.x2.p = y; else l0.x.p = y;
     cycle(c, A, 0, nu, A.comp0, true);
     double* result = l0.x.p;
diff --git a/dune_pnp_b200/csrc/pnp_capi.cu b/dune_pnp_b200/csrc/pnp_capi.cu
--- a/dune_pnp_b200/csrc/pnp_capi.cu
+++ b/dune_pnp_b200/csrc/pnp_capi.cu
@@ -3,6 +3,7 @@
 #include <cstring>
 
 #include "pnp_common.cuh"
+#include "pnp_spmv_tma.cuh"
 
 namespace pnp {
 int newton_apply(Ctx&, const Operator&, Vec&, Solver&, const pnp_newton_opts&, pnp_newton_result&);
@@ -226,8 +227,27 @@
   else if (n == "jac_compact") t.jac_compact = value != 0;
   else if (n == "p2_chunk") t.p2_chunk = (long)value;
   else if (n == "tma_min_rows") t.tma_min_rows = (long)value;
+  else if (n == "mg_fuse") t.mg_fuse = value != 0;
   else return PNP_E_ARG;
   return PNP_OK;
+}
+pnp_status pnp_fuse_plan_get(pnp_ctx* ctx, int rows_per_block, long* sizes, int* rowptr, int* col, int* hptr, int* hrows,
+                             unsigned short* lcol) {
+  API_BEGIN(ctx)
+  PNP_REQUIRE(c.finalized && c.n_own == c.nv && sizes, PNP_E_ARG, "fuse plan: needs a finalized one-GPU mesh");
+  FusePlan P;
+  fuse_plan_build(c, c.rp.p, c.adj.p, (int)c.nv, c.nslots, rows_per_block, P);
+  sizes[0] = c.nv; sizes[1] = c.nslots; sizes[2] = (long)P.hrows.n; sizes[3] = P.hmax;
+  if (rowptr) c.rp.download(rowptr, c.nv + 1, c.stream);
+  if (col) {
+    std::vector<unsigned> a(c.nslots);
+    c.adj.download(a.data(), c.nslots, c.stream);
+    for (long s = 0; s < c.nslots; s++) col[s] = (int)(a[s] & STAR_VMASK);
+  }
+  if (hptr) P.hptr.download(hptr, P.nblocks + 1, c.stream);
+  if (hrows) P.hrows.download(hrows, P.hrows.n, c.stream);
+  if (lcol) P.lcol.download(lcol, c.nslots, c.stream);
+  API_END
 }
 const char* pnp_last_error(pnp_ctx* ctx) { return ctx ? ctx->c.err.c_str() : "null context"; }
 long pnp_launch_count(pnp_ctx* ctx) { return ctx ? ctx->c.launches : 0; }
diff --git a/dune_pnp_b200/csrc/pnp_common.cuh b/dune_pnp_b200/csrc/pnp_common.cuh
--- a/dune_pnp_b200/csrc/pnp_common.cuh
+++ b/dune_pnp_b200/csrc/pnp_common.cuh
@@ -67,6 +67,7 @@
   int fd_warp = 1;
   int jac_compact = 1;
   long p2_chunk = 0;
+  int mg_fuse = 1;
 };
 inline Tune& tune() { static Tune t; return t; }
 
diff --git a/dune_pnp_b200/csrc/pnp_spmv_tma.cuh b/dune_pnp_b200/csrc/pnp_spmv_tma.cuh
--- a/dune_pnp_b200/csrc/pnp_spmv_tma.cuh
+++ b/dune_pnp_b200/csrc/pnp_spmv_tma.cuh
@@ -83,6 +83,87 @@
   }
   if constexpr (NP == 1) acc[0] += v[0] * x[0];
   else block_mac<NP>(v, x, acc);
+}
+
+template <int NP, int LPR, bool DG>
+__device__ __forceinline__ void staged_row_acc(const StarOpArgs& a, bool staged, int b0, int len, int sub, const double* sv,
+                                               const int* vb, const unsigned* sc, int cbase, const double* sx, int wlo,
+                                               unsigned wn, double* acc, double* dg) {
+  constexpr int F = NP == 1 ? 1 : 3;
+#pragma unroll
+  for (int k = 0; k < F; k++) acc[k] = 0.0;
+#pragma unroll
+  for (int p = 0; p < NP; p++) dg[p] = 0.0;
+  const int maxlen = __reduce_max_sync(0xffffffffu, len);
+  if (staged) {
+    constexpr int MAXS = (8 + LPR - 1) / LPR;
+    unsigned cj[MAXS];
+    bool okj[MAXS];
+    double xj[MAXS][F];
+#pragma unroll
+    for (int u = 0; u < MAXS; u++) {
+      const int j = sub + u * LPR;
+      okj[u] = j < len;
+      cj[u] = okj[u] ? (sc[b0 + j - cbase] & STAR_VMASK) : 0u;
+    }
+#pragma unroll
+    for (int u = 0; u < MAXS; u++) {
+      const unsigned cw = cj[u] - (unsigned)wlo;
+      const bool in = cw < wn;
+      const bool ldg = okj[u] && !in, lds = okj[u] && in;
+#pragma unroll
+      for (int k = 0; k < F; k++) {
+        double xg = 0.0, xs = 0.0;
+        if (ldg) xg = a.x[(size_t)F * cj[u] + k];
+        if (lds) xs = sx[F * cw + k];
+        xj[u][k] = in ? xs : xg;
+      }
+    }
+#pragma unroll
+    for (int u = 0; u < MAXS; u++) {
+      const int s = b0 + sub + u * LPR;
+      double v[NP];
+#pragma unroll
+      for (int p = 0; p < NP; p++) v[p] = okj[u] ? sv[vb[p] + s] : 0.0;
+      if (DG && u == 0) {
+#pragma unroll
+        for (int p = 0; p < NP; p++) dg[p] = v[p];
+      }
+      if constexpr (NP == 1) acc[0] += v[0] * xj[u][0];
+      else block_mac<NP>(v, xj[u], acc);
+    }
+    for (int j = sub + MAXS * LPR; j < maxlen; j += LPR)
+      slot_product<NP, true>(a, j < len, b0 + j, sv, vb, sc, cbase, sx, wlo, wn, acc, nullptr);
+  } else {
+    slot_product<NP, false>(a, sub < len, b0 + sub, sv, vb, sc, cbase, sx, wlo, wn, acc, DG ? dg : nullptr);
+    for (int j = sub + LPR; j < maxlen; j += LPR)
+      slot_product<NP, false>(a, j < len, b0 + j, sv, vb, sc, cbase, sx, wlo, wn, acc, nullptr);
+  }
+  if (LPR > 1) {
+#pragma unroll
+    for (int k = 0; k < F; k++)
+#pragma unroll
+      for (int o = LPR / 2; o > 0; o >>= 1) acc[k] += __shfl_xor_sync(0xffffffffu, acc[k], o);
+  }
+}
+
+template <int NP>
+__device__ __forceinline__ void jacobi_update(const double* dg, const double* acc, const double* b, const double* x,
+                                              double omega, double* y) {
+  constexpr int F = NP == 1 ? 1 : 3;
+  double r[F], z[F];
+#pragma unroll
+  for (int k = 0; k < F; k++) r[k] = b[k] - acc[k];
+  if constexpr (F == 3) {
+#pragma unroll
+    for (int k = 0; k < F; k++) {
+      double o[3];
+      block_inverse_row<NP>(dg, k, o);
+      z[k] = o[0] * r[0] + o[1] * r[1] + o[2] * r[2];
+    }
+  } else z[0] = (dg[0] != 0.0 ? 1.0 / dg[0] : 0.0) * r[0];
+#pragma unroll
+  for (int k = 0; k < F; k++) y[k] = x[k] + omega * z[k];
 }
 
 template <int NP, int EPI, int NDOT, int LPR>
@@ -186,62 +267,7 @@
       const bool valid = rl < rows;
       const int b0 = valid ? srp[rl] : hi, e0 = valid ? srp[rl + 1] : hi;
       double acc[F], dg[NP];
-#pragma unroll
-      for (int k = 0; k < F; k++) acc[k] = 0.0;
-#pragma unroll
-      for (int p = 0; p < NP; p++) dg[p] = 0.0;
-      const int len = e0 - b0;
-      const int maxlen = __reduce_max_sync(0xffffffffu, len);
-      if (staged) {
-        constexpr int MAXS = (8 + LPR - 1) / LPR;
-        unsigned cj[MAXS];
-        bool okj[MAXS];
-        double xj[MAXS][F];
-#pragma unroll
-        for (int u = 0; u < MAXS; u++) {
-          const int j = sub + u * LPR;
-          okj[u] = j < len;
-          cj[u] = okj[u] ? (sc[b0 + j - cbase] & STAR_VMASK) : 0u;
-        }
-#pragma unroll
-        for (int u = 0; u < MAXS; u++) {
-          const unsigned cw = cj[u] - (unsigned)wlo;
-          const bool in = cw < wn;
-          const bool ldg = okj[u] && !in, lds = okj[u] && in;
-#pragma unroll
-          for (int k = 0; k < F; k++) {
-            double xg = 0.0, xs = 0.0;
-            if (ldg) xg = a.x[(size_t)F * cj[u] + k];
-            if (lds) xs = sx[F * cw + k];
-            xj[u][k] = in ? xs : xg;
-          }
-        }
-#pragma unroll
-        for (int u = 0; u < MAXS; u++) {
-          const int s = b0 + sub + u * LPR;
-          double v[NP];
-#pragma unroll
-          for (int p = 0; p < NP; p++) v[p] = okj[u] ? sv[vb[p] + s] : 0.0;
-          if (EPI == EPI_JACOBI && u == 0) {
-#pragma unroll
-            for (int p = 0; p < NP; p++) dg[p] = v[p];
-          }
-          if constexpr (NP == 1) acc[0] += v[0] * xj[u][0];
-          else block_mac<NP>(v, xj[u], acc);
-        }
-        for (int j = sub + MAXS * LPR; j < maxlen; j += LPR)
-          slot_product<NP, true>(a, j < len, b0 + j, sv, vb, sc, cbase, sx, wlo, wn, acc, nullptr);
-      } else {
-        slot_product<NP, false>(a, sub < len, b0 + sub, sv, vb, sc, cbase, sx, wlo, wn, acc, EPI == EPI_JACOBI ? dg : nullptr);
-        for (int j = sub + LPR; j < maxlen; j += LPR)
-          slot_product<NP, false>(a, j < len, b0 + j, sv, vb, sc, cbase, sx, wlo, wn, acc, nullptr);
-      }
-      if (LPR > 1) {
-#pragma unroll
-        for (int k = 0; k < F; k++)
-#pragma unroll
-          for (int o = LPR / 2; o > 0; o >>= 1) acc[k] += __shfl_xor_sync(0xffffffffu, acc[k], o);
-      }
+      staged_row_acc<NP, LPR, EPI == EPI_JACOBI>(a, staged, b0, e0 - b0, sub, sv, vb, sc, cbase, sx, wlo, wn, acc, dg);
       const bool mine = valid && sub == 0;
       double yv[F];
 #pragma unroll
@@ -257,21 +283,7 @@
         } else if (EPI == EPI_RESIDUAL) {
 #pragma unroll
           for (int k = 0; k < F; k++) yv[k] = sb[F * rl + k] - acc[k];
-        } else {
-          double r[F], z[F];
-#pragma unroll
-          for (int k = 0; k < F; k++) r[k] = sb[F * rl + k] - acc[k];
-          if constexpr (F == 3) {
-#pragma unroll
-            for (int k = 0; k < F; k++) {
-              double o[3];
-              block_inverse_row<NP>(dg, k, o);
-              z[k] = o[0] * r[0] + o[1] * r[1] + o[2] * r[2];
-            }
-          } else z[0] = (dg[0] != 0.0 ? 1.0 / dg[0] : 0.0) * r[0];
-#pragma unroll
-          for (int k = 0; k < F; k++) yv[k] = sxo[F * rl + k] + a.omega * z[k];
-        }
+        } else jacobi_update<NP>(dg, acc, sb + F * rl, sxo + F * rl, a.omega, yv);
       }
       if (sub == 0) {
 #pragma unroll
@@ -307,6 +319,287 @@
         for (int o = 16; o > 0; o >>= 1) s += __shfl_xor_sync(0xffffffffu, s, o);
         if (lane == 0) a.partial[(long)blockIdx.x * NDOT + j] = s;
       }
+    }
+  }
+}
+
+constexpr int FUSE_T = 1024;
+constexpr int FUSE_SMEM_MAX = 227 * 1024;
+
+struct FusePlan {
+  int T = 0, nblocks = 0, hmax = 0;
+  long hns = 0;
+  DBuf<int> hptr;
+  DBuf<int> hrows;
+  DBuf<unsigned short> lcol;
+  DBuf<int> hrp;
+  DBuf<unsigned> hcol;
+  DBuf<double> hvals;
+};
+void fuse_plan_build(Ctx& c, const int* rp, const unsigned* col, int nv, long nslots, int T, FusePlan& P);
+void fuse_plan_values(Ctx& c, FusePlan& P, const int* rp, const double* vals, long stride, int nplanes);
+
+struct FuseArgs {
+  const int* hptr; const int* hrows; const unsigned short* lcol; int T; double* r;
+  const int* hrp; const unsigned* hcol; const double* hvals; long hns;
+};
+
+template <int NP>
+constexpr int fuse_smem_bytes(int stages, int T, int hmax) {
+  return TmaLayout<NP>::smem_bytes(stages) + (T + hmax) * (NP == 1 ? 1 : 3) * 8;
+}
+
+__device__ __forceinline__ void consumer_barrier(int nthreads) { asm volatile("bar.sync 1, %0;" ::"r"(nthreads) : "memory"); }
+
+template <int NP, int LPR>
+__device__ __forceinline__ void local_row_acc(const StarOpArgs& a, const unsigned short* glcol, bool staged, int b0, int len,
+                                              int sub, const double* sv, const int* vb, const unsigned short* slc, int lbase,
+                                              const double* xs, double* acc, double* dg) {
+  constexpr int F = NP == 1 ? 1 : 3;
+#pragma unroll
+  for (int k = 0; k < F; k++) acc[k] = 0.0;
+#pragma unroll
+  for (int p = 0; p < NP; p++) dg[p] = 0.0;
+  for (int j = sub; j < len; j += LPR) {
+    const int s = b0 + j;
+    const unsigned c = staged ? slc[s - lbase] : glcol[s];
+    double x[F], v[NP];
+#pragma unroll
+    for (int k = 0; k < F; k++) x[k] = xs[F * c + k];
+#pragma unroll
+    for (int p = 0; p < NP; p++) v[p] = staged ? sv[vb[p] + s] : a.vals[(size_t)p * a.stride + s];
+    if (j == sub) {
+#pragma unroll
+      for (int p = 0; p < NP; p++) dg[p] = v[p];
+    }
+    if constexpr (NP == 1) acc[0] += v[0] * x[0];
+    else block_mac<NP>(v, x, acc);
+  }
+  if (LPR > 1) {
+#pragma unroll
+    for (int k = 0; k < F; k++)
+#pragma unroll
+      for (int o = LPR / 2; o > 0; o >>= 1) acc[k] += __shfl_xor_sync(0xffffffffu, acc[k], o);
+  }
+}
+
+template <int NP, int SS, int LPR>
+__global__ void __launch_bounds__(tma_threads(NP, EPI_JACOBI, 0, LPR), 1)
+k_star_pair_tma(const StarOpArgs a, const FuseArgs f, const int nstages) {
+  using L = TmaLayout<NP>;
+  constexpr int F = L::F;
+  constexpr int TMA_NW = tma_nw(LPR);
+  constexpr int RW = 32 / LPR;
+  constexpr int NPROD = tma_producers(NP, EPI_JACOBI, 0);
+  extern __shared__ __align__(128) unsigned char smem[];
+  uint64_t* full = reinterpret_cast<uint64_t*>(smem);
+  uint64_t* empty = full + TMA_MAX_STAGES;
+  unsigned char* stages = smem + L::HEAD;
+  double* ybuf = reinterpret_cast<double*>(stages + (size_t)nstages * L::STAGE);
+  double* xs = ybuf + TMA_TR * F;
+  const int warp = threadIdx.x >> 5, lane = threadIdx.x & 31;
+  const int ntiles = (a.nv + TMA_TR - 1) / TMA_TR, tpb = f.T / TMA_TR, nblocks = (ntiles + tpb - 1) / tpb;
+  const int sp = (int)(a.stride & 1);
+  if (threadIdx.x == 0) {
+    for (int s = 0; s < nstages; s++) { mbar_init(&full[s], NPROD); mbar_init(&empty[s], TMA_NW); }
+    asm volatile("fence.mbarrier_init.release.cluster;" ::: "memory");
+  }
+  __syncthreads();
+
+  if (warp >= TMA_NW) {
+    const int role = warp - TMA_NW;
+    const int sph = (int)(f.hns & 1);
+    auto bounds = [&](int blk) { return (blk < nblocks && lane <= tpb) ? a.rp[min((blk * tpb + lane) * TMA_TR, a.nv)] : 0; };
+    auto halo_range = [&](int blk, int& h0, int& h1) { h0 = h1 = 0; if (blk < nblocks) { h0 = f.hptr[blk]; h1 = f.hptr[blk + 1]; } };
+    int cur = bounds(blockIdx.x), it = 0, hc0, hc1, hn0, hn1;
+    halo_range(blockIdx.x, hc0, hc1);
+    int hcur = f.hrp[min(hc0 + lane * TMA_TR, hc1)];
+    halo_range(blockIdx.x + gridDim.x, hn0, hn1);
+    for (int blk = blockIdx.x; blk < nblocks; blk += gridDim.x) {
+      const int nxt = bounds(blk + gridDim.x);
+      const int hnxt = f.hrp[min(hn0 + lane * TMA_TR, hn1)];
+      int hm0, hm1;
+      halo_range(blk + 2 * gridDim.x, hm0, hm1);
+      const int t0 = blk * tpb, nt = min(tpb, ntiles - t0), nht = (hc1 - hc0 + TMA_TR - 1) / TMA_TR;
+      for (int q = 0; q < 2 * nt + nht; q++, it++) {
+        const int ph = q < nt + nht ? 0 : 1, halo = q >= nt && ph == 0, qq = halo ? q - nt : (ph ? q - nt - nht : q);
+        const int bsrc = halo ? hcur : cur;
+        const int lo = __shfl_sync(0xffffffffu, bsrc, qq), hi = __shfl_sync(0xffffffffu, bsrc, qq + 1);
+        if (lane == 0) {
+          const int stage = it % nstages;
+          mbar_wait(&empty[stage], (unsigned)((it / nstages) & 1) ^ 1u);
+          unsigned char* st = stages + (size_t)stage * L::STAGE;
+          const int r0 = halo ? hc0 + qq * TMA_TR : (t0 + qq) * TMA_TR;
+          const int rows = halo ? min(TMA_TR, hc1 - r0) : min(TMA_TR, a.nv - r0);
+          const bool staged = hi - lo <= TMA_CAP;
+          const void* src = nullptr; void* dst = nullptr; unsigned nb = 0;
+          if (role < NP) {
+            if (staged) {
+              const int o = (lo + role * (halo ? sph : sp)) & 1;
+              nb = (unsigned)(((hi - lo + o) + 1) & ~1) * 8u;
+              src = (halo ? f.hvals + (size_t)role * f.hns : a.vals + (size_t)role * a.stride) + (lo - o);
+              dst = st + role * L::PLANE;
+            }
+          } else if (role == NP) {
+            if (staged && ph == 0) {
+              const int lo_c = lo & ~3;
+              nb = (unsigned)(((hi - lo_c) + 3) & ~3) * 4u;
+              src = (halo ? f.hcol : a.col) + lo_c; dst = st + L::COLS;
+            } else if (staged) {
+              const int lo_c = lo & ~7;
+              nb = (unsigned)(((hi - lo_c) + 7) & ~7) * 2u;
+              src = f.lcol + lo_c; dst = st + L::COLS;
+            }
+          } else if (role == NP + 1) {
+            const int o = halo ? (r0 & 3) : 0;
+            nb = (unsigned)((rows + 1 + o + 3) & ~3) * 4u;
+            src = (halo ? f.hrp : a.rp) + (r0 - o); dst = st + L::RP;
+          } else if (role == NP + 2) {
+            if (ph == 0 && !halo) {
+              const int wlo = max(r0 - TMA_W, 0), whi = min(r0 + TMA_TR + TMA_W, a.nv);
+              nb = (unsigned)((F * (whi - wlo) + 1) & ~1) * 8u;
+              src = a.x + (size_t)F * wlo; dst = st + L::XW;
+            }
+          } else if (halo) {
+            const int o = r0 & 3;
+            nb = (unsigned)((rows + o + 3) & ~3) * 4u;
+            src = f.hrows + (r0 - o); dst = st + L::B;
+          } else {
+            nb = (unsigned)((F * rows + 1) & ~1) * 8u;
+            src = a.b + (size_t)F * r0; dst = st + L::B;
+          }
+          if (nb) { mbar_expect_tx(&full[stage], nb); bulk_g2s(dst, src, nb, &full[stage]); }
+          else mbar_arrive(&full[stage]);
+        }
+        __syncwarp();
+      }
+      cur = nxt; hcur = hnxt; hc0 = hn0; hc1 = hn1; hn0 = hm0; hn1 = hm1;
+    }
+  } else {
+    const int sub = lane % LPR;
+    double* yw = ybuf + warp * RW * F;
+    int it = 0;
+    auto store = [&](double* y, int r0, const double* yv) {
+      if (sub == 0) {
+#pragma unroll
+        for (int k = 0; k < F; k++) yw[F * (lane / LPR) + k] = yv[k];
+      }
+      __syncwarp();
+      const size_t g0 = (size_t)F * (r0 + RW * warp), gend = (size_t)F * a.nv;
+#pragma unroll
+      for (int i = lane; i < RW * F; i += 32)
+        if (g0 + i < gend) y[g0 + i] = yw[i];
+      __syncwarp();
+    };
+    for (int blk = blockIdx.x; blk < nblocks; blk += gridDim.x) {
+      const int t0 = blk * tpb, nt = min(tpb, ntiles - t0);
+      for (int q = 0; q < nt; q++, it++) {
+        const int stage = it % nstages;
+        mbar_wait(&full[stage], (unsigned)((it / nstages) & 1));
+        const unsigned char* st = stages + (size_t)stage * L::STAGE;
+        const double* sv = reinterpret_cast<const double*>(st);
+        const unsigned* sc = reinterpret_cast<const unsigned*>(st + L::COLS);
+        const int* srp = reinterpret_cast<const int*>(st + L::RP);
+        const double* sb = reinterpret_cast<const double*>(st + L::B);
+        const double* sx = reinterpret_cast<const double*>(st + L::XW);
+        const int r0 = (t0 + q) * TMA_TR, rows = min(TMA_TR, a.nv - r0);
+        const int wlo = max(r0 - TMA_W, 0);
+        const unsigned wn = (unsigned)(min(r0 + TMA_TR + TMA_W, a.nv) - wlo);
+        const double* sxo = sx + (size_t)F * (r0 - wlo);
+        const int lo = srp[0], hi = srp[rows];
+        const bool staged = hi - lo <= TMA_CAP;
+        const int cbase = lo & ~3;
+        int vb[NP];
+#pragma unroll
+        for (int p = 0; p < NP; p++) vb[p] = p * (TMA_CAP + 2) - lo + ((lo + p * sp) & 1);
+        const int rl = RW * warp + lane / LPR;
+        const bool valid = rl < rows;
+        const int b0 = valid ? srp[rl] : hi, e0 = valid ? srp[rl + 1] : hi;
+        double acc[F], dg[NP], yv[F];
+        staged_row_acc<NP, LPR, true>(a, staged, b0, e0 - b0, sub, sv, vb, sc, cbase, sx, wlo, wn, acc, dg);
+#pragma unroll
+        for (int k = 0; k < F; k++) yv[k] = 0.0;
+        if (valid && sub == 0) {
+          jacobi_update<NP>(dg, acc, sb + F * rl, sxo + F * rl, a.omega, yv);
+#pragma unroll
+          for (int k = 0; k < F; k++) xs[F * (q * TMA_TR + rl) + k] = yv[k];
+        }
+        if (SS == 0) store(a.y, r0, yv);
+        if (lane == 0) mbar_arrive(&empty[stage]);
+      }
+      {
+        const int h0 = f.hptr[blk], nht = (f.hptr[blk + 1] - h0 + TMA_TR - 1) / TMA_TR;
+        const StarOpArgs ah{f.hrp, f.hcol, f.hvals, f.hns, 0, a.x, nullptr};
+        const int sph = (int)(f.hns & 1);
+        for (int q = 0; q < nht; q++, it++) {
+          const int stage = it % nstages;
+          mbar_wait(&full[stage], (unsigned)((it / nstages) & 1));
+          const unsigned char* st = stages + (size_t)stage * L::STAGE;
+          const int r0 = h0 + q * TMA_TR, rows = min(TMA_TR, f.hptr[blk + 1] - r0);
+          const double* sv = reinterpret_cast<const double*>(st);
+          const unsigned* sc = reinterpret_cast<const unsigned*>(st + L::COLS);
+          const int* srp = reinterpret_cast<const int*>(st + L::RP) + (r0 & 3);
+          const int* shr = reinterpret_cast<const int*>(st + L::B) + (r0 & 3);
+          const int lo = srp[0], hi = srp[rows];
+          const bool staged = hi - lo <= TMA_CAP;
+          int vb[NP];
+#pragma unroll
+          for (int p = 0; p < NP; p++) vb[p] = p * (TMA_CAP + 2) - lo + ((lo + p * sph) & 1);
+          const int rl = RW * warp + lane / LPR;
+          const bool valid = rl < rows;
+          const int b0 = valid ? srp[rl] : hi, e0 = valid ? srp[rl + 1] : hi;
+          const int h = valid ? shr[rl] : 0;
+          double hb[F], hx[F];
+#pragma unroll
+          for (int k = 0; k < F; k++) {
+            hb[k] = valid && sub == 0 ? a.b[(size_t)F * h + k] : 0.0;
+            hx[k] = valid && sub == 0 ? a.x[(size_t)F * h + k] : 0.0;
+          }
+          double acc[F], dg[NP];
+          staged_row_acc<NP, LPR, true>(ah, staged, b0, e0 - b0, sub, sv, vb, sc, lo & ~3, nullptr, 0, 0u, acc, dg);
+          if (valid && sub == 0) {
+            double yv[F];
+            jacobi_update<NP>(dg, acc, hb, hx, a.omega, yv);
+#pragma unroll
+            for (int k = 0; k < F; k++) xs[F * (f.T + q * TMA_TR + rl) + k] = yv[k];
+          }
+          __syncwarp();
+          if (lane == 0) mbar_arrive(&empty[stage]);
+        }
+      }
+      consumer_barrier(TMA_NW * 32);
+      for (int q = 0; q < nt; q++, it++) {
+        const int stage = it % nstages;
+        mbar_wait(&full[stage], (unsigned)((it / nstages) & 1));
+        const unsigned char* st = stages + (size_t)stage * L::STAGE;
+        const double* sv = reinterpret_cast<const double*>(st);
+        const unsigned short* slc = reinterpret_cast<const unsigned short*>(st + L::COLS);
+        const int* srp = reinterpret_cast<const int*>(st + L::RP);
+        const double* sb = reinterpret_cast<const double*>(st + L::B);
+        const int r0 = (t0 + q) * TMA_TR, rows = min(TMA_TR, a.nv - r0);
+        const int lo = srp[0], hi = srp[rows];
+        const bool staged = hi - lo <= TMA_CAP;
+        int vb[NP];
+#pragma unroll
+        for (int p = 0; p < NP; p++) vb[p] = p * (TMA_CAP + 2) - lo + ((lo + p * sp) & 1);
+        const int rl = RW * warp + lane / LPR;
+        const bool valid = rl < rows;
+        const int b0 = valid ? srp[rl] : hi, e0 = valid ? srp[rl + 1] : hi;
+        double acc[F], dg[NP], yv[F];
+        local_row_acc<NP, LPR>(a, f.lcol, staged, b0, e0 - b0, sub, sv, vb, slc, lo & ~7, xs, acc, dg);
+#pragma unroll
+        for (int k = 0; k < F; k++) yv[k] = 0.0;
+        if (valid && sub == 0) {
+          if (SS) jacobi_update<NP>(dg, acc, sb + F * rl, xs + F * (q * TMA_TR + rl), a.omega, yv);
+          else {
+#pragma unroll
+            for (int k = 0; k < F; k++) yv[k] = sb[F * rl + k] - acc[k];
+          }
+        }
+        store(SS ? a.y : f.r, r0, yv);
+        if (lane == 0) mbar_arrive(&empty[stage]);
+      }
+      consumer_barrier(TMA_NW * 32);
     }
   }
 }
@@ -366,4 +659,46 @@
   return launch_star_op<EPI, NDOT>(c, nplanes, a);
 }
 
-}
+inline bool star_pair_ok(const Ctx& c, const StarOpArgs& a, const FusePlan& P, int nplanes) {
+  const Tune& t = tune();
+  if (!t.mg_fuse || P.T <= 0 || !star_op_tma_ok(c, a, EPI_JACOBI)) return false;
+  if (t.tma_min_rows < 0 && P.nblocks < 2 * c.sm_count) return false;
+  if (P.hmax > 31 * TMA_TR || P.hvals.n != (size_t)nplanes * P.hns) return false;
+  const int st = star_op_tma_stages();
+  const int smem = nplanes == 1 ? fuse_smem_bytes<1>(st, P.T, P.hmax)
+                 : nplanes == PNP_COMPACT_PLANES ? fuse_smem_bytes<PNP_COMPACT_PLANES>(st, P.T, P.hmax)
+                                                 : fuse_smem_bytes<7>(st, P.T, P.hmax);
+  return smem <= FUSE_SMEM_MAX;
+}
+
+template <int NP, int SS, int LPR>
+inline void launch_star_pair_tma_lpr(Ctx& c, const StarOpArgs& a, const FuseArgs& f, const FusePlan& P) {
+  const int nstages = star_op_tma_stages();
+  static unsigned long long configured = 0;
+  if (!(configured >> (c.device & 63) & 1ull)) {
+    PNP_CUDA(cudaFuncSetAttribute(k_star_pair_tma<NP, SS, LPR>, cudaFuncAttributeMaxDynamicSharedMemorySize, FUSE_SMEM_MAX));
+    configured |= 1ull << (c.device & 63);
+  }
+  const int grid = P.nblocks < c.sm_count ? P.nblocks : c.sm_count;
+  k_star_pair_tma<NP, SS, LPR><<<grid, tma_threads(NP, EPI_JACOBI, 0, LPR), fuse_smem_bytes<NP>(nstages, P.T, P.hmax), c.stream>>>(
+      a, f, nstages);
+  PNP_CHECK_LAUNCH(); c.launches++;
+}
+template <int NP, int SS>
+inline void launch_star_pair_tma_inst(Ctx& c, const StarOpArgs& a, const FuseArgs& f, const FusePlan& P) {
+  if (tune().tma_lpr == 2) launch_star_pair_tma_lpr<NP, SS, 2>(c, a, f, P);
+  else launch_star_pair_tma_lpr<NP, SS, 1>(c, a, f, P);
+}
+
+template <int SS>
+inline void launch_star_pair(Ctx& c, int nplanes, const StarOpArgs& a, const FusePlan& P, double* r, bool fine) {
+  const double F = nplanes == 1 ? 1 : 3;
+  c.acct(fine ? Ctx::ACC_SPMV_FINE : Ctx::ACC_SPMV_COARSE,
+         star_op_bytes<EPI_JACOBI, 0>(nplanes, a) * (1.0 + (double)P.hrows.n / a.nv) + 2.0 * (double)a.stride + 8.0 * F * a.nv);
+  const FuseArgs f{P.hptr.p, P.hrows.p, P.lcol.p, P.T, r, P.hrp.p, P.hcol.p, P.hvals.p, P.hns};
+  if (nplanes == 1) launch_star_pair_tma_inst<1, SS>(c, a, f, P);
+  else if (nplanes == PNP_COMPACT_PLANES) launch_star_pair_tma_inst<PNP_COMPACT_PLANES, SS>(c, a, f, P);
+  else launch_star_pair_tma_inst<7, SS>(c, a, f, P);
+}
+
+}
diff --git a/include/pnp_b200.h b/include/pnp_b200.h
--- a/include/pnp_b200.h
+++ b/include/pnp_b200.h
@@ -30,6 +30,8 @@
 void pnp_ctx_destroy(pnp_ctx* ctx);
 const char* pnp_last_error(pnp_ctx* ctx);
 pnp_status pnp_tune(const char* name, double value);
+pnp_status pnp_fuse_plan_get(pnp_ctx*, int rows_per_block, long* sizes, int* rowptr, int* col, int* hptr, int* hrows,
+                             unsigned short* lcol);
 long pnp_launch_count(pnp_ctx* ctx);
 
 pnp_status pnp_profile_spmv(pnp_ctx*, int enable);
```

Result: slower. 417.7 million (median of 6 runs) (-6.9%).
